# jcribeiro98/V-GAN

Hardware: AMD Instinct MI355X
Metric: V-GAN train steps/sec (batch=1024, d=784) (higher is better)
Workload: dtype f32; MMD contractions of `value`: split-bf16 x3 on the bf16 MFMA with fp32 accumulation (centred operand); the same step with the fp32 MFMA is timed in `fp32_mode`; 1 GPU; configs[2]: MNIST-pixels-as-features stand-in, d=784, batch=1024 (VGAN_no_kl step); global_batch=1024, features=784, latent=49, rows_per_gpu=1024, parallelism=dp1 (row-sharded Gram, replicated front), hip_graph=True, generator=collapsed, chain_association=depth, mmd_precision=bf16x3, gram_tile=64

## Files before the change

include/vgan_hip.h:

```cpp
#ifndef VGAN_HIP_H
#define VGAN_HIP_H

#include <stdint.h>

#ifdef __cplusplus
extern "C" {
#endif

#define VGAN_OK 0
#define VGAN_ERR_ARG 1
#define VGAN_ERR_HIP 2

#define VGAN_ABI_VERSION 11

typedef void* vgan_stream_t;

int vgan_abi_version(void);
const char* vgan_last_error(void);

int vgan_linear_forward(const float* x, int ldx, int x_nslabs, int64_t x_slab_stride, const float* W,
                        int ldw, const float* b, float* y, int ldy, int n, int in, int out,
                        vgan_stream_t stream);
int vgan_linear_backward_input(const float* dy, int lddy, const float* W, int ldw,
                               float* dx, int lddx, int n, int in, int out, vgan_stream_t stream);
int vgan_linear_backward_params(const float* dy, int lddy, const float* x, int ldx, int x_nslabs,
                                int64_t x_slab_stride, float* dW, int lddw, float* db, int n, int in,
                                int out, int splits, int64_t slab_stride, vgan_stream_t stream);
struct vgan_xx_job;
int vgan_linear_backward_params_xx_supported(int n, int in, int out);
int vgan_linear_backward_params_xx(const float* dy, int lddy, const float* x, int ldx, float* dW, int lddw, int n, int in,
                                   int out, const struct vgan_xx_job* xx, vgan_stream_t stream);
int vgan_reduce_slabs(const float* src, int64_t slab_stride, int nslabs, float* dst, int64_t count,
                      vgan_stream_t stream);

typedef struct vgan_logits_chain {
    const float* za;
    const float* At4;
    int32_t ldza, ldat, e0, pad;
} vgan_logits_chain;
int vgan_mask_project_forward(const float* logits, int ldl, const float* data, int ldd,
                              const int32_t* rows, const uint64_t* row_cursor, int row_batches,
                              int row_stride, int row_offset, float* S, float* U, float* Zx, float* Zy,
                              int ldz, float* sqx, float* sqy, int n, int d, const float* center,
                              int norm_split, const vgan_logits_chain* chain, vgan_stream_t stream);
int vgan_col_mean(const float* data, int ldd, int rows, int d, float* out, vgan_stream_t stream);
int vgan_gather_rows(const float* data, int ldd, const int32_t* rows, const uint64_t* row_cursor,
                     int row_batches, int row_stride, int row_offset, float* out, int ldo,
                     float* sq, int n, int d, vgan_stream_t stream);
int vgan_gather_rows_split(const float* data, int ldd, const int32_t* rows, const uint64_t* row_cursor,
                           int row_batches, int row_stride, int row_offset, const float* center, float* out,
                           int ldo, float* sq, int norm_split, uint16_t* Zh, uint16_t* Zl, int kp, int n, int d,
                           vgan_stream_t stream);
int vgan_mask_backward(const float* gU, int ldg, int nslabs, int64_t slab_stride, const float* S,
                       int lds, const uint64_t* colkey, float pen_weight, int row_offset,
                       float* dlogits, int ldo, int n, int d, vgan_stream_t stream);
int vgan_colmax_chunks(int n);
int vgan_colmax(const float* S, int lds, int from_softmax, int row_offset, uint64_t* part,
                uint64_t* colkey, int n, int d, vgan_stream_t stream);
int vgan_colmax_partial(const float* S, int lds, int from_softmax, int row_offset, uint64_t* part,
                        int n, int d, vgan_stream_t stream);
int vgan_mask_from_softmax(const float* S, int lds, float* U, int ldu, int n, int d, vgan_stream_t stream);
int vgan_upper_softmax_forward(const float* logits, int ldl, float* S, float* U, int n, int d,
                               vgan_stream_t stream);

#define VGAN_TILE 64
#define VGAN_TILE_INTS 8
#define VGAN_TF_SLOT_MASK 3
#define VGAN_TF_TWICE 4
#define VGAN_TF_STORE 8
#define VGAN_TF_MIRROR 16
#define VGAN_TF_NEG 32

int vgan_mmd_build_tiles(int n, int grad_mode, int rank, int world, int tile, int32_t* out, int cap);
int vgan_mmd_order_tiles(int32_t* tiles, int count, int tile);

int vgan_mmd_gram(const float* Z, int ldz, const float* sq, int n, int p, const float* bw,
                  const int32_t* tiles, int ntiles, int calibrate,
                  float* Wg, int ldw, int wrow0, float* partial, vgan_stream_t stream);
#define VGAN_RBF_MAX_KERNELS 8
int vgan_mmd_gram_general(const float* Z, int ldz, const float* sq, int n, int p, const float* bw,
                          const int32_t* tiles, int ntiles, const float* multipliers, int n_kernels,
                          float* Wg, int ldw, int wrow0, float* partial, vgan_stream_t stream);
int vgan_mmd_gram_colmax(const float* Z, int ldz, const float* sq, int n, int p, const float* bw,
                         const int32_t* tiles, int ntiles, float* Wg, int ldw, int wrow0, float* partial,
                         const float* S, int lds, int from_softmax, int row_offset, uint64_t* colpart,
                         int nrows, int d, vgan_stream_t stream);
int vgan_mmd_reduce(const float* partial, const int32_t* tiles, int ntiles, double* stats,
                    int zero_first, vgan_stream_t stream);
int vgan_mmd_set_bandwidth(const double* stats, int n, float* bw, vgan_stream_t stream);
int vgan_mmd_loss(const double* stats, const uint64_t* colkey, int n, int d, float weight,
                  float* loss, float* loss_accum, float accum_scale, uint64_t* step_counter,
                  vgan_stream_t stream);
int vgan_mmd_finalize(const float* partial, const int32_t* tiles, int ntiles, const uint64_t* colpart,
                      int chunks, uint64_t* colkey, int n, int d, float weight, double* stats,
                      float* loss, float* loss_accum, float accum_scale, uint64_t* step_counter,
                      vgan_stream_t stream);
typedef struct vgan_finalize_job {
    const float* partial;
    const int32_t* tiles;
    const uint64_t* colpart;
    uint64_t* colkey;
    double* stats;
    float* loss;
    float* loss_accum;
    uint64_t* step_counter;
    int32_t ntiles, chunks, n, d;
    float weight, accum_scale;
    int32_t mode, ntiles_main;
} vgan_finalize_job;
int vgan_mmd_backward(const float* Wg, int ldw, const float* Z, int ldz, int wrow0, int nr,
                      int ncols, int p, const float* mul, int ldmul, const float* mul_shift, float* out,
                      int ldo, int splits, int64_t slab_stride, const vgan_finalize_job* finalize,
                      vgan_stream_t stream);
int vgan_mmd_bf3_prepare(const float* Z, int ldz, int rows, int p, uint16_t* Zh, uint16_t* Zl, int kp,
                         uint16_t* ZTh, uint16_t* ZTl, int kn, vgan_stream_t stream);
int64_t vgan_mmd_gram_bf3_tail_ws_bytes(void);
int vgan_mmd_gram_bf3(const uint16_t* Zh, const uint16_t* Zl, int kp, const float* sq, int n, const float* bw,
                      const int32_t* tiles, int ntiles, int tile, uint16_t* Wh, uint16_t* Wl, int ldw,
                      int wrow0, float* partial, const float* S, int lds, int from_softmax, int row_offset,
                      uint64_t* colpart, int nrows, int d, void* tail_ws, int64_t tail_ws_bytes,
                      float* rs_part, int ldrs, vgan_stream_t stream);
int vgan_mmd_backward_bf3_tile(int nr, int p, int splits, int tile);
int vgan_mmd_backward_bf3(const uint16_t* Wh, const uint16_t* Wl, int ldw, const uint16_t* ZTh,
                          const uint16_t* ZTl, int kn, int kp, const float* Z, int ldz, int wrow0, int nr,
                          int p, const float* mul, int ldmul, const float* mul_shift, float* out, int ldo,
                          int splits, int64_t slab_stride, int tile, const vgan_finalize_job* finalize,
                          vgan_stream_t stream);
int vgan_mmd_backward_bf3_rm(const uint16_t* Wh, const uint16_t* Wl, int ldw, int kn, const uint16_t* Zh,
                             const uint16_t* Zl, int kp, int zrows, const float* Z, int ldz, int wrow0, int nr,
                             int p, const float* mul, int ldmul, const float* mul_shift, float* out, int ldo,
                             int splits, int64_t slab_stride, int tile, const vgan_finalize_job* finalize,
                             const float* rs_part, int ldrs, vgan_stream_t stream);
int vgan_mmd_backward_bf3_rm_xx(const uint16_t* Wh, const uint16_t* Wl, int ldw, int kn, const uint16_t* Zh,
                                const uint16_t* Zl, int kp, int zrows, const float* Z, int ldz, int wrow0, int nr,
                                int p, const float* mul, int ldmul, const float* mul_shift, float* out, int ldo,
                                int splits, int64_t slab_stride, const vgan_finalize_job* finalize,
                                const struct vgan_xx_job* xx, vgan_stream_t stream);
#define VGAN_GEMM_MAX_GROUP 4
#define VGAN_GEMM_NN 0
#define VGAN_GEMM_NT 1
#define VGAN_GEMM_TN 2
#define VGAN_GEMM_NT_NT 3
typedef struct vgan_gemm_problem {
    const float* a;
    const float* b;
    float* c;
    int32_t kind, m, n, k, lda, ldb, ldc, splitk;
    const float* d;
    float* scratch;
    int32_t ldd, k2;
} vgan_gemm_problem;
int vgan_gemm_grouped(const vgan_gemm_problem* problems, int count, vgan_stream_t stream);
typedef struct vgan_adadelta_layer {
    float* w_packed;
    int64_t off_w, off_b;
    int32_t ldp, out, in, pad;
} vgan_adadelta_layer;
typedef struct vgan_grouped_extras {
    const float* copy_src;
    float* copy_dst;
    int64_t copy_count;
    int32_t adadelta, pad;
    float* p;
    float* sq_avg;
    float* acc_delta;
    float lr, rho, eps, weight_decay, grad_scale;
    int32_t ld_extra;
    vgan_adadelta_layer layer[VGAN_GEMM_MAX_GROUP + 1];
    const float* g_extra;
    float* next_noise;
    int32_t noise_rows, noise_cols, noise_ld, noise_ones_col;
    uint64_t seed;
    const uint64_t* step_counter;
    const vgan_finalize_job* fold;
} vgan_grouped_extras;
int vgan_gemm_grouped_ex(const vgan_gemm_problem* problems, int count, const vgan_grouped_extras* extras,
                         vgan_stream_t stream);

typedef struct vgan_xx_job {
    const uint16_t* Dh;
    const uint16_t* Dl;
    const float* dsq;
    const int32_t* tiles;
    const float* bw;
    float* partial;
    int32_t ldd, ntiles;
} vgan_xx_job;
int vgan_mask_project_forward_bf3(const float* logits, int ldl, const float* data, int ldd, const int32_t* rows,
                                  const uint64_t* row_cursor, int row_batches, int row_stride, float* S, float* Z,
                                  int ldz, float* sq, uint16_t* Zh, uint16_t* Zl, int kp, uint16_t* ZTh,
                                  uint16_t* ZTl, int kn, int n, int d, const float* center, int write_x,
                                  const vgan_xx_job* xx, const vgan_logits_chain* chain, vgan_stream_t stream);
int vgan_row_sqnorm(const float* Z, int ldz, float* sq, int rows, int p, vgan_stream_t stream);

int vgan_adadelta_step(float* p, const float* g, int nslabs, int64_t slab_stride, float* sq_avg,
                       float* acc_delta, int64_t count, float lr, float rho, float eps,
                       float weight_decay, float grad_scale, vgan_stream_t stream);

int vgan_noise_normal(float* z, int rows, int cols, int ld, int ones_col, uint64_t seed,
                      const uint64_t* step_counter, uint64_t stream_id, vgan_stream_t stream);

int vgan_homogeneous_pack(const int64_t* desc, int count, int max_elems, int unpack, vgan_stream_t stream);
int vgan_adadelta_step_packed(float* p, const int32_t* pmap, const float* g_packed, float* w_packed,
                              float* sq_avg, float* acc_delta, int64_t count, float lr, float rho,
                              float eps, float weight_decay, float grad_scale, float* next_noise,
                              int noise_rows, int noise_cols, int noise_ld, int noise_ones_col,
                              uint64_t seed, const uint64_t* step_counter, vgan_stream_t stream);

int vgan_mse(const float* a, int lda, const float* b, int ldb, int n, int d, float scale,
             float* out, int accumulate, vgan_stream_t stream);

int vgan_mse_grad(const float* target, int ldt, const float* pred, int ldp, int n, int d, float gscale,
                  double* part, float* g, int ldg, vgan_stream_t stream);
int vgan_sum_f64(const double* in, int count, double scale, float* out, int accumulate, vgan_stream_t stream);

#define VGAN_DP_ID_BYTES 128
typedef struct vgan_dp_comm vgan_dp_comm;
int vgan_dp_unique_id(uint8_t* id );
int vgan_dp_comm_create(vgan_dp_comm** comm, int nranks, const uint8_t* id, int rank);
int vgan_dp_allreduce_sum(vgan_dp_comm* comm, float* buf, int64_t count, vgan_stream_t stream);
int vgan_dp_allgather(vgan_dp_comm* comm, void* buf, int64_t bytes_per_rank, vgan_stream_t stream);
int vgan_dp_comm_destroy(vgan_dp_comm* comm);

int vgan_shuffle_epoch(int32_t* perm, int64_t count, int64_t train_size, uint64_t seed, uint64_t epoch,
                       vgan_stream_t stream);
int64_t vgan_shuffle_index(int64_t i, int64_t train_size, uint64_t seed, uint64_t epoch);
int vgan_mask_unique(const uint8_t* masks, int ldm, int n, int d, uint64_t* keys, int32_t* work,
                     int32_t* out_row, int32_t* out_count, vgan_stream_t stream);

int vgan_rbf_kernel_matrix(const float* Z, int ldz, int m, int p, const float* sq, float alpha, float* K, int ldk,
                           vgan_stream_t stream);
int vgan_rbf_multi_kernel_matrix(const float* Z, int ldz, int m, int p, const float* sq, const float* bw,
                                 const float* multipliers, int n_kernels, float* K, int ldk, float* dK, int lddk,
                                 vgan_stream_t stream);
int vgan_rows_dot(const float* A, int lda, const float* B, int ldb, double* out, int rows, int cols,
                  vgan_stream_t stream);

#define VGAN_OUTLIER_MAX_K 32
#define VGAN_OUTLIER_ENGINE_EXACT 0
#define VGAN_OUTLIER_ENGINE_GRAM 1
#define VGAN_OUTLIER_KNN_LARGEST 0
#define VGAN_OUTLIER_KNN_MEAN 1
#define VGAN_OUTLIER_KNN_MEDIAN 2
#define VGAN_OUTLIER_LRD 3
#define VGAN_OUTLIER_LOF 4
#define VGAN_OUTLIER_KDE_MAX_ROWS 8388607
int vgan_outlier_pack(const float* X, int ldx, int n, int d, const float* center, const int32_t* feat,
                      const int32_t* feat_off, const int64_t* col_off, int first, int count, float* packed, float* sq,
                      vgan_stream_t stream);
int vgan_outlier_knn(const float* Pq, const float* sq_q, int nq, const float* Pr, const float* sq_r, int nr,
                     const int32_t* feat_off, const int64_t* col_off, int first, int count, int k, int exclude_self,
                     int engine, int splits, float* part_d, int32_t* part_i, int32_t* nbr, vgan_stream_t stream);
int vgan_outlier_refine(const float* Xq, int ldq, int nq, const float* Xr, int ldr, int nr, int d, const int32_t* feat,
                        const int32_t* feat_off, int first, int count, const int32_t* nbr, int k, int32_t* out_idx,
                        float* out_dist, float* kdist, vgan_stream_t stream);
int vgan_outlier_score(const int32_t* idx, const float* dist, int nq, int k, int count, int method, const float* kdist_ref,
                       const double* lrd_ref, int nr, float* score, const int32_t* score_row, int ld_score, double* lrd_out,
                       vgan_stream_t stream);
int vgan_outlier_kde(const float* Pq, const float* sq_q, int nq, const float* Pr, const float* sq_r, int nr,
                     const int32_t* feat_off, const int64_t* col_off, int first, int count, const double* bandwidth,
                     int exclude_self, int engine, int splits, uint32_t* pivot, uint64_t* acc, float* score,
                     const int32_t* score_row, int ld_score, vgan_stream_t stream);
int vgan_outlier_combine(const float* score, int ld, int S, int n, const double* weights, double* out,
                         vgan_stream_t stream);
int vgan_outlier_abod(const float* Xq, int ldq, int nq, const float* Xr, int ldr, int nr, int d, const int32_t* feat,
                      const int32_t* feat_off, int first, int count, const int32_t* idx, int k, float* score,
                      const int32_t* score_row, int ld_score, vgan_stream_t stream);
int vgan_outlier_abod_floor(float* score, int ld, int S, int n, int fit, double* score_floor, int32_t* n_degenerate,
                            vgan_stream_t stream);
#define VGAN_OUTLIER_NORM_ZSCORE 1
#define VGAN_OUTLIER_NORM_ROBUST 2
#define VGAN_OUTLIER_NORM_MINMAX 3
#define VGAN_OUTLIER_COMBINE_SUM 0
#define VGAN_OUTLIER_COMBINE_MAX 1
int64_t vgan_outlier_score_stats_ws_bytes(int S, int n, int mode);
int vgan_outlier_score_stats(const float* score, int ld, int S, int n, int mode, double* center, double* scale,
                             void* workspace, int64_t workspace_bytes, vgan_stream_t stream);
int vgan_outlier_combine_normalized(const float* score, int ld, int S, int n, const double* center, const double* scale,
                                    const double* weights, int combination, double* out, vgan_stream_t stream);

#define VGAN_CLUSTER_MAX_CLUSTERS 64
#define VGAN_CLUSTER_SLICE_ROWS 1024
int64_t vgan_cluster_lloyd_ws_bytes(int n, int n_clusters, int count, int total_dims);
int vgan_cluster_image(const double* centers, int n_clusters, const int32_t* feat, const int32_t* feat_off,
                       const int64_t* col_off, int first, int count, const float* col_center, float* img, float* img_sq,
                       vgan_stream_t stream);
int vgan_cluster_lloyd(const float* Pq, const float* sq_q, const float* X, int ldx, int n, int d, const int32_t* feat,
                       const int32_t* feat_off, const int64_t* col_off, int first, int count, int total_dims, int max_dims,
                       int n_clusters, int engine, const float* col_center, const double* tol_var, double* centers,
                       float* img, float* img_sq, int32_t* label, int32_t* changed, int32_t* done, int32_t* n_iter,
                       void* workspace, int64_t workspace_bytes, int iterations, vgan_stream_t stream);
int vgan_cluster_final(const float* Xq, int ldq, int nq, int d, const int32_t* feat, const int32_t* feat_off, int S,
                       int n_clusters, const double* centers, const int32_t* large, int64_t* sizes, int use_weights,
                       int32_t* label, double* inertia_part, double* inertia, float* score, const int32_t* score_row,
                       int ld_score, vgan_stream_t stream);

#ifdef __cplusplus
}
#endif
#endif
```

v-gan_amd/csrc/mmd_bf16.hip:

```cpp
#include "gemm_bf3.hpp"
#include "gemm_bf3w.hpp"
#include "mmd_common.hpp"
#include "mmd_xx.hpp"

namespace vgan {


__global__ __launch_bounds__(kBlock) void bf3_prepare_kernel(const float* __restrict__ Z, int ldz, int rows, int p,
                                                            unsigned short* __restrict__ Zh, unsigned short* __restrict__ Zl, int kp,
                                                            unsigned short* __restrict__ ZTh, unsigned short* __restrict__ ZTl, int kn,
                                                            int vec) {
    __shared__ unsigned short th[64][68], tl[64][68];
    const int j0 = blockIdx.x * 64, k0 = blockIdx.y * 64;
    const int tj = 4 * (threadIdx.x & 15), tk = 4 * (threadIdx.x >> 4);
    unsigned short hi[4][4], lo[4][4];
#pragma unroll
    for (int a = 0; a < 4; ++a) {
        const int k = k0 + tk + a;
        float v[4] = {0.f, 0.f, 0.f, 0.f};
        if (k < rows) {
            if (vec && j0 + tj + 3 < p) {
                const float4 q = *reinterpret_cast<const float4*>(Z + (long)k * ldz + j0 + tj);
                v[0] = q.x; v[1] = q.y; v[2] = q.z; v[3] = q.w;
            } else {
// ... 296 lines not shown
#pragma unroll
            for (int i = 0; i < 4; ++i)
#pragma unroll
                for (int j = 0; j < 4; ++j)
                    __builtin_amdgcn_raw_buffer_store_b128(__builtin_bit_cast(u32x4, acc[i][j]), slabs, mine + (4 * i + j) * (G::NCONS * 16), 0, kCoherent);
        }
        asm volatile("s_waitcnt vmcnt(0)" ::: "memory");
        __syncthreads();
        if (threadIdx.x == 0) {
            const int old = __hip_atomic_fetch_add(ts.tickets + tq, 1, __ATOMIC_RELAXED, __HIP_MEMORY_SCOPE_AGENT);
            last_part = old == ts.parts - 1;
            if (old == ts.parts - 1) __hip_atomic_store(ts.tickets + tq, 0, __ATOMIC_RELAXED, __HIP_MEMORY_SCOPE_AGENT);
        }
        __syncthreads();
        if (!last_part) return;
        if (cons) {
#pragma unroll
            for (int i = 0; i < 4; ++i)
#pragma unroll
                for (int j = 0; j < 4; ++j) acc[i][j] = f32x4w{0.f, 0.f, 0.f, 0.f};
            for (int q = 0; q < ts.parts; ++q) {
                const int theirs = slab0 + q * (int)kTailSlabBytes + threadIdx.x * 16;
#pragma unroll
                for (int i = 0; i < 4; ++i)
#pragma unroll
                    for (int j = 0; j < 4; ++j)
                        acc[i][j] += __builtin_bit_cast(f32x4w, __builtin_amdgcn_raw_buffer_load_b128(slabs, theirs + (4 * i + j) * (G::NCONS * 16), 0, kCoherent));
            }
        }
    }

    const float c2 = -1.4426950408889634f / (4.f * bw);
    const float wscale = -((td.flags & VGAN_TF_NEG) ? -1.f : 1.f) * 2.f / ((float)n * (float)n * bw);
    const bool store = (td.flags & VGAN_TF_STORE) && Wh != nullptr;
    const bool mirror = store && (td.flags & VGAN_TF_MIRROR);
    float ksum = 0.f;
    if (cons) {
#pragma unroll
        for (int i = 0; i < 4; ++i)
#pragma unroll
            for (int j = 0; j < 4; ++j)
#pragma unroll
                for (int r = 0; r < 4; ++r) {
                    const bool ok = (td.r0 + G::sub_row(i, r) < td.rlim) && (td.c0 + G::sub_col(j) < td.clim);
                    const float L = fmaxf(siv[i][r] + sjv[j] - 2.f * acc[i][j][r], 0.f);
                    const float t = __builtin_amdgcn_exp2f(L * c2);
                    const float t2 = t * t, t4 = t2 * t2, t8 = t4 * t4, t16 = t8 * t8;
                    ksum += ok ? ((t + t2) + (t4 + t8)) + t16 : 0.f;
                    acc[i][j][r] = wscale * (((0.25f * t + 0.5f * t2) + (t4 + 2.f * t8)) + 4.f * t16);
                }
    }
    if (store) {
        lds_f* Wt = (lds_f*)(float*)lds;
        auto emit = [&](const float (&w)[16], long rowo, int c_first, int c_lim) -> float {
            unsigned hp[8], lp[8];
            float sums[4] = {0.f, 0.f, 0.f, 0.f};
#pragma unroll
            for (int e = 0; e < 8; ++e) {
                unsigned short h0, l0, h1, l1;
                split_bf16(w[2 * e], h0, l0);
                split_bf16(w[2 * e + 1], h1, l1);
                hp[e] = (unsigned)h0 | ((unsigned)h1 << 16);
                lp[e] = (unsigned)l0 | ((unsigned)l1 << 16);
                const float v0 = __uint_as_float((unsigned)h0 << 16) + __uint_as_float((unsigned)l0 << 16);
                const float v1 = __uint_as_float((unsigned)h1 << 16) + __uint_as_float((unsigned)l1 << 16);
                sums[e & 3] += (c_first + 2 * e < c_lim ? v0 : 0.f) + (c_first + 2 * e + 1 < c_lim ? v1 : 0.f);
            }
            if (c_first + 15 < c_lim) {
                uint4* dh = reinterpret_cast<uint4*>(Wh + rowo + c_first);
                uint4* dl = reinterpret_cast<uint4*>(Wl + rowo + c_first);
                dh[0] = make_uint4(hp[0], hp[1], hp[2], hp[3]);
                dh[1] = make_uint4(hp[4], hp[5], hp[6], hp[7]);
                dl[0] = make_uint4(lp[0], lp[1], lp[2], lp[3]);
                dl[1] = make_uint4(lp[4], lp[5], lp[6], lp[7]);
            } else {
#pragma unroll
                for (int e = 0; e < 16; ++e)
                    if (c_first + e < c_lim) {
                        Wh[rowo + c_first + e] = (unsigned short)(hp[e >> 1] >> (16 * (e & 1)));
                        Wl[rowo + c_first + e] = (unsigned short)(lp[e >> 1] >> (16 * (e & 1)));
                    }
            }
            return (sums[0] + sums[1]) + (sums[2] + sums[3]);
        };
        auto slot_sum = [&](float v) -> float {
            v += __shfl_xor(v, 1);
            v += __shfl_xor(v, 2);
            v += __shfl_xor(v, 4);
            return v;
        };
        float w[16];
        if (cons) {
#pragma unroll
            for (int i = 0; i < 4; ++i)
#pragma unroll
                for (int j = 0; j < 4; ++j)
#pragma unroll
                    for (int r = 0; r < 4; ++r) Wt[G::sub_row(i, r) * LDT + G::sub_col(j)] = acc[i][j][r];
        }
        __syncthreads();
        for (int t = threadIdx.x; t < 256 * 8; t += G::NTH) {
            const int line = t >> 3, q16 = 16 * (t & 7);
            float cs = 0.f;
            if (td.r0 + line < td.rlim && td.c0 + q16 < td.clim) {
#pragma unroll
                for (int e = 0; e < 4; ++e) {
                    const f32x4 v = *(const lds_f4*)(Wt + line * LDT + q16 + 4 * e);
                    w[4 * e] = v[0]; w[4 * e + 1] = v[1]; w[4 * e + 2] = v[2]; w[4 * e + 3] = v[3];
                }
                cs = emit(w, (long)(td.r0 + line - wrow0) * ldw, td.c0 + q16, td.clim);
            }
            if (rs_part != nullptr) {
                cs = slot_sum(cs);
                if ((t & 7) == 0 && td.r0 + line < td.rlim) rs_part[(long)(td.c0 >> 7) * ldrs + (td.r0 + line - wrow0)] = cs;
            }
        }
        if (mirror) {
            __syncthreads();
            if (cons) {
#pragma unroll
                for (int i = 0; i < 4; ++i)
#pragma unroll
                    for (int j = 0; j < 4; ++j)
                        *(lds_f4*)(Wt + G::sub_col(j) * LDM + G::sub_row(i, 0)) = f32x4{acc[i][j][0], acc[i][j][1], acc[i][j][2], acc[i][j][3]};
            }
            __syncthreads();
            for (int t = threadIdx.x; t < 128 * 16; t += G::NTH) {
                const int line = t >> 4, q16 = 16 * (t & 15);
                float cs = 0.f;
                if (td.c0 + line < td.clim && td.r0 + q16 < td.rlim) {
#pragma unroll
                    for (int e = 0; e < 4; ++e) {
                        const f32x4 v = *(const lds_f4*)(Wt + line * LDM + q16 + 4 * e);
                        w[4 * e] = v[0]; w[4 * e + 1] = v[1]; w[4 * e + 2] = v[2]; w[4 * e + 3] = v[3];
                    }
                    cs = emit(w, (long)(td.c0 + line - wrow0) * ldw, td.r0 + q16, td.rlim);
                }
                if (rs_part != nullptr) {
                    cs = slot_sum(cs);
                    if ((t & 7) == 0 && td.c0 + line < td.clim && td.r0 + q16 < td.rlim)
                        rs_part[(long)((td.r0 + q16) >> 7) * ldrs + (td.c0 + line - wrow0)] = cs;
                }
            }
        }
    }
    ksum = wave_sum(ksum);
    if (lane == 0) red[wave] = ksum;
    __syncthreads();
    if (threadIdx.x == 0)
        reinterpret_cast<float4*>(partial)[ti] =
            make_float4(((red[0] + red[1]) + (red[2] + red[3])) + ((red[4] + red[5]) + (red[6] + red[7])), 0.f, 0.f, 0.f);
}

template <int BK, bool RM>
__global__ __launch_bounds__(kBlock, BK == 64 ? 2 : 3) void mmd_backward_bf3_kernel(const unsigned short* __restrict__ Wh, const unsigned short* __restrict__ Wl,
                                                                    int ldw, const unsigned short* __restrict__ ZTh,
                                                                    const unsigned short* __restrict__ ZTl, int kn, int ldb, int brows,
                                                                    const float* __restrict__ Z, int ldz, int wrow0, int nr, int p,
                                                                    int ptiles, const float* __restrict__ mul, int ldmul,
                                                                    const float* __restrict__ mul_shift, float* __restrict__ out, int ldo,
                                                                    int kchunk, long slab_stride, vgan_finalize_job job, int nfin,
                                                                    XXJob xx) {
    using G = GemmBF3<BK>;
    constexpr int kBytes = (RM ? G::kLdsBytesT : G::kLdsBytes) > G::kLdsBytes ? (RM ? G::kLdsBytesT : G::kLdsBytes) : G::kLdsBytes;
    __shared__ __attribute__((aligned(16))) char lds[kBytes];
    __shared__ float rs[64];
    const int gx = ptiles, gy = (nr + 63) / 64, total = gx * gy;
    if ((int)blockIdx.x >= total) {
        if (blockIdx.y != 0) return;
        const int extra = (int)blockIdx.x - total;
        if (extra < nfin)
            finalize_body(job);
        else if constexpr (BK == 64)
            xx_tile_body(xx, extra - nfin, lds, rs);
        return;
    }
    const int xcd = blockIdx.x % 8, kidx = blockIdx.x / 8;
    const int q = total / 8, r8 = total % 8;
    const int t = (xcd < r8 ? xcd * (q + 1) : r8 * (q + 1) + (xcd - r8) * q) + kidx;
    const int band = t / (4 * gx), rem = t - band * 4 * gx;
    const int rows_in_band = min(4, gy - band * 4);
    const int m0 = (band * 4 + rem % rows_in_band) * 64, n0 = (rem / rows_in_band) * 64;
    f32x16 acc;
#pragma unroll
    for (int r = 0; r < 16; ++r) acc[r] = 0.f;
    const int k0 = blockIdx.y * kchunk, klen = min(kchunk, kn - k0);
    out += blockIdx.y * slab_stride;
    const int col = n0 + G::sub_col(), colc = min(col, p - 1);
    float z_pre[16], m_pre[16];
    const float mshift = mul_shift != nullptr ? mul_shift[colc] : 0.f;
#pragma unroll
    for (int r = 0; r < 16; ++r) {
        const int rowc = min(m0 + G::sub_row(r), nr - 1);
        z_pre[r] = Z[(long)(wrow0 + rowc) * ldz + colc];
        m_pre[r] = mul != nullptr ? mul[(long)rowc * ldmul + colc] + mshift : 1.f;
    }
    if (klen > 0) {
        if constexpr (RM)
            G::template run_bt<true>(Wh + k0, Wl + k0, ldw, ZTh + (long)k0 * ldb, ZTl + (long)k0 * ldb, ldb, brows - k0, m0, n0, nr, klen, lds,
                                     rs, acc);
        else
            G::template run<true>(Wh + k0, Wl + k0, ldw, ZTh + k0, ZTl + k0, ldb, m0, n0, nr, gx * 64, klen, lds, rs, acc);
    }
    if (col >= p) return;
#pragma unroll
    for (int r = 0; r < 16; ++r) {
        const int lrow = G::sub_row(r), row = m0 + lrow;
        if (row < nr) {
            const float v = klen > 0 ? 2.f * (rs[lrow] * z_pre[r] - acc[r]) : 0.f;
            out[(long)row * ldo + col] = v * m_pre[r];
        }
    }
}

template <bool RM>
__global__ __launch_bounds__(512, 2) void mmd_backward_bf3_big_kernel(const unsigned short* __restrict__ Wh, const unsigned short* __restrict__ Wl,
                                                                      int ldw, const unsigned short* __restrict__ ZTh,
                                                                      const unsigned short* __restrict__ ZTl, int kn, int ldb, int brows,
                                                                      const float* __restrict__ Z, int ldz, int wrow0, int nr, int p,
                                                                      int ptiles, const float* __restrict__ mul, int ldmul,
                                                                      const float* __restrict__ mul_shift, float* __restrict__ out, int ldo,
                                                                      int kchunk, long slab_stride, int nb_rows, vgan_finalize_job job) {
    using G = GemmBF3Big;
    __shared__ __attribute__((aligned(16))) char lds[RM ? G::kLdsBytesT : G::kLdsBytes];
    __shared__ float rs[128];
    const int gx = ptiles, gy = (nr + 127) / 128, total = gx * gy;
    if ((int)blockIdx.x >= total) {
        if (blockIdx.y == 0) finalize_body(job);
        return;
    }
    const int xcd = blockIdx.x % 8, kidx = blockIdx.x / 8;
    const int q = total / 8, r8 = total % 8;
    const int t = (xcd < r8 ? xcd * (q + 1) : r8 * (q + 1) + (xcd - r8) * q) + kidx;
    const int band = t / (4 * gx), rem = t - band * 4 * gx;
    const int rows_in_band = min(4, gy - band * 4);
    const int m0 = (band * 4 + rem % rows_in_band) * 128, n0 = (rem / rows_in_band) * 128;
    const int k0 = blockIdx.y * kchunk, klen = min(kchunk, kn - k0);
    out += blockIdx.y * slab_stride;
    const int col = n0 + G::sub_col(), colc = min(col, p - 1);
    const float mshift = mul_shift != nullptr ? mul_shift[colc] : 0.f;
    f32x16 acc[2];
#pragma unroll
    for (int i2 = 0; i2 < 2; ++i2)
#pragma unroll
        for (int r = 0; r < 16; ++r) acc[i2][r] = 0.f;
    if (klen > 0) {
        if constexpr (RM)
            G::template run_bt<true>(Wh + k0, Wl + k0, ldw, ZTh + (long)k0 * ldb, ZTl + (long)k0 * ldb, ldb, nb_rows, brows - k0, m0, n0, nr, klen,
                                     lds, acc, rs);
        else
            G::template run<true>(Wh + k0, Wl + k0, ldw, ZTh + k0, ZTl + k0, ldb, m0, n0, nr, nb_rows, klen, lds, acc, rs);
    }
    if (col >= p) return;
#pragma unroll
    for (int i2 = 0; i2 < 2; ++i2) {
        float z_pre[16], m_pre[16];
#pragma unroll
        for (int r = 0; r < 16; ++r) {
            const int rowc = min(m0 + G::sub_row(i2, r), nr - 1);
            z_pre[r] = Z[(long)(wrow0 + rowc) * ldz + colc];
            m_pre[r] = mul != nullptr ? mul[(long)rowc * ldmul + colc] + mshift : 1.f;
        }
#pragma unroll
        for (int r = 0; r < 16; ++r) {
            const int lrow = G::sub_row(i2, r), row = m0 + lrow;
            if (row < nr) {
                const float v = klen > 0 ? 2.f * (rs[lrow] * z_pre[r] - acc[i2][r]) : 0.f;
                out[(long)row * ldo + col] = v * m_pre[r];
            }
        }
    }
}


__global__ __launch_bounds__(768, 3) void mmd_backward_bf3_wide_kernel(const unsigned short* __restrict__ Wh, const unsigned short* __restrict__ Wl,
                                                                       int ldw, const unsigned short* __restrict__ Bh,
                                                                       const unsigned short* __restrict__ Bl, int kn, int ldb, int brows,
                                                                       const float* __restrict__ Z, int ldz, int wrow0, int nr, int p,
                                                                       int ptiles, const float* __restrict__ mul, int ldmul,
                                                                       const float* __restrict__ mul_shift, float* __restrict__ out, int ldo,
                                                                       int kchunk, long slab_stride, int nb_cols, vgan_finalize_job job,
                                                                       const float* __restrict__ rs_part, int ldrs) {
    using G = GemmBF3Wide;
    extern __shared__ __attribute__((aligned(16))) char lds[];
    __shared__ float rs[256];
    const int gx = ptiles, gy = (nr + 255) / 256, total = gx * gy;
    if ((int)blockIdx.x >= total) {
        if (blockIdx.y == 0) finalize_body(job);
        return;
    }
    const int xcd = blockIdx.x % 8, kidx = blockIdx.x / 8;
    const int q = total / 8, r8 = total % 8;
    const int t = (xcd < r8 ? xcd * (q + 1) : r8 * (q + 1) + (xcd - r8) * q) + kidx;
    const int band = t / (4 * gx), rem = t - band * 4 * gx;
    const int rows_in_band = min(4, gy - band * 4);
    const int m0 = (band * 4 + rem % rows_in_band) * 256, n0 = (rem / rows_in_band) * 128;
    const int k0 = blockIdx.y * kchunk, klen = min(kchunk, kn - k0);
    out += blockIdx.y * slab_stride;
    f32x4w acc[4][4];
#pragma unroll
    for (int i = 0; i < 4; ++i)
#pragma unroll
        for (int j = 0; j < 4; ++j) acc[i][j] = f32x4w{0.f, 0.f, 0.f, 0.f};
    if (klen > 0 && rs_part != nullptr) {
        if (threadIdx.x < 256) {
            const float* src = rs_part + min(m0 + (int)threadIdx.x, nr - 1);
            const int s0 = k0 >> 7, s1 = (k0 + klen + 127) >> 7;
            float a0 = 0.f, a1 = 0.f, a2 = 0.f, a3 = 0.f;
            int sl = s0;
            for (; sl + 4 <= s1; sl += 4) {
                a0 += src[(long)sl * ldrs];
                a1 += src[(long)(sl + 1) * ldrs];
                a2 += src[(long)(sl + 2) * ldrs];
                a3 += src[(long)(sl + 3) * ldrs];
            }
            for (; sl < s1; ++sl) a0 += src[(long)sl * ldrs];
            rs[threadIdx.x] = (a0 + a1) + (a2 + a3);
        }
        G::run_bt<false>(Wh + k0, Wl + k0, ldw, Bh + (long)k0 * ldb, Bl + (long)k0 * ldb, ldb, nb_cols, brows - k0, m0, n0, nr, klen, lds, acc);
    } else if (klen > 0)
        G::run_bt<true>(Wh + k0, Wl + k0, ldw, Bh + (long)k0 * ldb, Bl + (long)k0 * ldb, ldb, nb_cols, brows - k0, m0, n0, nr, klen, lds, acc, rs);
    if (G::is_loader()) return;
#pragma unroll
    for (int j = 0; j < 4; ++j) {
        const int col = n0 + G::sub_col(j);
        if (col >= p) continue;
        const float mshift = mul_shift != nullptr ? mul_shift[col] : 0.f;
#pragma unroll
        for (int i = 0; i < 4; ++i) {
            float z_pre[4], m_pre[4];
#pragma unroll
            for (int r = 0; r < 4; ++r) {
                const int rowc = min(m0 + G::sub_row(i, r), nr - 1);
                z_pre[r] = Z[(long)(wrow0 + rowc) * ldz + col];
                m_pre[r] = mul != nullptr ? mul[(long)rowc * ldmul + col] + mshift : 1.f;
            }
#pragma unroll
            for (int r = 0; r < 4; ++r) {
                const int lrow = G::sub_row(i, r), row = m0 + lrow;
                if (row < nr) {
                    const float v = klen > 0 ? 2.f * (rs[lrow] * z_pre[r] - acc[i][j][r]) : 0.f;
                    out[(long)row * ldo + col] = v * m_pre[r];
                }
            }
        }
    }
}

}

using namespace vgan;

extern "C" int vgan_mmd_bf3_prepare(const float* Z, int ldz, int rows, int p, uint16_t* Zh, uint16_t* Zl, int kp, uint16_t* ZTh,
                                    uint16_t* ZTl, int kn, vgan_stream_t stream) {
    VGAN_CHECK_ARG(Z && Zh && Zl && rows > 0 && p > 0 && ldz >= p && kp >= p && kp % 64 == 0 && aligned16(Zh) && aligned16(Zl));
    VGAN_CHECK_ARG((ZTh == nullptr) == (ZTl == nullptr) && (ZTh == nullptr || (kn >= rows && kn % 64 == 0)));
    dim3 grid(kp / 64, (rows + 63) / 64);
    if (ZTh != nullptr) grid.y = kn / 64;
    const int vec = (ldz % 4 == 0) && aligned16(Z);
    hipLaunchKernelGGL(bf3_prepare_kernel, grid, dim3(kBlock), 0, (hipStream_t)stream, Z, ldz, rows, p, Zh, Zl, kp, ZTh, ZTl, kn, vec);
    VGAN_CHECK_LAUNCH();
    return VGAN_OK;
}

#ifndef VGAN_TAIL_MAX_PARTS
#define VGAN_TAIL_MAX_PARTS 4
#endif
extern "C" int64_t vgan_mmd_gram_bf3_tail_ws_bytes(void) { return kTailSlabs * kTailSlabBytes + kTailTicketBytes; }

extern "C" int vgan_mmd_gram_bf3(const uint16_t* Zh, const uint16_t* Zl, int kp, const float* sq, int n, const float* bw,
                                 const int32_t* tiles, int ntiles, int tile, uint16_t* Wh, uint16_t* Wl, int ldw, int wrow0,
                                 float* partial, const float* S, int lds, int from_softmax, int row_offset, uint64_t* colpart,
                                 int nrows, int d, void* tail_ws, int64_t tail_ws_bytes, float* rs_part, int ldrs,
                                 vgan_stream_t stream) {
    VGAN_CHECK_ARG(Zh && Zl && sq && bw && tiles && partial && n > 0 && ntiles > 0 && kp > 0 && kp % 64 == 0);
    VGAN_CHECK_ARG((Wh == nullptr) == (Wl == nullptr) && (reinterpret_cast<uintptr_t>(partial) & 15) == 0);
    VGAN_CHECK_ARG(aligned16(Zh) && aligned16(Zl) && (Wh == nullptr || (aligned16(Wh) && aligned16(Wl))));
    ColmaxJob cj{};
    int extra = 0;
    if (S != nullptr) {
        VGAN_CHECK_ARG(colpart && nrows > 0 && d > 0 && lds >= d);
        cj = ColmaxJob{S, reinterpret_cast<unsigned long long*>(colpart), lds, row_offset, nrows, d, from_softmax, (d + 63) / 64};
        extra = cj.nbx * ((nrows + kColChunkRows - 1) / kColChunkRows);
    }
    VGAN_CHECK_ARG(tile == 64 || tile == 128 || tile == 256);
    VGAN_CHECK_ARG(rs_part == nullptr || (tile == 256 && Wh != nullptr && ldrs > 0 && wrow0 >= 0 && n % 128 == 0));
    if (tile == 256) {
        static const hipError_t attr = hipFuncSetAttribute(reinterpret_cast<const void*>(&mmd_gram_bf3_wide_kernel),
                                                           hipFuncAttributeMaxDynamicSharedMemorySize, GemmBF3Wide::kLdsBytes);
        VGAN_CHECK_ARG(attr == hipSuccess);
        TailSplit ts{nullptr, nullptr, ntiles, 1, kp};
        if (tail_ws != nullptr) {
            VGAN_CHECK_ARG(tail_ws_bytes >= vgan_mmd_gram_bf3_tail_ws_bytes() && aligned16(tail_ws));
            static const int cus = [] {
                int dev = 0, v = 0;
                if (hipGetDevice(&dev) != hipSuccess || hipDeviceGetAttribute(&v, hipDeviceAttributeMultiprocessorCount, dev) != hipSuccess) v = 0;
                return v;
            }();
            const int slots = cus < kTailSlabs ? cus : kTailSlabs;
            const int r = slots > 0 ? ntiles % slots : 0, nst = kp / GemmBF3Wide::BK;
            int parts = 1;
            while (r > 0 && parts < VGAN_TAIL_MAX_PARTS && 2 * parts * r <= slots && nst / (2 * parts) >= 8) parts *= 2;
            if (parts > 1) {
                const int kchunk = ((nst + parts - 1) / parts) * GemmBF3Wide::BK;
                ts = TailSplit{static_cast<float*>(tail_ws), reinterpret_cast<int*>(static_cast<char*>(tail_ws) + kTailSlabs * kTailSlabBytes),
                               ntiles - r, (kp + kchunk - 1) / kchunk, kchunk};
            }
        }
        const int nblk = ts.first + (ntiles - ts.first) * ts.parts;
        hipLaunchKernelGGL(mmd_gram_bf3_wide_kernel, dim3(nblk + extra), dim3(GemmBF3Wide::NTH), GemmBF3Wide::kLdsBytes, (hipStream_t)stream, Zh,
                           Zl, kp, sq, n, bw, reinterpret_cast<const TileDesc*>(tiles), ntiles, Wh, Wl, ldw, wrow0, partial, cj, ts, rs_part, ldrs);
    } else if (tile == 128)
        hipLaunchKernelGGL(mmd_gram_bf3_big_kernel, dim3(ntiles + extra), dim3(512), 0, (hipStream_t)stream, Zh, Zl, kp, sq, n, bw,
                           reinterpret_cast<const TileDesc*>(tiles), ntiles, Wh, Wl, ldw, wrow0, partial, cj);
    else
        hipLaunchKernelGGL(mmd_gram_bf3_kernel<64>, dim3(ntiles + extra), dim3(kBlock), 0, (hipStream_t)stream, Zh, Zl, kp, sq, n, bw,
                           reinterpret_cast<const TileDesc*>(tiles), ntiles, Wh, Wl, ldw, wrow0, partial, cj);
    VGAN_CHECK_LAUNCH();
    return VGAN_OK;
}

extern "C" int vgan_mmd_backward_bf3_tile(int nr, int p, int splits, int tile) {
    if (tile == 64 || tile == 128 || tile == 256) return tile;
    const int wide_tiles = ((p + 127) / 128) * ((nr + 255) / 256);
    if (nr >= 256 && wide_tiles * splits >= 256) return 256;
    const int big_tiles = ((p + 127) / 128) * ((nr + 127) / 128);
    return big_tiles * splits >= 512 ? 128 : 64;
}

static int launch_backward_bf3(int rm, const uint16_t* Wh, const uint16_t* Wl, int ldw, const uint16_t* Bh, const uint16_t* Bl, int kn, int kp,
                               int zrows, const float* Z, int ldz, int wrow0, int nr, int p, const float* mul, int ldmul,
                               const float* mul_shift, float* out, int ldo, int splits, int64_t slab_stride, int tile,
                               const vgan_finalize_job* finalize, vgan_stream_t stream, const vgan_xx_job* xxjob = nullptr,
                               const float* rs_part = nullptr, int ldrs = 0) {
    VGAN_CHECK_ARG(Wh && Wl && Bh && Bl && Z && out && nr > 0 && p > 0 && kn > 0 && kn % 64 == 0 && kp >= p && kp % 64 == 0);
    VGAN_CHECK_ARG(ldw >= kn && ldz >= p && ldo >= p && (mul == nullptr || ldmul >= p) && wrow0 >= 0);
    VGAN_CHECK_ARG(aligned16(Wh) && aligned16(Wl) && aligned16(Bh) && aligned16(Bl) && ldw % 8 == 0);
    VGAN_CHECK_ARG(splits >= 1 && splits <= 64 && (splits == 1 || slab_stride >= (int64_t)nr * ldo));
    VGAN_CHECK_ARG((tile == 0 || tile == 64 || tile == 128 || tile == 256) && (mul_shift == nullptr || mul != nullptr) && (!rm || zrows > 0));
    const int kchunk = ((kn / 64 + splits - 1) / splits) * 64;
    const int ldb = rm ? kp : kn;
    vgan_finalize_job job{};
    if (finalize != nullptr) {
        VGAN_CHECK_ARG(finalize_job_ok(*finalize));
        job = *finalize;
    }
    hipStream_t st = (hipStream_t)stream;
    XXJob xx{};
    if (xxjob != nullptr) {
        const vgan_xx_job& j = *xxjob;
        VGAN_CHECK_ARG(rm && tile == 64 && j.Dh && j.Dl && j.dsq && j.tiles && j.bw && j.partial && j.ntiles > 0 && j.ldd % 64 == 0 &&
                       aligned16(j.Dh) && aligned16(j.Dl) && (reinterpret_cast<uintptr_t>(j.partial) & 15) == 0);
        xx = XXJob{j.Dh, j.Dl, j.dsq, nullptr, nullptr, reinterpret_cast<const TileDesc*>(j.tiles), j.bw, j.partial, j.ldd, 1, 0, j.ntiles, 0};
    }
    const int nfin = finalize != nullptr ? 1 : 0;
    int edge = vgan_mmd_backward_bf3_tile(nr, p, splits, tile);
    if (edge == 256 && !rm) edge = 128;
    if (edge == 256) {
        static const hipError_t attr = hipFuncSetAttribute(reinterpret_cast<const void*>(&mmd_backward_bf3_wide_kernel),
                                                           hipFuncAttributeMaxDynamicSharedMemorySize, GemmBF3Wide::kLdsBytes);
        VGAN_CHECK_ARG(attr == hipSuccess);
        const int pt = (p + 127) / 128;
        dim3 grid(pt * ((nr + 255) / 256) + nfin, splits);
        if (rs_part != nullptr && !(ldrs >= nr && (splits == 1 || kchunk % 128 == 0))) rs_part = nullptr;
        hipLaunchKernelGGL(mmd_backward_bf3_wide_kernel, grid, dim3(GemmBF3Wide::NTH), GemmBF3Wide::kLdsBytes, st, Wh, Wl, ldw, Bh, Bl, kn, ldb,
                           zrows, Z, ldz, wrow0, nr, p, pt, mul, ldmul, mul_shift, out, ldo, kchunk, (long)slab_stride, kp, job, rs_part, ldrs);
        VGAN_CHECK_LAUNCH();
        return VGAN_OK;
    }
    if (edge == 128) {
        const int pt = (p + 127) / 128;
        dim3 grid(pt * ((nr + 127) / 128) + (finalize != nullptr ? 1 : 0), splits);
        if (rm)
            hipLaunchKernelGGL(mmd_backward_bf3_big_kernel<true>, grid, dim3(512), 0, st, Wh, Wl, ldw, Bh, Bl, kn, ldb, zrows, Z, ldz, wrow0, nr,
                               p, pt, mul, ldmul, mul_shift, out, ldo, kchunk, (long)slab_stride, kp, job);
        else
            hipLaunchKernelGGL(mmd_backward_bf3_big_kernel<false>, grid, dim3(512), 0, st, Wh, Wl, ldw, Bh, Bl, kn, ldb, 0, Z, ldz, wrow0, nr, p,
                               pt, mul, ldmul, mul_shift, out, ldo, kchunk, (long)slab_stride, kp, job);
        VGAN_CHECK_LAUNCH();
        return VGAN_OK;
    }
    const int ptiles = (p + 63) / 64;
    dim3 grid(ptiles * ((nr + 63) / 64) + nfin + xx.ntiles, splits);
    if (rm)
        hipLaunchKernelGGL((mmd_backward_bf3_kernel<64, true>), grid, dim3(kBlock), 0, st, Wh, Wl, ldw, Bh, Bl, kn, ldb, zrows, Z, ldz, wrow0, nr,
                           p, ptiles, mul, ldmul, mul_shift, out, ldo, kchunk, (long)slab_stride, job, nfin, xx);
    else
        hipLaunchKernelGGL((mmd_backward_bf3_kernel<64, false>), grid, dim3(kBlock), 0, st, Wh, Wl, ldw, Bh, Bl, kn, ldb, 0, Z, ldz, wrow0, nr, p,
                           ptiles, mul, ldmul, mul_shift, out, ldo, kchunk, (long)slab_stride, job, nfin, xx);
    VGAN_CHECK_LAUNCH();
    return VGAN_OK;
}

extern "C" int vgan_mmd_backward_bf3(const uint16_t* Wh, const uint16_t* Wl, int ldw, const uint16_t* ZTh, const uint16_t* ZTl, int kn,
                                     int kp, const float* Z, int ldz, int wrow0, int nr, int p, const float* mul, int ldmul,
                                     const float* mul_shift, float* out, int ldo, int splits, int64_t slab_stride, int tile,
                                     const vgan_finalize_job* finalize, vgan_stream_t stream) {
    return launch_backward_bf3(0, Wh, Wl, ldw, ZTh, ZTl, kn, kp, 0, Z, ldz, wrow0, nr, p, mul, ldmul, mul_shift, out, ldo, splits, slab_stride,
                               tile, finalize, stream);
}

extern "C" int vgan_mmd_backward_bf3_rm_xx(const uint16_t* Wh, const uint16_t* Wl, int ldw, int kn, const uint16_t* Zh, const uint16_t* Zl,
                                           int kp, int zrows, const float* Z, int ldz, int wrow0, int nr, int p, const float* mul, int ldmul,
                                           const float* mul_shift, float* out, int ldo, int splits, int64_t slab_stride,
                                           const vgan_finalize_job* finalize, const vgan_xx_job* xx, vgan_stream_t stream) {
    VGAN_CHECK_ARG(xx != nullptr);
    return launch_backward_bf3(1, Wh, Wl, ldw, Zh, Zl, kn, kp, zrows, Z, ldz, wrow0, nr, p, mul, ldmul, mul_shift, out, ldo, splits,
                               slab_stride, 64, finalize, stream, xx);
}

extern "C" int vgan_mmd_backward_bf3_rm(const uint16_t* Wh, const uint16_t* Wl, int ldw, int kn, const uint16_t* Zh, const uint16_t* Zl,
                                        int kp, int zrows, const float* Z, int ldz, int wrow0, int nr, int p, const float* mul, int ldmul,
                                        const float* mul_shift, float* out, int ldo, int splits, int64_t slab_stride, int tile,
                                        const vgan_finalize_job* finalize, const float* rs_part, int ldrs, vgan_stream_t stream) {
    return launch_backward_bf3(1, Wh, Wl, ldw, Zh, Zl, kn, kp, zrows, Z, ldz, wrow0, nr, p, mul, ldmul, mul_shift, out, ldo, splits,
                               slab_stride, tile, finalize, stream, nullptr, rs_part, ldrs);
}
```

v-gan_amd/csrc/rows.hip:

```cpp
#include "mmd_xx.hpp"
#include "vgan_common.hpp"

namespace vgan {

constexpr int kRowsPerBlock = kBlock / kWave;

struct RowSel {
    const int* rows;
    const unsigned long long* cursor;
    int row_batches, row_stride, row_offset;
    __device__ __forceinline__ long operator()(int i) const {
        if (rows == nullptr) return (long)(row_offset + i);
        const long b = cursor ? (long)(cursor[0] % (unsigned long long)row_batches) : 0l;
        return (long)rows[b * row_stride + row_offset + i];
    }
};

__device__ __forceinline__ float project_centred(float u, float x, float c) {
#pragma clang fp contract(off)
    const float y = u * x;
    return y - c;
}

template <bool PROJECT>
__global__ __launch_bounds__(kBlock) void mask_forward_kernel(const float* __restrict__ logits, int ldl, const float* __restrict__ data,
                                                             int ldd, RowSel rows, float* __restrict__ S,
                                                             float* __restrict__ U, float* __restrict__ Zx, float* __restrict__ Zy,
                                                             int ldz, float* __restrict__ sqx, float* __restrict__ sqy, int n, int d,
                                                             const float* __restrict__ center, int norm_split) {
    const int lane = threadIdx.x & 63;
    const int i = blockIdx.x * kRowsPerBlock + (threadIdx.x >> 6);
    if (i >= n) return;
    const float* x = logits + (long)i * ldl;
    float m = -INFINITY;
    for (int j = lane; j < d; j += 64) m = fmaxf(m, x[j]);
    m = wave_max(m);
    float sum = 0.f;
    for (int j = lane; j < d; j += 64) sum += expf(x[j] - m);
    sum = wave_sum(sum);
    const float tau = 1.0f / (float)d;
    const float* xr = nullptr;
    float *zx = nullptr, *zy = nullptr;
    if constexpr (PROJECT) {
        const long src = rows(i);
        xr = data + src * ldd;
        zx = Zx ? Zx + (long)i * ldz : nullptr;
        zy = Zy + (long)i * ldz;
    }
    float nx = 0.f, ny = 0.f;
    for (int j = lane; j < d; j += 64) {
        const float s = expf(x[j] - m) / sum;
        const float u = s < tau ? s : 1.0f;
        S[(long)i * d + j] = s;
        if (U) U[(long)i * d + j] = u;
        if constexpr (PROJECT) {
            const float c = center ? center[j] : 0.f;
            const float xv = xr[j] - c;
            const float yv = project_centred(u, xr[j], c);
            if (zx) zx[j] = xv;
            zy[j] = yv;
            const float xn = norm_split ? split_value(xv) : xv, yn = norm_split ? split_value(yv) : yv;
            nx = fmaf(xn, xn, nx);
            ny = fmaf(yn, yn, ny);
        }
    }
    if constexpr (PROJECT) {
        nx = wave_sum(nx);
        ny = wave_sum(ny);
        if (lane == 0) {
            if (sqx) sqx[i] = nx;
            sqy[i] = ny;
        }
    }
}


struct LogitsChain {
    const float* za;
    const float* At4;
    int ldza, ldat, e0;
};
constexpr int kChainK = 16;
__host__ __device__ constexpr int chain_pitch(int d) { return ((d + 3) / 4) * 4 + 4; }

template <int NT>
__device__ __forceinline__ void chain_logits(const LogitsChain& ch, float* __restrict__ lds_at, int d, int row, bool row_ok, float4 (&v)[NT]) {
    const int lane = threadIdx.x & 63, nq = d >> 2, pitch = chain_pitch(d);
#pragma unroll
    for (int t = 0; t < NT; ++t) v[t] = make_float4(0.f, 0.f, 0.f, 0.f);
    const float* zr = ch.za + (long)(row_ok ? row : 0) * ch.ldza;
    for (int kc = 0; kc < ch.e0; kc += kChainK) {
        __syncthreads();
        for (int idx = threadIdx.x; idx < d * (kChainK / 4); idx += blockDim.x) {
            const int col = idx / (kChainK / 4), kq = idx % (kChainK / 4), k = kc + 4 * kq;
            const float4 a = k < ch.e0 ? *reinterpret_cast<const float4*>(ch.At4 + (long)col * ch.ldat + k) : make_float4(0.f, 0.f, 0.f, 0.f);
            lds_at[(4 * kq + 0) * pitch + col] = a.x;
            lds_at[(4 * kq + 1) * pitch + col] = a.y;
            lds_at[(4 * kq + 2) * pitch + col] = a.z;
            lds_at[(4 * kq + 3) * pitch + col] = a.w;
        }
        __syncthreads();
        const int kw = min(kChainK, ch.e0 - kc);
        for (int k = 0; k < kw; ++k) {
            const float z = zr[kc + k];
#pragma unroll
            for (int t = 0; t < NT; ++t) {
                const int q = min(lane + 64 * t, nq - 1);
                const float4 a = *reinterpret_cast<const float4*>(lds_at + k * pitch + 4 * q);
                v[t].x = fmaf(z, a.x, v[t].x);
                v[t].y = fmaf(z, a.y, v[t].y);
                v[t].z = fmaf(z, a.z, v[t].z);
                v[t].w = fmaf(z, a.w, v[t].w);
            }
        }
    }
#pragma unroll
    for (int t = 0; t < NT; ++t)
        if (lane + 64 * t >= nq) v[t] = make_float4(-INFINITY, -INFINITY, -INFINITY, -INFINITY);
}

template <int NT, bool CHAIN>
__global__ __launch_bounds__(kBlock) void mask_forward_vec_kernel(const float* __restrict__ logits, int ldl, const float* __restrict__ data,
                                                                 int ldd, RowSel rows, float* __restrict__ S, float* __restrict__ U,
                                                                 float* __restrict__ Zx, float* __restrict__ Zy, int ldz,
                                                                 float* __restrict__ sqx, float* __restrict__ sqy, int n, int d,
                                                                 const float* __restrict__ center, int norm_split, LogitsChain ch) {
    extern __shared__ __attribute__((aligned(16))) float chain_lds[];
    const int lane = threadIdx.x & 63;
    const int i = blockIdx.x * kRowsPerBlock + (threadIdx.x >> 6);
    const int nq = d >> 2;
    float4 v[NT], xv[NT], cv[NT];
    if constexpr (CHAIN) chain_logits<NT>(ch, chain_lds, d, i, i < n, v);
    if (i >= n) return;
    const float4* x4 = reinterpret_cast<const float4*>(logits + (long)i * ldl);
    const float4* xr4 = reinterpret_cast<const float4*>(data + rows(i) * ldd);
#pragma unroll
    for (int t = 0; t < NT; ++t) {
        const int q = lane + 64 * t;
        const bool ok = q < nq;
        if constexpr (!CHAIN) v[t] = ok ? x4[min(q, nq - 1)] : make_float4(-INFINITY, -INFINITY, -INFINITY, -INFINITY);
        xv[t] = xr4[min(q, nq - 1)];
        cv[t] = center ? reinterpret_cast<const float4*>(center)[min(q, nq - 1)] : make_float4(0.f, 0.f, 0.f, 0.f);
    }
    float m = -INFINITY;
#pragma unroll
    for (int t = 0; t < NT; ++t) m = fmaxf(m, fmaxf(fmaxf(v[t].x, v[t].y), fmaxf(v[t].z, v[t].w)));
    m = wave_max(m);
    float sum = 0.f;
#pragma unroll
    for (int t = 0; t < NT; ++t) {
        v[t].x = expf(v[t].x - m); v[t].y = expf(v[t].y - m); v[t].z = expf(v[t].z - m); v[t].w = expf(v[t].w - m);
        sum += (v[t].x + v[t].y) + (v[t].z + v[t].w);
    }
    sum = wave_sum(sum);
    const float tau = 1.0f / (float)d;
    float nx = 0.f, ny = 0.f;
#pragma unroll
    for (int t = 0; t < NT; ++t) {
        const int q = lane + 64 * t;
        if (q < nq) {
            float4 s4 = make_float4(v[t].x / sum, v[t].y / sum, v[t].z / sum, v[t].w / sum);
            float4 u4 = make_float4(s4.x < tau ? s4.x : 1.f, s4.y < tau ? s4.y : 1.f, s4.z < tau ? s4.z : 1.f, s4.w < tau ? s4.w : 1.f);
            const float4 x4c = make_float4(xv[t].x - cv[t].x, xv[t].y - cv[t].y, xv[t].z - cv[t].z, xv[t].w - cv[t].w);
            const float4 y4 = make_float4(project_centred(u4.x, xv[t].x, cv[t].x), project_centred(u4.y, xv[t].y, cv[t].y), project_centred(u4.z, xv[t].z, cv[t].z),
                                              project_centred(u4.w, xv[t].w, cv[t].w));
            reinterpret_cast<float4*>(S + (long)i * d)[q] = s4;
            if (U) reinterpret_cast<float4*>(U + (long)i * d)[q] = u4;
            if (Zx) reinterpret_cast<float4*>(Zx + (long)i * ldz)[q] = x4c;
            reinterpret_cast<float4*>(Zy + (long)i * ldz)[q] = y4;
            const float xs[4] = {x4c.x, x4c.y, x4c.z, x4c.w}, ys[4] = {y4.x, y4.y, y4.z, y4.w};
            float xn[4], yn[4];
#pragma unroll
            for (int e = 0; e < 4; ++e) {
                xn[e] = norm_split ? split_value(xs[e]) : xs[e];
                yn[e] = norm_split ? split_value(ys[e]) : ys[e];
            }
            nx += (xn[0] * xn[0] + xn[1] * xn[1]) + (xn[2] * xn[2] + xn[3] * xn[3]);
            ny += (yn[0] * yn[0] + yn[1] * yn[1]) + (yn[2] * yn[2] + yn[3] * yn[3]);
        }
    }
    nx = wave_sum(nx);
    ny = wave_sum(ny);
    if (lane == 0) {
        if (sqx) sqx[i] = nx;
        sqy[i] = ny;
    }
}

template <int NT, bool XX, bool CHAIN>
__global__ __launch_bounds__(512) void mask_forward_bf3_kernel(const float* __restrict__ logits, int ldl, const float* __restrict__ data,
                                                                 int ldd, RowSel rows, float* __restrict__ S, float* __restrict__ Z,
                                                                 int ldz, float* __restrict__ sq, unsigned short* __restrict__ Zh,
                                                                 unsigned short* __restrict__ Zl, int kp, unsigned short* __restrict__ ZTh,
                                                                 unsigned short* __restrict__ ZTl, int kn, int n, int d,
                                                                 const float* __restrict__ center, int write_x, int mask_blocks,
                                                                 XXJob xx, LogitsChain ch) {
    constexpr int R = 8;
    if constexpr (XX) {
        __shared__ __attribute__((aligned(16))) char xx_lds[GemmBF3<64>::kLdsBytes];
        __shared__ float xx_red[4];
        if ((int)blockIdx.x >= mask_blocks) {
            xx_tile_body(xx, blockIdx.x - mask_blocks, xx_lds, xx_red);
            return;
        }
    }
    extern __shared__ __attribute__((aligned(16))) unsigned short tile[];
    const int ldt = 4 * (d >> 2) + 8;
    const int lane = threadIdx.x & 63, wave = threadIdx.x >> 6;
    const int nq = d >> 2;
    const int groups = n / R, C = (groups + 7) / 8;
    const int grp = (blockIdx.x % 8) * C + blockIdx.x / 8;
    if (grp >= groups) return;
    const int i0 = grp * R;
    const float tau = 1.0f / (float)d;
    {
        const int lr = wave, i = i0 + lr;
        float4 v[NT];
        if constexpr (CHAIN) chain_logits<NT>(ch, reinterpret_cast<float*>(tile), d, i, i < n, v);
        if (i < n) {
            const float4* x4 = reinterpret_cast<const float4*>(logits + (long)i * ldl);
            const float4* xr4 = reinterpret_cast<const float4*>(data + rows(i) * ldd);
            float4 xv[NT], cv[NT];
#pragma unroll
            for (int t = 0; t < NT; ++t) {
                const int q = lane + 64 * t;
                const bool ok = q < nq;
                if constexpr (!CHAIN) v[t] = ok ? x4[min(q, nq - 1)] : make_float4(-INFINITY, -INFINITY, -INFINITY, -INFINITY);
                xv[t] = xr4[min(q, nq - 1)];
                cv[t] = center ? reinterpret_cast<const float4*>(center)[min(q, nq - 1)] : make_float4(0.f, 0.f, 0.f, 0.f);
            }
            float m = -INFINITY;
#pragma unroll
            for (int t = 0; t < NT; ++t) m = fmaxf(m, fmaxf(fmaxf(v[t].x, v[t].y), fmaxf(v[t].z, v[t].w)));
            m = wave_max(m);
            float sum = 0.f;
#pragma unroll
            for (int t = 0; t < NT; ++t) {
                v[t].x = expf(v[t].x - m); v[t].y = expf(v[t].y - m); v[t].z = expf(v[t].z - m); v[t].w = expf(v[t].w - m);
                sum += (v[t].x + v[t].y) + (v[t].z + v[t].w);
            }
            sum = wave_sum(sum);
            float nx = 0.f, ny = 0.f;
#pragma unroll
            for (int t = 0; t < NT; ++t) {
                const int q = lane + 64 * t;
                if (q < nq) {
                    const float4 s4 = make_float4(v[t].x / sum, v[t].y / sum, v[t].z / sum, v[t].w / sum);
                    const float4 u4 = make_float4(s4.x < tau ? s4.x : 1.f, s4.y < tau ? s4.y : 1.f, s4.z < tau ? s4.z : 1.f, s4.w < tau ? s4.w : 1.f);
                    const float4 x4c = make_float4(xv[t].x - cv[t].x, xv[t].y - cv[t].y, xv[t].z - cv[t].z, xv[t].w - cv[t].w);
                    const float4 y4 = make_float4(project_centred(u4.x, xv[t].x, cv[t].x), project_centred(u4.y, xv[t].y, cv[t].y), project_centred(u4.z, xv[t].z, cv[t].z),
                                              project_centred(u4.w, xv[t].w, cv[t].w));
                    reinterpret_cast<float4*>(S + (long)i * d)[q] = s4;
                    if (write_x) reinterpret_cast<float4*>(Z + (long)i * ldz)[q] = x4c;
                    reinterpret_cast<float4*>(Z + (long)(n + i) * ldz)[q] = y4;
                    const float xs[4] = {x4c.x, x4c.y, x4c.z, x4c.w}, ys[4] = {y4.x, y4.y, y4.z, y4.w};
                    unsigned short h[2][4], l[2][4];
                    float xn[4], yn[4];
#pragma unroll
                    for (int e = 0; e < 4; ++e) {
                        split_bf16(xs[e], h[0][e], l[0][e]);
                        split_bf16(ys[e], h[1][e], l[1][e]);
                        xn[e] = bf16_val(h[0][e]) + bf16_val(l[0][e]);
                        yn[e] = bf16_val(h[1][e]) + bf16_val(l[1][e]);
                    }
                    nx += (xn[0] * xn[0] + xn[1] * xn[1]) + (xn[2] * xn[2] + xn[3] * xn[3]);
                    ny += (yn[0] * yn[0] + yn[1] * yn[1]) + (yn[2] * yn[2] + yn[3] * yn[3]);
#pragma unroll
                    for (int im = 0; im < 2; ++im) {
                        const uint2 ph = make_uint2((unsigned)h[im][0] | ((unsigned)h[im][1] << 16), (unsigned)h[im][2] | ((unsigned)h[im][3] << 16));
                        const uint2 pl = make_uint2((unsigned)l[im][0] | ((unsigned)l[im][1] << 16), (unsigned)l[im][2] | ((unsigned)l[im][3] << 16));
                        const long grow = (long)(im * n + i) * kp + 4 * q;
                        if (im == 1 || write_x) {
                            *reinterpret_cast<uint2*>(Zh + grow) = ph;
                            *reinterpret_cast<uint2*>(Zl + grow) = pl;
                        }
                        if (ZTh != nullptr) {
                            *reinterpret_cast<uint2*>(tile + ((2 * im) * R + lr) * ldt + 4 * q) = ph;
                            *reinterpret_cast<uint2*>(tile + ((2 * im + 1) * R + lr) * ldt + 4 * q) = pl;
                        }
                    }
                }
            }
            nx = wave_sum(nx);
            ny = wave_sum(ny);
            if (lane == 0) {
                if (write_x) sq[i] = nx;
                sq[n + i] = ny;
            }
        } else if (ZTh != nullptr) {
            for (int c = lane; c < ldt; c += 64)
#pragma unroll
                for (int im = 0; im < 4; ++im) tile[(im * R + lr) * ldt + c] = 0;
        }
    }
    if (ZTh == nullptr) return;
    __syncthreads();
    const int npairs = d >> 1;
    for (int item = threadIdx.x; item < 4 * npairs; item += 512) {
        const int im = item / npairs, j = 2 * (item - im * npairs);
        unsigned w0[4], w1[4];
#pragma unroll
        for (int e = 0; e < 4; ++e) {
            const unsigned a = *reinterpret_cast<const unsigned*>(tile + (im * R + 2 * e) * ldt + j);
            const unsigned c = *reinterpret_cast<const unsigned*>(tile + (im * R + 2 * e + 1) * ldt + j);
            w0[e] = (a & 0xFFFFu) | (c << 16);
            w1[e] = (a >> 16) | (c & 0xFFFF0000u);
        }
        unsigned short* dst = ((im & 1) ? ZTl : ZTh) + (long)j * kn + (im >> 1) * n + i0;
        *reinterpret_cast<uint4*>(dst) = make_uint4(w0[0], w0[1], w0[2], w0[3]);
        *reinterpret_cast<uint4*>(dst + kn) = make_uint4(w1[0], w1[1], w1[2], w1[3]);
    }
}

template <int NT>
__global__ __launch_bounds__(kBlock) void mask_backward_vec_kernel(const float* __restrict__ gU, int ldg, const float* __restrict__ S,
                                                                  int lds, const unsigned long long* __restrict__ colkey,
                                                                  float pen_weight, int row_offset, float* __restrict__ dlogits,
                                                                  int ldo, int n, int d, int nslabs, long slab_stride) {
    const int lane = threadIdx.x & 63;
    const int i = blockIdx.x * kRowsPerBlock + (threadIdx.x >> 6);
    if (i >= n) return;
    const int nq = d >> 2;
    const float tau = 1.0f / (float)d;
    const float pg = -pen_weight / (float)d;
    const unsigned me = (unsigned)(row_offset + i);
    float4 sv[NT], gs[NT];
    float dot = 0.f;
#pragma unroll
    for (int t = 0; t < NT; ++t) {
        const int q = min(lane + 64 * t, nq - 1);
        const bool ok = lane + 64 * t < nq;
        sv[t] = reinterpret_cast<const float4*>(S + (long)i * lds)[q];
        float4 g = reinterpret_cast<const float4*>(gU + (long)i * ldg)[q];
        for (int sl = 1; sl < nslabs; ++sl) {
            const float4 b = reinterpret_cast<const float4*>(gU + sl * slab_stride + (long)i * ldg)[q];
            g.x += b.x; g.y += b.y; g.z += b.z; g.w += b.w;
        }
        if (colkey != nullptr) {
            const ulonglong2 k0 = reinterpret_cast<const ulonglong2*>(colkey)[2 * q], k1 = reinterpret_cast<const ulonglong2*>(colkey)[2 * q + 1];
            if (colkey_row(k0.x) == me) g.x += pg;
            if (colkey_row(k0.y) == me) g.y += pg;
            if (colkey_row(k1.x) == me) g.z += pg;
            if (colkey_row(k1.y) == me) g.w += pg;
        }
        gs[t] = make_float4(ok && sv[t].x < tau ? g.x : 0.f, ok && sv[t].y < tau ? g.y : 0.f, ok && sv[t].z < tau ? g.z : 0.f,
                            ok && sv[t].w < tau ? g.w : 0.f);
        dot += (gs[t].x * sv[t].x + gs[t].y * sv[t].y) + (gs[t].z * sv[t].z + gs[t].w * sv[t].w);
    }
    dot = wave_sum(dot);
#pragma unroll
    for (int t = 0; t < NT; ++t) {
        const int q = lane + 64 * t;
        if (q < nq)
            reinterpret_cast<float4*>(dlogits + (long)i * ldo)[q] =
                make_float4(sv[t].x * (gs[t].x - dot), sv[t].y * (gs[t].y - dot), sv[t].z * (gs[t].z - dot), sv[t].w * (gs[t].w - dot));
    }
}

__global__ __launch_bounds__(kBlock) void mask_backward_kernel(const float* __restrict__ gU, int ldg, const float* __restrict__ S,
                                                              int lds, const unsigned long long* __restrict__ colkey,
                                                              float pen_weight, int row_offset, float* __restrict__ dlogits,
                                                              int ldo, int n, int d, int nslabs, long slab_stride) {
    const int lane = threadIdx.x & 63;
    const int i = blockIdx.x * kRowsPerBlock + (threadIdx.x >> 6);
    if (i >= n) return;
    const float tau = 1.0f / (float)d;
    const float pg = -pen_weight / (float)d;
    const float* g = gU + (long)i * ldg;
    const float* s = S + (long)i * lds;
    const unsigned me = (unsigned)(row_offset + i);
    auto grad = [&](int j) {
        float gv = g[j];
        for (int q = 1; q < nslabs; ++q) gv += g[q * slab_stride + j];
        if (colkey != nullptr && colkey_row(colkey[j]) == me) gv += pg;
        return gv;
    };
    float dot = 0.f;
    for (int j = lane; j < d; j += 64) {
        const float sv = s[j];
        dot = fmaf(sv < tau ? grad(j) : 0.f, sv, dot);
    }
    dot = wave_sum(dot);
    for (int j = lane; j < d; j += 64) {
        const float sv = s[j];
        dlogits[(long)i * ldo + j] = sv * ((sv < tau ? grad(j) : 0.f) - dot);
    }
}

__global__ __launch_bounds__(kBlock) void colmax_partial_kernel(const float* __restrict__ S, int lds, int row_offset,
                                                               unsigned long long* __restrict__ part, int n, int d, int from_softmax) {
    colmax_partial_body<4>(S, lds, row_offset, part, n, d, from_softmax, blockIdx.x, blockIdx.y);
}
__global__ void colmax_final_kernel(const unsigned long long* __restrict__ part, int chunks, unsigned long long* __restrict__ colkey,
                                    int d) {
    const int j = blockIdx.x * blockDim.x + threadIdx.x;
    if (j >= d) return;
    unsigned long long b = 0ull;
    for (int c = 0; c < chunks; ++c) {
        const unsigned long long k = part[(long)c * d + j];
        b = k > b ? k : b;
    }
    colkey[j] = b;
}

__global__ __launch_bounds__(kBlock) void gather_rows_kernel(const float* __restrict__ data, int ldd, RowSel rows,
                                                            float* __restrict__ out, int ldo, float* __restrict__ sq, int n, int d) {
    const int lane = threadIdx.x & 63;
    const int i = blockIdx.x * kRowsPerBlock + (threadIdx.x >> 6);
    if (i >= n) return;
    const float* x = data + rows(i) * ldd;
    float* o = out + (long)i * ldo;
    float nx = 0.f;
    for (int j = lane; j < d; j += 64) {
        const float v = x[j];
        o[j] = v;
        nx = fmaf(v, v, nx);
    }
    nx = wave_sum(nx);
    if (lane == 0 && sq) sq[i] = nx;
}

__global__ __launch_bounds__(kBlock) void gather_center_split_kernel(const float* __restrict__ data, int ldd, RowSel rows,
                                                                    const float* __restrict__ center, float* __restrict__ out, int ldo,
                                                                    float* __restrict__ sq, int norm_split,
                                                                    unsigned short* __restrict__ Zh, unsigned short* __restrict__ Zl,
                                                                    int kp, int n, int d) {
    const int lane = threadIdx.x & 63;
    const int i = blockIdx.x * kRowsPerBlock + (threadIdx.x >> 6);
    if (i >= n) return;
    const float* x = data + rows(i) * ldd;
    float nx = 0.f;
    for (int j = lane; j < d; j += 64) {
        const float v = x[j] - (center ? center[j] : 0.f);
        if (out) out[(long)i * ldo + j] = v;
        unsigned short hi, lo;
        split_bf16(v, hi, lo);
        if (Zh) {
            Zh[(long)i * kp + j] = hi;
            Zl[(long)i * kp + j] = lo;
        }
        const float vn = norm_split ? bf16_val(hi) + bf16_val(lo) : v;
        nx = fmaf(vn, vn, nx);
    }
    nx = wave_sum(nx);
    if (lane == 0 && sq) sq[i] = nx;
}

__global__ __launch_bounds__(kBlock) void gather_center_split_vec_kernel(const float* __restrict__ data, int ldd, RowSel rows,
                                                                        const float* __restrict__ center, float* __restrict__ out, int ldo,
                                                                        float* __restrict__ sq, int norm_split,
                                                                        unsigned short* __restrict__ Zh, unsigned short* __restrict__ Zl,
                                                                        int kp, int n, int d) {
    const int lane = threadIdx.x & 63;
    const int i = blockIdx.x * kRowsPerBlock + (threadIdx.x >> 6);
    if (i >= n) return;
    const float4* x4 = reinterpret_cast<const float4*>(data + rows(i) * ldd);
    const int nq = d >> 2;
    float nx = 0.f;
    for (int q = lane; q < nq; q += 64) {
        float4 v = x4[q];
        if (center) {
            const float4 c = reinterpret_cast<const float4*>(center)[q];
            v.x -= c.x; v.y -= c.y; v.z -= c.z; v.w -= c.w;
        }
        if (out) reinterpret_cast<float4*>(out + (long)i * ldo)[q] = v;
        const float vs[4] = {v.x, v.y, v.z, v.w};
        unsigned short h[4], l[4];
        float vn[4];
#pragma unroll
        for (int e = 0; e < 4; ++e) {
            split_bf16(vs[e], h[e], l[e]);
            vn[e] = norm_split ? bf16_val(h[e]) + bf16_val(l[e]) : vs[e];
        }
        if (Zh) {
            *reinterpret_cast<uint2*>(Zh + (long)i * kp + 4 * q) = make_uint2((unsigned)h[0] | ((unsigned)h[1] << 16), (unsigned)h[2] | ((unsigned)h[3] << 16));
            *reinterpret_cast<uint2*>(Zl + (long)i * kp + 4 * q) = make_uint2((unsigned)l[0] | ((unsigned)l[1] << 16), (unsigned)l[2] | ((unsigned)l[3] << 16));
        }
        nx += (vn[0] * vn[0] + vn[1] * vn[1]) + (vn[2] * vn[2] + vn[3] * vn[3]);
    }
    nx = wave_sum(nx);
    if (lane == 0 && sq) sq[i] = nx;
}

__global__ void mask_from_softmax_kernel(const float* __restrict__ S, int lds, float* __restrict__ U, int ldu, int n, int d) {
    const long idx = (long)blockIdx.x * blockDim.x + threadIdx.x;
    if (idx >= (long)n * d) return;
    const int i = (int)(idx / d), j = (int)(idx % d);
    const float sv = S[(long)i * lds + j];
    U[(long)i * ldu + j] = sv < 1.0f / (float)d ? sv : 1.0f;
}

}

using namespace vgan;

extern "C" int vgan_mask_project_forward(const float* logits, int ldl, const float* data, int ldd, const int32_t* rows,
                                         const uint64_t* row_cursor, int row_batches, int row_stride, int row_offset, float* S,
                                         float* U, float* Zx, float* Zy, int ldz, float* sqx, float* sqy, int n, int d,
                                         const float* center, int norm_split, const vgan_logits_chain* chain, vgan_stream_t stream) {
    VGAN_CHECK_ARG((logits || chain) && data && S && Zy && sqy && n > 0 && d > 0 && (logits == nullptr || ldl >= d) && ldd >= d && ldz >= d);
    VGAN_CHECK_ARG(row_batches >= 1 && row_stride >= 0 && row_offset >= 0);
    LogitsChain ch{};
    if (chain != nullptr) {
        VGAN_CHECK_ARG(chain->za && chain->At4 && chain->e0 > 0 && chain->e0 % 4 == 0 && chain->ldza >= chain->e0 && chain->ldat >= chain->e0 &&
                       chain->ldat % 4 == 0 && aligned16(chain->At4));
        ch = LogitsChain{chain->za, chain->At4, chain->ldza, chain->ldat, chain->e0};
        if (logits == nullptr) { logits = chain->za; ldl = 4; }
    }
    const RowSel sel{rows, reinterpret_cast<const unsigned long long*>(row_cursor), row_batches, row_stride, row_offset};
    const dim3 grid((n + kRowsPerBlock - 1) / kRowsPerBlock), block(kBlock);
    hipStream_t st = (hipStream_t)stream;
    const bool vec = (d % 4 == 0) && (d <= (chain != nullptr ? 1024 : 4096)) && (ldl % 4 == 0) && (ldd % 4 == 0) && (ldz % 4 == 0) && aligned16(logits) &&
                     aligned16(data) && aligned16(S) && (U == nullptr || aligned16(U)) && (Zx == nullptr || aligned16(Zx)) && aligned16(Zy) && (center == nullptr || aligned16(center));
    if (vec) {
        const int nt = (d / 4 + 63) / 64;
        const size_t chain_bytes = (size_t)kChainK * chain_pitch(d) * sizeof(float);
#define VGAN_LAUNCH_FWD(NT)                                                                                                               \
    do {                                                                                                                                  \
        if (chain != nullptr) {                                                                                                           \
            if (chain_bytes > 64 * 1024)                                                                                                  \
                (void)hipFuncSetAttribute(reinterpret_cast<const void*>(&mask_forward_vec_kernel<NT, true>),                                \
                                          hipFuncAttributeMaxDynamicSharedMemorySize, (int)chain_bytes);                                  \
            hipLaunchKernelGGL((mask_forward_vec_kernel<NT, true>), grid, block, chain_bytes, st, logits, ldl, data, ldd, sel, S, U, Zx, Zy, ldz, \
                               sqx, sqy, n, d, center, norm_split, ch);                                                                   \
        } else                                                                                                                            \
            hipLaunchKernelGGL((mask_forward_vec_kernel<NT, false>), grid, block, 0, st, logits, ldl, data, ldd, sel, S, U, Zx, Zy, ldz, sqx, \
                               sqy, n, d, center, norm_split, ch);                                                                        \
    } while (0)
        if (nt == 1) VGAN_LAUNCH_FWD(1); else if (nt == 2) VGAN_LAUNCH_FWD(2); else if (nt == 3) VGAN_LAUNCH_FWD(3); else if (nt == 4) VGAN_LAUNCH_FWD(4);
        else if (nt <= 8)
            hipLaunchKernelGGL((mask_forward_vec_kernel<8, false>), grid, block, 0, st, logits, ldl, data, ldd, sel, S, U, Zx, Zy, ldz, sqx, sqy, n, d,
                               center, norm_split, ch);
        else
            hipLaunchKernelGGL((mask_forward_vec_kernel<16, false>), grid, block, 0, st, logits, ldl, data, ldd, sel, S, U, Zx, Zy, ldz, sqx, sqy, n, d,
                               center, norm_split, ch);
#undef VGAN_LAUNCH_FWD
    } else {
        VGAN_CHECK_ARG(chain == nullptr);
        hipLaunchKernelGGL(mask_forward_kernel<true>, grid, block, 0, st, logits, ldl, data, ldd, sel, S, U, Zx, Zy, ldz, sqx, sqy, n, d, center,
                           norm_split);
    }
    VGAN_CHECK_LAUNCH();
    return VGAN_OK;
}

extern "C" int vgan_mask_project_forward_bf3(const float* logits, int ldl, const float* data, int ldd, const int32_t* rows,
                                             const uint64_t* row_cursor, int row_batches, int row_stride, float* S, float* Z, int ldz,
                                             float* sq, uint16_t* Zh, uint16_t* Zl, int kp, uint16_t* ZTh, uint16_t* ZTl, int kn,
                                             int n, int d, const float* center, int write_x, const vgan_xx_job* xxjob,
                                             const vgan_logits_chain* chain, vgan_stream_t stream) {
    VGAN_CHECK_ARG((logits || chain) && data && S && Z && sq && Zh && Zl && n > 0 && d > 0 && (logits == nullptr || ldl >= d) && ldd >= d &&
                   ldz >= d);
    LogitsChain ch{};
    if (chain != nullptr) {
        VGAN_CHECK_ARG(ZTh == nullptr && chain->za && chain->At4 && chain->e0 > 0 && chain->e0 % 4 == 0 && chain->ldza >= chain->e0 &&
                       chain->ldat >= chain->e0 && chain->ldat % 4 == 0 && aligned16(chain->At4));
        ch = LogitsChain{chain->za, chain->At4, chain->ldza, chain->ldat, chain->e0};
        if (logits == nullptr) { logits = chain->za; ldl = 4; }
    }
    VGAN_CHECK_ARG((ZTh == nullptr) == (ZTl == nullptr));
    VGAN_CHECK_ARG(row_batches >= 1 && row_stride >= 0 && kp >= d && kp % 64 == 0 && (ZTh == nullptr || (kn >= 2 * n && kn % 64 == 0)));
    VGAN_CHECK_ARG(write_x || ZTh == nullptr);
    VGAN_CHECK_ARG(d % 4 == 0 && d <= 1024 && n % 8 == 0 && ldl % 4 == 0 && ldd % 4 == 0 && ldz % 4 == 0);
    VGAN_CHECK_ARG(aligned16(logits) && aligned16(data) && aligned16(S) && aligned16(Z) && aligned16(Zh) && aligned16(Zl) &&
                   (ZTh == nullptr || (aligned16(ZTh) && aligned16(ZTl))) && (center == nullptr || aligned16(center)));
    const RowSel sel{rows, reinterpret_cast<const unsigned long long*>(row_cursor), row_batches, row_stride, 0};
    const int mask_blocks = 8 * ((n / 8 + 7) / 8);
    XXJob xx{};
    int xx_blocks = 0;
    if (xxjob != nullptr) {
        const vgan_xx_job& j = *xxjob;
        VGAN_CHECK_ARG(ZTh == nullptr && j.Dh && j.Dl && j.dsq && j.tiles && j.bw && j.partial && j.ntiles > 0 && j.ldd >= d && j.ldd % 64 == 0);
        VGAN_CHECK_ARG(aligned16(j.Dh) && aligned16(j.Dl) && (reinterpret_cast<uintptr_t>(j.partial) & 15) == 0);
        xx = XXJob{j.Dh, j.Dl, j.dsq, rows, reinterpret_cast<const unsigned long long*>(row_cursor), reinterpret_cast<const TileDesc*>(j.tiles),
                   j.bw, j.partial, j.ldd, row_batches, row_stride, j.ntiles, n};
        xx_blocks = j.ntiles;
    }
    const dim3 grid(mask_blocks + xx_blocks), block(512);
    const size_t shmem = ZTh != nullptr ? (size_t)4 * 8 * (d + 8) * sizeof(unsigned short)
                                        : (chain != nullptr ? (size_t)kChainK * chain_pitch(d) * sizeof(float) : 0);
    hipStream_t st = (hipStream_t)stream;
    const int nt = (d / 4 + 63) / 64;
#define VGAN_LAUNCH_K3(NT, XXF, CHF)                                                                                                \
    do {                                                                                                                            \
        if (shmem > 64 * 1024)                                                                                                      \
            (void)hipFuncSetAttribute(reinterpret_cast<const void*>(&mask_forward_bf3_kernel<NT, XXF, CHF>),                          \
                                      hipFuncAttributeMaxDynamicSharedMemorySize, (int)shmem);                                      \
        hipLaunchKernelGGL((mask_forward_bf3_kernel<NT, XXF, CHF>), grid, block, shmem, st, logits, ldl, data, ldd, sel, S, Z, ldz, sq, \
                           Zh, Zl, kp, ZTh, ZTl, kn, n, d, center, write_x, mask_blocks, xx, ch);                                    \
    } while (0)
#define VGAN_LAUNCH_FWD3(NT)                                                                                                        \
    do {                                                                                                                            \
        if (xx_blocks > 0 && chain != nullptr) VGAN_LAUNCH_K3(NT, true, true);                                                      \
        else if (xx_blocks > 0) VGAN_LAUNCH_K3(NT, true, false);                                                                    \
        else if (chain != nullptr) VGAN_LAUNCH_K3(NT, false, true);                                                                 \
        else VGAN_LAUNCH_K3(NT, false, false);                                                                                      \
    } while (0)
    if (nt == 1) VGAN_LAUNCH_FWD3(1); else if (nt == 2) VGAN_LAUNCH_FWD3(2); else if (nt == 3) VGAN_LAUNCH_FWD3(3); else VGAN_LAUNCH_FWD3(4);
#undef VGAN_LAUNCH_FWD3
#undef VGAN_LAUNCH_K3
    VGAN_CHECK_LAUNCH();
    return VGAN_OK;
}

extern "C" int vgan_upper_softmax_forward(const float* logits, int ldl, float* S, float* U, int n, int d, vgan_stream_t stream) {
    VGAN_CHECK_ARG(logits && S && n > 0 && d > 0 && ldl >= d);
    hipLaunchKernelGGL(mask_forward_kernel<false>, dim3((n + kRowsPerBlock - 1) / kRowsPerBlock), dim3(kBlock), 0,
                       (hipStream_t)stream, logits, ldl, nullptr, 0, RowSel{nullptr, nullptr, 1, 0, 0}, S, U, nullptr, nullptr, 0, nullptr, nullptr, n, d, nullptr, 0);
    VGAN_CHECK_LAUNCH();
    return VGAN_OK;
}

extern "C" int vgan_mask_backward(const float* gU, int ldg, int nslabs, int64_t slab_stride, const float* S, int lds,
                                  const uint64_t* colkey, float pen_weight, int row_offset, float* dlogits, int ldo, int n, int d,
                                  vgan_stream_t stream) {
    VGAN_CHECK_ARG(gU && S && dlogits && n > 0 && d > 0 && ldg >= d && lds >= d && ldo >= d && nslabs >= 1);
    const dim3 grid((n + kRowsPerBlock - 1) / kRowsPerBlock), block(kBlock);
    hipStream_t st = (hipStream_t)stream;
    const unsigned long long* ck = reinterpret_cast<const unsigned long long*>(colkey);
    const bool vec = (d % 4 == 0) && (d <= 4096) && (ldg % 4 == 0) && (lds % 4 == 0) && (ldo % 4 == 0) && (slab_stride % 4 == 0) &&
                     aligned16(gU) && aligned16(S) && aligned16(dlogits) && (colkey == nullptr || aligned16(colkey));
    if (vec) {
        const int nt = (d / 4 + 63) / 64;
#define VGAN_LAUNCH_BWD(NT) hipLaunchKernelGGL(mask_backward_vec_kernel<NT>, grid, block, 0, st, gU, ldg, S, lds, ck, pen_weight, row_offset, dlogits, ldo, n, d, nslabs, (long)slab_stride)
        if (nt == 1) VGAN_LAUNCH_BWD(1); else if (nt == 2) VGAN_LAUNCH_BWD(2); else if (nt == 3) VGAN_LAUNCH_BWD(3); else if (nt == 4) VGAN_LAUNCH_BWD(4);
        else if (nt <= 8) VGAN_LAUNCH_BWD(8); else VGAN_LAUNCH_BWD(16);
#undef VGAN_LAUNCH_BWD
    } else
        hipLaunchKernelGGL(mask_backward_kernel, grid, block, 0, st, gU, ldg, S, lds, ck, pen_weight, row_offset, dlogits, ldo, n, d, nslabs,
                           (long)slab_stride);
    VGAN_CHECK_LAUNCH();
    return VGAN_OK;
}

extern "C" int vgan_gather_rows(const float* data, int ldd, const int32_t* rows, const uint64_t* row_cursor, int row_batches,
                                int row_stride, int row_offset, float* out, int ldo, float* sq, int n, int d, vgan_stream_t stream) {
    VGAN_CHECK_ARG(data && out && n > 0 && d > 0 && ldd >= d && ldo >= d && row_batches >= 1 && row_stride >= 0 && row_offset >= 0);
    const RowSel sel{rows, reinterpret_cast<const unsigned long long*>(row_cursor), row_batches, row_stride, row_offset};
    hipLaunchKernelGGL(gather_rows_kernel, dim3((n + kRowsPerBlock - 1) / kRowsPerBlock), dim3(kBlock), 0, (hipStream_t)stream, data,
                       ldd, sel, out, ldo, sq, n, d);
    VGAN_CHECK_LAUNCH();
    return VGAN_OK;
}

extern "C" int vgan_gather_rows_split(const float* data, int ldd, const int32_t* rows, const uint64_t* row_cursor, int row_batches,
                                      int row_stride, int row_offset, const float* center, float* out, int ldo, float* sq,
                                      int norm_split, uint16_t* Zh, uint16_t* Zl, int kp, int n, int d, vgan_stream_t stream) {
    VGAN_CHECK_ARG(data && n > 0 && d > 0 && ldd >= d && row_batches >= 1 && row_stride >= 0 && row_offset >= 0);
    VGAN_CHECK_ARG((out == nullptr || ldo >= d) && (out || sq || Zh) && (Zh == nullptr) == (Zl == nullptr) && (Zh == nullptr || kp >= d));
    const RowSel sel{rows, reinterpret_cast<const unsigned long long*>(row_cursor), row_batches, row_stride, row_offset};
    const bool vec = (d % 4 == 0) && (ldd % 4 == 0) && aligned16(data) && (center == nullptr || aligned16(center)) &&
                     (out == nullptr || (ldo % 4 == 0 && aligned16(out))) && (Zh == nullptr || (kp % 4 == 0 && aligned16(Zh) && aligned16(Zl)));
    const dim3 grid((n + kRowsPerBlock - 1) / kRowsPerBlock), block(kBlock);
    if (vec)
        hipLaunchKernelGGL(gather_center_split_vec_kernel, grid, block, 0, (hipStream_t)stream, data, ldd, sel, center, out, ldo, sq, norm_split,
                           Zh, Zl, kp, n, d);
    else
        hipLaunchKernelGGL(gather_center_split_kernel, grid, block, 0, (hipStream_t)stream, data, ldd, sel, center, out, ldo, sq, norm_split,
                           Zh, Zl, kp, n, d);
    VGAN_CHECK_LAUNCH();
    return VGAN_OK;
}

extern "C" int vgan_colmax_chunks(int n) { return n > 0 ? (n + kColChunkRows - 1) / kColChunkRows : 0; }

extern "C" int vgan_colmax_partial(const float* S, int lds, int from_softmax, int row_offset, uint64_t* part, int n, int d,
                                   vgan_stream_t stream) {
    VGAN_CHECK_ARG(S && part && n > 0 && d > 0 && lds >= d);
    hipLaunchKernelGGL(colmax_partial_kernel, dim3((d + 63) / 64, vgan_colmax_chunks(n)), dim3(kBlock), 0, (hipStream_t)stream, S,
                       lds, row_offset, reinterpret_cast<unsigned long long*>(part), n, d, from_softmax);
    VGAN_CHECK_LAUNCH();
    return VGAN_OK;
}

extern "C" int vgan_colmax(const float* S, int lds, int from_softmax, int row_offset, uint64_t* part, uint64_t* colkey, int n,
                           int d, vgan_stream_t stream) {
    VGAN_CHECK_ARG(S && part && colkey && n > 0 && d > 0 && lds >= d);
    const int chunks = vgan_colmax_chunks(n);
    hipLaunchKernelGGL(colmax_partial_kernel, dim3((d + 63) / 64, chunks), dim3(kBlock), 0, (hipStream_t)stream, S, lds, row_offset,
                       reinterpret_cast<unsigned long long*>(part), n, d, from_softmax);
    VGAN_CHECK_LAUNCH();
    hipLaunchKernelGGL(colmax_final_kernel, dim3((d + 255) / 256), dim3(256), 0, (hipStream_t)stream,
                       reinterpret_cast<const unsigned long long*>(part), chunks, reinterpret_cast<unsigned long long*>(colkey), d);
    VGAN_CHECK_LAUNCH();
    return VGAN_OK;
}

extern "C" int vgan_mask_from_softmax(const float* S, int lds, float* U, int ldu, int n, int d, vgan_stream_t stream) {
    VGAN_CHECK_ARG(S && U && n > 0 && d > 0 && lds >= d && ldu >= d);
    const long total = (long)n * d;
    hipLaunchKernelGGL(mask_from_softmax_kernel, dim3((unsigned)((total + 255) / 256)), dim3(256), 0, (hipStream_t)stream, S, lds, U,
                       ldu, n, d);
    VGAN_CHECK_LAUNCH();
    return VGAN_OK;
}
```

v-gan_amd/csrc/vgan_common.hpp:

```cpp
#pragma once
#include <hip/hip_runtime.h>
#include <stdint.h>

#include "../../include/vgan_hip.h"

namespace vgan {

typedef float f32x16 __attribute__((ext_vector_type(16)));
typedef float f32x4 __attribute__((ext_vector_type(4)));

constexpr int kWave = 64;
constexpr int kBlock = 256;

void set_error(const char* fmt, ...);

#define VGAN_CHECK_ARG(cond)                                                        \
    do {                                                                            \
        if (!(cond)) {                                                              \
            ::vgan::set_error("%s:%d: bad argument: %s", __FILE__, __LINE__, #cond); \
            return VGAN_ERR_ARG;                                                    \
        }                                                                           \
    } while (0)

#define VGAN_CHECK_LAUNCH()                                                                     \
    do {                                                                                        \
        hipError_t e_ = hipGetLastError();                                                      \
        if (e_ != hipSuccess) {                                                                 \
            ::vgan::set_error("%s:%d: launch failed: %s", __FILE__, __LINE__, hipGetErrorString(e_)); \
            return VGAN_ERR_HIP;                                                                \
        }                                                                                       \
    } while (0)

__device__ __forceinline__ float wave_sum(float v) {
#pragma unroll
    for (int o = 32; o > 0; o >>= 1) v += __shfl_xor(v, o, 64);
    return v;
}
__device__ __forceinline__ double wave_sum(double v) {
#pragma unroll
    for (int o = 32; o > 0; o >>= 1) v += __shfl_xor(v, o, 64);
    return v;
}
__device__ __forceinline__ int wave_sum(int v) {
#pragma unroll
    for (int o = 32; o > 0; o >>= 1) v += __shfl_xor(v, o, 64);
    return v;
}
__device__ __forceinline__ float wave_max(float v) {
#pragma unroll
    for (int o = 32; o > 0; o >>= 1) v = fmaxf(v, __shfl_xor(v, o, 64));
    return v;
}
__device__ __forceinline__ unsigned long long wave_max(unsigned long long v) {
#pragma unroll
    for (int o = 32; o > 0; o >>= 1) {
        unsigned long long t = __shfl_xor(v, o, 64);
        v = t > v ? t : v;
    }
    return v;
}

__device__ __forceinline__ double block_sum(double v, double* red) {
    v = wave_sum(v);
    if ((threadIdx.x & 63) == 0) red[threadIdx.x >> 6] = v;
    __syncthreads();
    return ((red[0] + red[1]) + red[2]) + red[3];
}

__device__ __forceinline__ unsigned long long colkey_pack(float u, unsigned row) {
    return ((unsigned long long)__float_as_uint(u) << 32) | (unsigned long long)(0xFFFFFFFFu - row);
}
__device__ __forceinline__ float colkey_value(unsigned long long k) { return __uint_as_float((unsigned)(k >> 32)); }
__device__ __forceinline__ unsigned colkey_row(unsigned long long k) { return 0xFFFFFFFFu - (unsigned)(k & 0xFFFFFFFFull); }

constexpr int kColChunkRows = 64;
template <int NW>
__device__ __forceinline__ void colmax_partial_body(const float* __restrict__ S, int lds, int row_offset,
                                                    unsigned long long* __restrict__ part, int n, int d, int from_softmax, int bx,
                                                    int by) {
    __shared__ unsigned long long colmax_red[NW][64];
    const int lane = threadIdx.x & 63, wave = threadIdx.x >> 6;
    const int j = bx * 64 + lane;
    const int r0 = by * kColChunkRows;
    const float tau = from_softmax ? 1.0f / (float)d : INFINITY;
    unsigned long long best = 0ull;
    if (j < d) {
        constexpr int PER = (kColChunkRows + NW - 1) / NW;
        float sv[PER];
#pragma unroll
        for (int e = 0; e < PER; ++e) sv[e] = S[(long)min(r0 + min(wave + e * NW, kColChunkRows - 1), n - 1) * lds + j];
#pragma unroll
        for (int e = 0; e < PER; ++e) {
            const unsigned long long k = colkey_pack(sv[e] < tau ? sv[e] : 1.0f,
                                                     (unsigned)(row_offset + min(r0 + min(wave + e * NW, kColChunkRows - 1), n - 1)));
            best = k > best ? k : best;
        }
    }
    colmax_red[wave][lane] = best;
    __syncthreads();
    if (wave == 0 && j < d) {
        unsigned long long b = colmax_red[0][lane];
#pragma unroll
        for (int w = 1; w < NW; ++w) b = colmax_red[w][lane] > b ? colmax_red[w][lane] : b;
        part[(long)by * d + j] = b;
    }
}

__device__ __forceinline__ unsigned short bf16_bits(float v) { return __builtin_bit_cast(unsigned short, (__bf16)v); }
__device__ __forceinline__ float bf16_val(unsigned short b) { return __uint_as_float((unsigned)b << 16); }
__device__ __forceinline__ void split_bf16(float v, unsigned short& hi, unsigned short& lo) {
    hi = bf16_bits(v);
    lo = bf16_bits(v - bf16_val(hi));
}

__device__ __forceinline__ float split_value(float v) {
    unsigned short hi, lo;
    split_bf16(v, hi, lo);
    return bf16_val(hi) + bf16_val(lo);
}

inline bool aligned16(const void* p) { return (reinterpret_cast<uintptr_t>(p) & 15) == 0; }

}
```

v-gan_amd/lib.py:

```python
import ctypes
import os

_HERE = os.path.dirname(os.path.abspath(__file__))
LIB_PATH = os.path.join(_HERE, "libvgan_hip.so")

_p = ctypes.c_void_p
_i = ctypes.c_int
_f = ctypes.c_float
_i64 = ctypes.c_int64
_u64 = ctypes.c_uint64

class FinalizeJob(ctypes.Structure):
    _fields_ = [("partial", _p), ("tiles", _p), ("colpart", _p), ("colkey", _p), ("stats", _p), ("loss", _p), ("loss_accum", _p),
                ("step_counter", _p), ("ntiles", ctypes.c_int32), ("chunks", ctypes.c_int32), ("n", ctypes.c_int32),
                ("d", ctypes.c_int32), ("weight", _f), ("accum_scale", _f), ("mode", ctypes.c_int32), ("ntiles_main", ctypes.c_int32)]


class GemmProblem(ctypes.Structure):
    _fields_ = [("a", _p), ("b", _p), ("c", _p), ("kind", ctypes.c_int32), ("m", ctypes.c_int32), ("n", ctypes.c_int32),
                ("k", ctypes.c_int32), ("lda", ctypes.c_int32), ("ldb", ctypes.c_int32), ("ldc", ctypes.c_int32), ("splitk", ctypes.c_int32),
                ("d", _p), ("scratch", _p), ("ldd", ctypes.c_int32), ("k2", ctypes.c_int32)]


class LogitsChain(ctypes.Structure):
    _fields_ = [("za", _p), ("At4", _p), ("ldza", ctypes.c_int32), ("ldat", ctypes.c_int32), ("e0", ctypes.c_int32), ("pad", ctypes.c_int32)]


class XXJob(ctypes.Structure):
    _fields_ = [("Dh", _p), ("Dl", _p), ("dsq", _p), ("tiles", _p), ("bw", _p), ("partial", _p), ("ldd", ctypes.c_int32),
                ("ntiles", ctypes.c_int32)]


class AdadeltaLayer(ctypes.Structure):
    _fields_ = [("w_packed", _p), ("off_w", _i64), ("off_b", _i64), ("ldp", ctypes.c_int32), ("out", ctypes.c_int32),
                ("inp", ctypes.c_int32), ("pad", ctypes.c_int32)]


class GroupedExtras(ctypes.Structure):
    _fields_ = [("copy_src", _p), ("copy_dst", _p), ("copy_count", _i64), ("adadelta", ctypes.c_int32), ("pad", ctypes.c_int32),
                ("p", _p), ("sq_avg", _p), ("acc_delta", _p), ("lr", _f), ("rho", _f), ("eps", _f), ("weight_decay", _f),
                ("grad_scale", _f), ("ld_extra", ctypes.c_int32), ("layer", AdadeltaLayer * 5), ("g_extra", _p), ("next_noise", _p),
                ("noise_rows", ctypes.c_int32), ("noise_cols", ctypes.c_int32), ("noise_ld", ctypes.c_int32),
                ("noise_ones_col", ctypes.c_int32), ("seed", _u64), ("step_counter", _p), ("fold", _p)]


GEMM_NN, GEMM_NT, GEMM_TN, GEMM_NT_NT = 0, 1, 2, 3
GEMM_MAX_GROUP = 4

SIGNATURES = {
    "vgan_abi_version": (_i, []),
    "vgan_last_error": (ctypes.c_char_p, []),
    "vgan_linear_forward": (_i, [_p, _i, _i, _i64, _p, _i, _p, _p, _i, _i, _i, _i, _p]),
    "vgan_linear_backward_input": (_i, [_p, _i, _p, _i, _p, _i, _i, _i, _i, _p]),
    "vgan_linear_backward_params": (_i, [_p, _i, _p, _i, _i, _i64, _p, _i, _p, _i, _i, _i, _i, _i64, _p]),
    "vgan_linear_backward_params_xx_supported": (_i, [_i, _i, _i]),
    "vgan_linear_backward_params_xx": (_i, [_p, _i, _p, _i, _p, _i, _i, _i, _i, _p, _p]),
    "vgan_reduce_slabs": (_i, [_p, _i64, _i, _p, _i64, _p]),
    "vgan_mask_project_forward": (_i, [_p, _i, _p, _i, _p, _p, _i, _i, _i, _p, _p, _p, _p, _i, _p, _p, _i, _i, _p, _i, _p, _p]),
    "vgan_col_mean": (_i, [_p, _i, _i, _i, _p, _p]),
    "vgan_gather_rows": (_i, [_p, _i, _p, _p, _i, _i, _i, _p, _i, _p, _i, _i, _p]),
    "vgan_gather_rows_split": (_i, [_p, _i, _p, _p, _i, _i, _i, _p, _p, _i, _p, _i, _p, _p, _i, _i, _i, _p]),
    "vgan_mask_backward": (_i, [_p, _i, _i, _i64, _p, _i, _p, _f, _i, _p, _i, _i, _i, _p]),
    "vgan_colmax_partial": (_i, [_p, _i, _i, _i, _p, _i, _i, _p]),
    "vgan_mmd_finalize": (_i, [_p, _p, _i, _p, _i, _p, _i, _i, _f, _p, _p, _p, _f, _p, _p]),
    "vgan_colmax_chunks": (_i, [_i]),
    "vgan_colmax": (_i, [_p, _i, _i, _i, _p, _p, _i, _i, _p]),
    "vgan_mask_from_softmax": (_i, [_p, _i, _p, _i, _i, _i, _p]),
    "vgan_upper_softmax_forward": (_i, [_p, _i, _p, _p, _i, _i, _p]),
    "vgan_mmd_build_tiles": (_i, [_i, _i, _i, _i, _i, _p, _i]),
    "vgan_mmd_order_tiles": (_i, [_p, _i, _i]),
    "vgan_mmd_gram": (_i, [_p, _i, _p, _i, _i, _p, _p, _i, _i, _p, _i, _i, _p, _p]),
    "vgan_mmd_gram_general": (_i, [_p, _i, _p, _i, _i, _p, _p, _i, _p, _i, _p, _i, _i, _p, _p]),
    "vgan_mmd_gram_colmax": (_i, [_p, _i, _p, _i, _i, _p, _p, _i, _p, _i, _i, _p, _p, _i, _i, _i, _p, _i, _i, _p]),
    "vgan_mmd_reduce": (_i, [_p, _p, _i, _p, _i, _p]),
    "vgan_mmd_set_bandwidth": (_i, [_p, _i, _p, _p]),
    "vgan_mmd_loss": (_i, [_p, _p, _i, _i, _f, _p, _p, _f, _p, _p]),
    "vgan_mmd_backward": (_i, [_p, _i, _p, _i, _i, _i, _i, _i, _p, _i, _p, _p, _i, _i, _i64, _p, _p]),
    "vgan_mmd_bf3_prepare": (_i, [_p, _i, _i, _i, _p, _p, _i, _p, _p, _i, _p]),
    "vgan_mmd_gram_bf3": (_i, [_p, _p, _i, _p, _i, _p, _p, _i, _i, _p, _p, _i, _i, _p, _p, _i, _i, _i, _p, _i, _i, _p, _i64, _p, _i, _p]),
    "vgan_mmd_gram_bf3_tail_ws_bytes": (_i64, []),
    "vgan_mmd_backward_bf3": (_i, [_p, _p, _i, _p, _p, _i, _i, _p, _i, _i, _i, _i, _p, _i, _p, _p, _i, _i, _i64, _i, _p, _p]),
    "vgan_mmd_backward_bf3_tile": (_i, [_i, _i, _i, _i]),
    "vgan_mmd_backward_bf3_rm": (_i, [_p, _p, _i, _i, _p, _p, _i, _i, _p, _i, _i, _i, _i, _p, _i, _p, _p, _i, _i, _i64, _i, _p, _p, _i, _p]),
    "vgan_mmd_backward_bf3_rm_xx": (_i, [_p, _p, _i, _i, _p, _p, _i, _i, _p, _i, _i, _i, _i, _p, _i, _p, _p, _i, _i, _i64, _p, _p, _p]),
    "vgan_row_sqnorm": (_i, [_p, _i, _p, _i, _i, _p]),
    "vgan_adadelta_step": (_i, [_p, _p, _i, _i64, _p, _p, _i64, _f, _f, _f, _f, _f, _p]),
    "vgan_noise_normal": (_i, [_p, _i, _i, _i, _i, _u64, _p, _u64, _p]),
    "vgan_homogeneous_pack": (_i, [_p, _i, _i, _i, _p]),
    "vgan_adadelta_step_packed": (_i, [_p, _p, _p, _p, _p, _p, _i64, _f, _f, _f, _f, _f, _p, _i, _i, _i, _i, _u64, _p, _p]),
    "vgan_gemm_grouped": (_i, [_p, _i, _p]),
    "vgan_gemm_grouped_ex": (_i, [_p, _i, _p, _p]),
    "vgan_mask_project_forward_bf3": (_i, [_p, _i, _p, _i, _p, _p, _i, _i, _p, _p, _i, _p, _p, _p, _i, _p, _p, _i, _i, _i, _p, _i, _p, _p, _p]),
    "vgan_mse_grad": (_i, [_p, _i, _p, _i, _i, _i, _f, _p, _p, _i, _p]),
    "vgan_sum_f64": (_i, [_p, _i, ctypes.c_double, _p, _i, _p]),
    "vgan_rbf_kernel_matrix": (_i, [_p, _i, _i, _i, _p, _f, _p, _i, _p]),
    "vgan_rbf_multi_kernel_matrix": (_i, [_p, _i, _i, _i, _p, _p, _p, _i, _p, _i, _p, _i, _p]),
    "vgan_rows_dot": (_i, [_p, _i, _p, _i, _p, _i, _i, _p]),
    "vgan_shuffle_epoch": (_i, [_p, _i64, _i64, _u64, _u64, _p]),
    "vgan_shuffle_index": (_i64, [_i64, _i64, _u64, _u64]),
    "vgan_mask_unique": (_i, [_p, _i, _i, _i, _p, _p, _p, _p, _p]),
    "vgan_dp_unique_id": (_i, [_p]),
    "vgan_dp_comm_create": (_i, [_p, _i, _p, _i]),
    "vgan_dp_allreduce_sum": (_i, [_p, _p, _i64, _p]),
    "vgan_dp_allgather": (_i, [_p, _p, _i64, _p]),
    "vgan_dp_comm_destroy": (_i, [_p]),
    "vgan_mse": (_i, [_p, _i, _p, _i, _i, _i, _f, _p, _i, _p]),
    "vgan_outlier_pack": (_i, [_p, _i, _i, _i, _p, _p, _p, _p, _i, _i, _p, _p, _p]),
    "vgan_outlier_knn": (_i, [_p, _p, _i, _p, _p, _i, _p, _p, _i, _i, _i, _i, _i, _i, _p, _p, _p, _p]),
    "vgan_outlier_refine": (_i, [_p, _i, _i, _p, _i, _i, _i, _p, _p, _i, _i, _p, _i, _p, _p, _p, _p]),
    "vgan_outlier_score": (_i, [_p, _p, _i, _i, _i, _i, _p, _p, _i, _p, _p, _i, _p, _p]),
    "vgan_outlier_kde": (_i, [_p, _p, _i, _p, _p, _i, _p, _p, _i, _i, _p, _i, _i, _i, _p, _p, _p, _p, _i, _p]),
    "vgan_outlier_combine": (_i, [_p, _i, _i, _i, _p, _p, _p]),
    "vgan_outlier_abod": (_i, [_p, _i, _i, _p, _i, _i, _i, _p, _p, _i, _i, _p, _i, _p, _p, _i, _p]),
    "vgan_outlier_abod_floor": (_i, [_p, _i, _i, _i, _i, _p, _p, _p]),
    "vgan_outlier_score_stats_ws_bytes": (_i64, [_i, _i, _i]),
    "vgan_outlier_score_stats": (_i, [_p, _i, _i, _i, _i, _p, _p, _p, _i64, _p]),
    "vgan_outlier_combine_normalized": (_i, [_p, _i, _i, _i, _p, _p, _p, _i, _p, _p]),
    "vgan_cluster_lloyd_ws_bytes": (_i64, [_i, _i, _i, _i]),
    "vgan_cluster_image": (_i, [_p, _i, _p, _p, _p, _i, _i, _p, _p, _p, _p]),
    "vgan_cluster_lloyd": (_i, [_p, _p, _p, _i, _i, _i, _p, _p, _p, _i, _i, _i, _i, _i, _i, _p, _p, _p, _p, _p, _p, _p, _p, _p,
                                _p, _i64, _i, _p]),
    "vgan_cluster_final": (_i, [_p, _i, _i, _i, _p, _p, _i, _i, _p, _p, _p, _i, _p, _p, _p, _p, _p, _i, _p]),
}

ABI_VERSION = 11
_lib = None


class VganHipError(RuntimeError):
    pass


def load():
    global _lib
    if _lib is not None:
        return _lib
    if not os.path.exists(LIB_PATH):
        raise VganHipError(
            f"{LIB_PATH} is missing: build it with `python -c 'import __graft_entry__ as g; g.build()'` "
            "(or `make -C v-gan_amd/csrc`).  vgan_amd has no CPU fallback.")
    lib = ctypes.CDLL(LIB_PATH)
    for name, (res, args) in SIGNATURES.items():
        fn = getattr(lib, name)
        fn.restype = res
        fn.argtypes = args
    if lib.vgan_abi_version() != ABI_VERSION:
        raise VganHipError(f"ABI mismatch: library {lib.vgan_abi_version()} vs binding {ABI_VERSION}")
    _lib = lib
    return lib


def check(rc, what=""):
    if rc != 0:
        msg = load().vgan_last_error().decode(errors="replace")
        raise VganHipError(f"{what} failed (code {rc}): {msg}")


def build_tiles(n, grad_mode, rank=0, world=1, tile=64):
    lib = load()
    cnt = lib.vgan_mmd_build_tiles(n, grad_mode, rank, world, tile, None, 0)
    if cnt < 0:
        raise VganHipError("vgan_mmd_build_tiles: " + lib.vgan_last_error().decode())
    buf = (ctypes.c_int32 * (cnt * 8))()
    got = lib.vgan_mmd_build_tiles(n, grad_mode, rank, world, tile, ctypes.cast(buf, ctypes.c_void_p), cnt)
    if got != cnt:
        raise VganHipError("vgan_mmd_build_tiles: inconsistent tile count")
    return list(buf), cnt


def split_tiles(table, tile=64, yy_last=False):
    import torch
    lib = load()
    slot = table[:, 4] & 3
    first = (slot != 2) if yy_last else (slot != 0)
    parts = []
    for keep in (first, ~first):
        sub = table[keep].contiguous()
        if sub.shape[0] > 1:
            buf = (ctypes.c_int32 * sub.numel())(*sub.reshape(-1).tolist())
            if lib.vgan_mmd_order_tiles(ctypes.cast(buf, ctypes.c_void_p), sub.shape[0], tile) != 0:
                raise VganHipError("vgan_mmd_order_tiles: " + lib.vgan_last_error().decode())
            sub = torch.tensor(list(buf), dtype=torch.int32).view(-1, 8)
        parts.append(sub)
    return parts
```

v-gan_amd/ops.py:

```python
import ctypes

import torch

from . import lib as _lib

_f32 = torch.float32


def _round4(v):
    return (int(v) + 3) // 4 * 4


def _ptr(t):
    return ctypes.c_void_p(t.data_ptr()) if t is not None else None


def _mat(t, name):
    if not (t.is_cuda and t.dtype == _f32 and t.dim() == 2 and t.stride(1) == 1):
        raise ValueError(f"{name}: need a float32 HIP matrix with unit inner stride, got "
                         f"{t.dtype} {tuple(t.shape)} strides {t.stride()} on {t.device}")
    return t


def _vec(t, name, dtype=_f32):
    if not (t.is_cuda and t.dtype == dtype and t.is_contiguous()):
        raise ValueError(f"{name}: need a contiguous {dtype} HIP tensor, got {t.dtype} on {t.device}")
    return t


class HipOps:

    name = "hip"

    def __init__(self):
        self.lib = _lib.load()
        if not torch.cuda.is_available():
            raise _lib.VganHipError("vgan_amd needs a HIP device (torch.cuda.is_available() is False); "
                                    "there is no CPU fallback")

    @staticmethod
    def _stream():
        return ctypes.c_void_p(torch.cuda.current_stream().cuda_stream)

    def build_tiles(self, n, grad_mode, rank=0, world=1, device=None, tile=64, split_xx=False, split=None):
        flat, cnt = _lib.build_tiles(n, grad_mode, rank, world, tile)
        table = torch.tensor(flat, dtype=torch.int32).view(cnt, 8)
        if split_xx or split:
            first, second = _lib.split_tiles(table, tile, yy_last=(split == "yy_last"))
            return torch.cat([first, second]).to(device or "cuda"), first.shape[0]
        return table.to(device or "cuda")

    def colmax_chunks(self, n):
        return self.lib.vgan_colmax_chunks(n)

    def linear_forward(self, x, W, b, y, x_nslabs=1, x_slab_stride=0):
        _mat(x, "x"), _mat(W, "W"), _mat(y, "y")
        n, kin = x.shape
        out = W.shape[0]
        assert W.shape[1] == kin and y.shape == (n, out)
        _lib.check(self.lib.vgan_linear_forward(_ptr(x), x.stride(0), int(x_nslabs), int(x_slab_stride), _ptr(W), W.stride(0),
                                                _ptr(b), _ptr(y), y.stride(0), n, kin, out, self._stream()), "vgan_linear_forward")

    def linear_backward_input(self, dy, W, dx):
        _mat(dy, "dy"), _mat(W, "W"), _mat(dx, "dx")
        n, out = dy.shape
        kin = W.shape[1]
        assert W.shape[0] == out and dx.shape == (n, kin)
        _lib.check(self.lib.vgan_linear_backward_input(_ptr(dy), dy.stride(0), _ptr(W), W.stride(0), _ptr(dx), dx.stride(0),
                                                       n, kin, out, self._stream()), "vgan_linear_backward_input")

    def linear_backward_params(self, dy, x, dW, db, splits=1, slab_stride=0, x_nslabs=1, x_slab_stride=0):
        _mat(dy, "dy"), _mat(x, "x"), _mat(dW, "dW")
        n, out = dy.shape
        kin = x.shape[1]
        assert x.shape[0] == n and dW.shape == (out, kin)
        _lib.check(self.lib.vgan_linear_backward_params(_ptr(dy), dy.stride(0), _ptr(x), x.stride(0), int(x_nslabs), int(x_slab_stride),
                                                        _ptr(dW), dW.stride(0), _ptr(db), n, kin, out, int(splits), int(slab_stride),
                                                        self._stream()), "vgan_linear_backward_params")

    def linear_backward_params_xx_supported(self, n, kin, out):
        return bool(self.lib.vgan_linear_backward_params_xx_supported(int(n), int(kin), int(out)))

    def linear_backward_params_xx(self, dy, x, dW, xx):
        _mat(dy, "dy"), _mat(x, "x"), _mat(dW, "dW")
        n, out = dy.shape
        kin = x.shape[1]
        assert x.shape[0] == n and dW.shape == (out, kin)
        _lib.check(self.lib.vgan_linear_backward_params_xx(_ptr(dy), dy.stride(0), _ptr(x), x.stride(0), _ptr(dW), dW.stride(0), n, kin, out,
                                                           ctypes.byref(xx), self._stream()), "vgan_linear_backward_params_xx")

    def reduce_slabs(self, src, slab_stride, nslabs, dst):
        _vec(dst, "dst")
        _lib.check(self.lib.vgan_reduce_slabs(_ptr(src), int(slab_stride), int(nslabs), _ptr(dst), dst.numel(), self._stream()),
                   "vgan_reduce_slabs")

    def col_mean(self, data, out):
        _mat(data, "data"), _vec(out, "out")
        rows, d = data.shape
        assert out.numel() >= d
        _lib.check(self.lib.vgan_col_mean(_ptr(data), data.stride(0), rows, d, _ptr(out), self._stream()), "vgan_col_mean")

    @staticmethod
    def logits_chain(za, At4):
        _mat(za, "za"), _mat(At4, "At4")
        assert za.shape[1] == At4.shape[1]
        return _lib.LogitsChain(_ptr(za), _ptr(At4), za.stride(0), At4.stride(0), za.shape[1], 0)

    @staticmethod
    def chain_fusable(n, d, *lds):
        return d % 4 == 0 and d <= 1024 and all(int(v) % 4 == 0 for v in lds)

    def mask_project_forward(self, logits, data, rows, S, U, Zx, Zy, sqx, sqy, row_cursor=None, row_batches=1, row_stride=0,
                             row_offset=0, center=None, norm_split=False, chain=None):
        _mat(data, "data"), _mat(Zy, "Zy"), _mat(S, "S")
        n, d = S.shape
        if logits is not None:
            _mat(logits, "logits")
            assert tuple(logits.shape) == (n, d)
        assert S.is_contiguous() and S.shape == (n, d) and (U is None or (U.is_contiguous() and U.shape == (n, d)))
        assert Zx is None or Zx.stride(0) == Zy.stride(0)
        if rows is not None:
            _vec(rows, "rows", torch.int32)
        _lib.check(self.lib.vgan_mask_project_forward(_ptr(logits), logits.stride(0) if logits is not None else 0, _ptr(data), data.stride(0), _ptr(rows),
                                                      _ptr(row_cursor), int(row_batches), int(row_stride), int(row_offset), _ptr(S), _ptr(U), _ptr(Zx), _ptr(Zy), Zy.stride(0), _ptr(sqx), _ptr(sqy),
                                                      n, d, _ptr(center), int(bool(norm_split)),
                                                      ctypes.byref(chain) if chain is not None else None, self._stream()), "vgan_mask_project_forward")

    def xx_job(self, Dh, Dl, dsq, tiles, bw, partial):
        assert tiles.is_contiguous() and partial.is_contiguous() and Dh.stride(0) == Dl.stride(0)
        return _lib.XXJob(_ptr(Dh), _ptr(Dl), _ptr(dsq), _ptr(tiles), _ptr(bw), _ptr(partial), Dh.stride(0), tiles.shape[0])

    def mask_project_forward_bf3(self, logits, data, rows, S, Z, sq, Zh, Zl, ZTh, ZTl, row_cursor=None, row_batches=1, row_stride=0,
                                 center=None, write_x=True, xx=None, chain=None):
        _mat(data, "data"), _mat(Z, "Z"), _mat(S, "S")
        n, d = S.shape
        if logits is not None:
            _mat(logits, "logits")
        _lib.check(self.lib.vgan_mask_project_forward_bf3(_ptr(logits), logits.stride(0) if logits is not None else 0, _ptr(data), data.stride(0), _ptr(rows),
                                                          _ptr(row_cursor), int(row_batches), int(row_stride), _ptr(S), _ptr(Z), Z.stride(0),
                                                          _ptr(sq), _ptr(Zh), _ptr(Zl), Zh.stride(0), _ptr(ZTh), _ptr(ZTl),
                                                          ZTh.stride(0) if ZTh is not None else 0,
                                                          n, d, _ptr(center), int(bool(write_x)),
                                                          ctypes.byref(xx) if xx is not None else None,
                                                          ctypes.byref(chain) if chain is not None else None, self._stream()),
                   "vgan_mask_project_forward_bf3")

    @staticmethod
    def bf3_fusable(n, d, *lds):
        return d % 4 == 0 and d <= 1024 and n % 8 == 0 and all(int(v) % 4 == 0 for v in lds)

    def gather_rows(self, data, rows, out, sq, row_cursor=None, row_batches=1, row_stride=0, row_offset=0):
        _mat(data, "data"), _mat(out, "out")
        n, d = out.shape[0], data.shape[1]
        _lib.check(self.lib.vgan_gather_rows(_ptr(data), data.stride(0), _ptr(rows), _ptr(row_cursor), int(row_batches),
                                             int(row_stride), int(row_offset), _ptr(out), out.stride(0), _ptr(sq), n, d,
                                             self._stream()), "vgan_gather_rows")

    def gather_rows_split(self, data, rows, center, out, sq, norm_split=False, Zh=None, Zl=None, row_cursor=None, row_batches=1,
                          row_stride=0, row_offset=0, n=None):
        _mat(data, "data")
        d = data.shape[1]
        n = int(n if n is not None else (out.shape[0] if out is not None else sq.numel()))
        _lib.check(self.lib.vgan_gather_rows_split(_ptr(data), data.stride(0), _ptr(rows), _ptr(row_cursor), int(row_batches),
                                                   int(row_stride), int(row_offset), _ptr(center), _ptr(out),
                                                   out.stride(0) if out is not None else 0, _ptr(sq), int(bool(norm_split)), _ptr(Zh),
                                                   _ptr(Zl), Zh.stride(0) if Zh is not None else 0, n, d, self._stream()),
                   "vgan_gather_rows_split")

    def upper_softmax_forward(self, logits, S, U):
        _mat(logits, "logits")
        n, d = logits.shape
        assert S.is_contiguous() and (U is None or U.is_contiguous())
        _lib.check(self.lib.vgan_upper_softmax_forward(_ptr(logits), logits.stride(0), _ptr(S), _ptr(U), n, d, self._stream()),
                   "vgan_upper_softmax_forward")

    def mask_backward(self, gU, S, colkey, pen_weight, row_offset, dlogits, nslabs=1, slab_stride=0):
        _mat(gU, "gU"), _mat(S, "S"), _mat(dlogits, "dlogits")
        n, d = S.shape
        _lib.check(self.lib.vgan_mask_backward(_ptr(gU), gU.stride(0), int(nslabs), int(slab_stride), _ptr(S), S.stride(0),
                                               _ptr(colkey), float(pen_weight),
                                               int(row_offset), _ptr(dlogits), dlogits.stride(0), n, d, self._stream()),
                   "vgan_mask_backward")

    def colmax(self, S, row_offset, part, colkey, from_softmax=True):
        _mat(S, "S")
        n, d = S.shape
        assert part.dtype == torch.int64 and colkey.dtype == torch.int64 and part.numel() >= self.colmax_chunks(n) * d
        _lib.check(self.lib.vgan_colmax(_ptr(S), S.stride(0), int(bool(from_softmax)), int(row_offset), _ptr(part), _ptr(colkey), n, d, self._stream()),
                   "vgan_colmax")

    def colmax_partial(self, S, row_offset, part, from_softmax=True):
        _mat(S, "S")
        n, d = S.shape
        assert part.dtype == torch.int64 and part.numel() >= self.colmax_chunks(n) * d
        _lib.check(self.lib.vgan_colmax_partial(_ptr(S), S.stride(0), int(bool(from_softmax)), int(row_offset), _ptr(part), n, d,
                                                self._stream()), "vgan_colmax_partial")

    def mmd_finalize(self, partial, tiles, colpart, chunks, colkey, n, d, weight, stats, loss, loss_accum=None, accum_scale=1.0,
                     step_counter=None):
        _lib.check(self.lib.vgan_mmd_finalize(_ptr(partial), _ptr(tiles), tiles.shape[0], _ptr(colpart), int(chunks), _ptr(colkey),
                                              int(n), int(d), float(weight), _ptr(stats), _ptr(loss), _ptr(loss_accum),
                                              float(accum_scale), _ptr(step_counter), self._stream()), "vgan_mmd_finalize")

    def finalize_job(self, partial, tiles, colpart, chunks, colkey, n, d, weight, stats, loss, loss_accum=None, accum_scale=1.0,
                     step_counter=None, mode=0, ntiles_main=0):
        return _lib.FinalizeJob(_ptr(partial), _ptr(tiles), _ptr(colpart), _ptr(colkey), _ptr(stats), _ptr(loss), _ptr(loss_accum),
                                _ptr(step_counter), tiles.shape[0], int(chunks), int(n), int(d), float(weight), float(accum_scale),
                                int(mode), int(ntiles_main))

    def mask_from_softmax(self, S, U):
        _mat(S, "S"), _mat(U, "U")
        n, d = S.shape
        _lib.check(self.lib.vgan_mask_from_softmax(_ptr(S), S.stride(0), _ptr(U), U.stride(0), n, d, self._stream()),
                   "vgan_mask_from_softmax")

    def row_sqnorm(self, Z, sq, p):
        _mat(Z, "Z")
        _lib.check(self.lib.vgan_row_sqnorm(_ptr(Z), Z.stride(0), _ptr(sq), Z.shape[0], int(p), self._stream()), "vgan_row_sqnorm")

    def mmd_gram(self, Z, sq, n, p, bw, tiles, calibrate, Wg, wrow0, partial):
        _mat(Z, "Z")
        assert (calibrate or Z.shape[0] >= 2 * n) and tiles.dtype == torch.int32 and tiles.is_contiguous()
        ntiles = tiles.shape[0]
        assert partial.numel() >= 4 * ntiles
        ldw = Wg.stride(0) if Wg is not None else 0
        _lib.check(self.lib.vgan_mmd_gram(_ptr(Z), Z.stride(0), _ptr(sq), int(n), int(p), _ptr(bw), _ptr(tiles), ntiles,
                                          int(bool(calibrate)), _ptr(Wg), ldw, int(wrow0), _ptr(partial), self._stream()),
                   "vgan_mmd_gram")

    @staticmethod
    def _mults(multipliers):
        vals = [float(v) for v in multipliers]
        return (ctypes.c_float * len(vals))(*vals), len(vals)

    def mmd_gram_general(self, Z, sq, n, p, bw, tiles, multipliers, Wg, wrow0, partial):
        _mat(Z, "Z")
        ntiles = tiles.shape[0]
        assert partial.numel() >= 4 * ntiles
        arr, nk = self._mults(multipliers)
        ldw = Wg.stride(0) if Wg is not None else 0
        _lib.check(self.lib.vgan_mmd_gram_general(_ptr(Z), Z.stride(0), _ptr(sq), int(n), int(p), _ptr(bw), _ptr(tiles), ntiles, arr, nk,
                                                  _ptr(Wg), ldw, int(wrow0), _ptr(partial), self._stream()), "vgan_mmd_gram_general")

    def rbf_multi_kernel_matrix(self, Z, sq, bw, multipliers, K, dK=None):
        _mat(Z, "Z"), _mat(K, "K")
        m, p = Z.shape
        arr, nk = self._mults(multipliers)
        _lib.check(self.lib.vgan_rbf_multi_kernel_matrix(_ptr(Z), Z.stride(0), m, p, _ptr(sq), _ptr(bw), arr, nk, _ptr(K), K.stride(0),
                                                         _ptr(dK), dK.stride(0) if dK is not None else 0, self._stream()),
                   "vgan_rbf_multi_kernel_matrix")

    def mmd_gram_colmax(self, Z, sq, n, p, bw, tiles, Wg, wrow0, partial, S, row_offset, colpart, from_softmax=True):
        _mat(Z, "Z"), _mat(S, "S")
        ntiles = tiles.shape[0]
        nrows, d = S.shape
        assert partial.numel() >= 4 * ntiles and colpart.dtype == torch.int64 and colpart.numel() >= self.colmax_chunks(nrows) * d
        ldw = Wg.stride(0) if Wg is not None else 0
        _lib.check(self.lib.vgan_mmd_gram_colmax(_ptr(Z), Z.stride(0), _ptr(sq), int(n), int(p), _ptr(bw), _ptr(tiles), ntiles,
                                                 _ptr(Wg), ldw, int(wrow0), _ptr(partial), _ptr(S), S.stride(0),
                                                 int(bool(from_softmax)), int(row_offset), _ptr(colpart), nrows, d, self._stream()),
                   "vgan_mmd_gram_colmax")

    def mmd_reduce(self, partial, tiles, stats, zero_first=True):
        assert stats.dtype == torch.float64 and stats.numel() >= 4
        _lib.check(self.lib.vgan_mmd_reduce(_ptr(partial), _ptr(tiles), tiles.shape[0], _ptr(stats), int(bool(zero_first)),
                                            self._stream()), "vgan_mmd_reduce")

    def mmd_set_bandwidth(self, stats, n, bw):
        _lib.check(self.lib.vgan_mmd_set_bandwidth(_ptr(stats), int(n), _ptr(bw), self._stream()), "vgan_mmd_set_bandwidth")

    def mmd_loss(self, stats, colkey, n, d, weight, loss, loss_accum=None, accum_scale=1.0, step_counter=None):
        _lib.check(self.lib.vgan_mmd_loss(_ptr(stats), _ptr(colkey), int(n), int(d), float(weight), _ptr(loss), _ptr(loss_accum),
                                          float(accum_scale), _ptr(step_counter), self._stream()), "vgan_mmd_loss")

    def mmd_backward(self, Wg, Z, wrow0, nr, ncols, p, mul, out, splits=1, slab_stride=0, finalize=None, mul_shift=None):
        _mat(Wg, "Wg"), _mat(Z, "Z"), _mat(out, "out")
        ldmul = mul.stride(0) if mul is not None else 0
        _lib.check(self.lib.vgan_mmd_backward(_ptr(Wg), Wg.stride(0), _ptr(Z), Z.stride(0), int(wrow0), int(nr), int(ncols), int(p),
                                              _ptr(mul), ldmul, _ptr(mul_shift), _ptr(out), out.stride(0), int(splits), int(slab_stride),
                                              ctypes.byref(finalize) if finalize is not None else None, self._stream()),
                   "vgan_mmd_backward")

    def mmd_bf3_prepare(self, Z, rows, p, Zh, Zl, ZTh=None, ZTl=None):
        _mat(Z, "Z")
        for t in (Zh, Zl, ZTh, ZTl):
            assert t is None or (t.dtype == torch.int16 and t.is_cuda and t.stride(1) == 1)
        kn = ZTh.stride(0) if ZTh is not None else 0
        _lib.check(self.lib.vgan_mmd_bf3_prepare(_ptr(Z), Z.stride(0), int(rows), int(p), _ptr(Zh), _ptr(Zl), Zh.stride(0),
                                                 _ptr(ZTh), _ptr(ZTl), kn, self._stream()), "vgan_mmd_bf3_prepare")

    def gram_tail_workspace(self, device):
        return torch.zeros(int(self.lib.vgan_mmd_gram_bf3_tail_ws_bytes()) // 4, dtype=torch.int32, device=device)

    def mmd_gram_bf3(self, Zh, Zl, sq, n, bw, tiles, Wh, Wl, wrow0, partial, S=None, row_offset=0, colpart=None, from_softmax=True,
                     tile=64, tail_ws=None, rs_part=None):
        ntiles = tiles.shape[0]
        nrows, d = (S.shape if S is not None else (0, 0))
        ldw = Wh.stride(0) if Wh is not None else 0
        _lib.check(self.lib.vgan_mmd_gram_bf3(_ptr(Zh), _ptr(Zl), Zh.stride(0), _ptr(sq), int(n), _ptr(bw), _ptr(tiles), ntiles,
                                              int(tile), _ptr(Wh), _ptr(Wl), ldw, int(wrow0), _ptr(partial), _ptr(S),
                                              S.stride(0) if S is not None else 0, int(bool(from_softmax)), int(row_offset),
                                              _ptr(colpart), nrows, d, _ptr(tail_ws), tail_ws.numel() * 4 if tail_ws is not None else 0,
                                              _ptr(rs_part), rs_part.stride(0) if rs_part is not None else 0, self._stream()),
                   "vgan_mmd_gram_bf3")

    def mmd_backward_bf3(self, Wh, Wl, ZTh, ZTl, Z, wrow0, nr, p, mul, out, splits=1, slab_stride=0, finalize=None, mul_shift=None,
                         tile=0):
        _mat(Z, "Z"), _mat(out, "out")
        ldmul = mul.stride(0) if mul is not None else 0
        _lib.check(self.lib.vgan_mmd_backward_bf3(_ptr(Wh), _ptr(Wl), Wh.stride(0), _ptr(ZTh), _ptr(ZTl), ZTh.stride(0),
                                                  ZTh.shape[0], _ptr(Z), Z.stride(0), int(wrow0), int(nr), int(p), _ptr(mul), ldmul,
                                                  _ptr(mul_shift), _ptr(out), out.stride(0), int(splits), int(slab_stride), int(tile),
                                                  ctypes.byref(finalize) if finalize is not None else None, self._stream()),
                   "vgan_mmd_backward_bf3")

    def mmd_backward_bf3_rm(self, Wh, Wl, Zh, Zl, zrows, Z, wrow0, nr, p, mul, out, splits=1, slab_stride=0, finalize=None, mul_shift=None,
                            tile=0, xx=None, rs_part=None):
        _mat(Z, "Z"), _mat(out, "out")
        ldmul = mul.stride(0) if mul is not None else 0
        kn = (int(zrows) + 63) // 64 * 64
        assert Wh.stride(0) >= kn and Zh.shape[0] >= zrows
        if xx is not None:
            assert tile in (0, 64)
            _lib.check(self.lib.vgan_mmd_backward_bf3_rm_xx(_ptr(Wh), _ptr(Wl), Wh.stride(0), kn, _ptr(Zh), _ptr(Zl), Zh.stride(0), int(zrows),
                                                            _ptr(Z), Z.stride(0), int(wrow0), int(nr), int(p), _ptr(mul), ldmul, _ptr(mul_shift),
                                                            _ptr(out), out.stride(0), int(splits), int(slab_stride),
                                                            ctypes.byref(finalize) if finalize is not None else None, ctypes.byref(xx),
                                                            self._stream()), "vgan_mmd_backward_bf3_rm_xx")
            return
        _lib.check(self.lib.vgan_mmd_backward_bf3_rm(_ptr(Wh), _ptr(Wl), Wh.stride(0), kn, _ptr(Zh), _ptr(Zl), Zh.stride(0), int(zrows),
                                                     _ptr(Z), Z.stride(0), int(wrow0), int(nr), int(p), _ptr(mul), ldmul, _ptr(mul_shift),
                                                     _ptr(out), out.stride(0), int(splits), int(slab_stride), int(tile),
                                                     ctypes.byref(finalize) if finalize is not None else None, _ptr(rs_part),
                                                     rs_part.stride(0) if rs_part is not None else 0, self._stream()),
                   "vgan_mmd_backward_bf3_rm")

    def mmd_backward_bf3_tile(self, nr, p, splits=1, tile=0):
        return int(self.lib.vgan_mmd_backward_bf3_tile(int(nr), int(p), int(splits), int(tile)))

    def gemm_grouped(self, problems, copy=None, adadelta=None, noise=None, fold=None):
        assert 1 <= len(problems) <= _lib.GEMM_MAX_GROUP
        arr = (_lib.GemmProblem * len(problems))()
        for q, (kind, A, B, C, *rest) in zip(arr, problems):
            if kind == "NT2":
                D, scratch = rest
                _mat(A, "A"), _mat(B, "B"), _mat(C, "C"), _mat(D, "D")
                (m, k), (k2, kb), (n, k2d) = A.shape, B.shape, D.shape
                assert k == kb and k2 == k2d and tuple(C.shape) == (m, n)
                tiles = ((m + 63) // 64) * ((n + 63) // 64)
                assert scratch.is_cuda and scratch.dtype == _f32 and scratch.is_contiguous() and scratch.numel() >= tiles * 64 * _round4(k2)
                q.a, q.b, q.c, q.d, q.scratch = A.data_ptr(), B.data_ptr(), C.data_ptr(), D.data_ptr(), scratch.data_ptr()
                q.kind, q.m, q.n, q.k, q.k2, q.splitk = _lib.GEMM_NT_NT, m, n, k, k2, 1
                q.lda, q.ldb, q.ldc, q.ldd = A.stride(0), B.stride(0), C.stride(0), D.stride(0)
                continue
            q.splitk = int(rest[0]) if rest else 1
            if q.splitk > 1:
                assert C.dim() == 3 and C.shape[0] == q.splitk and C.is_contiguous()
                C = C[0]
            _mat(A, "A"), _mat(B, "B"), _mat(C, "C")
            if kind == "NN":
                (m, k), (k2, n), code = A.shape, B.shape, _lib.GEMM_NN
            elif kind == "NT":
                (m, k), (n, k2), code = A.shape, B.shape, _lib.GEMM_NT
            elif kind == "TN":
                (k, m), (k2, n), code = A.shape, B.shape, _lib.GEMM_TN
            else:
                raise ValueError(kind)
            assert k == k2 and tuple(C.shape) == (m, n), (kind, tuple(A.shape), tuple(B.shape), tuple(C.shape))
            q.a, q.b, q.c, q.kind, q.m, q.n, q.k = A.data_ptr(), B.data_ptr(), C.data_ptr(), code, m, n, k
            q.lda, q.ldb, q.ldc = A.stride(0), B.stride(0), C.stride(0)
        if copy is None and adadelta is None and noise is None and fold is None:
            _lib.check(self.lib.vgan_gemm_grouped(arr, len(problems), self._stream()), "vgan_gemm_grouped")
            return
        x = _lib.GroupedExtras()
        if copy is not None:
            src, dst = copy
            _vec(src, "copy src"), _vec(dst, "copy dst")
            assert src.numel() == dst.numel()
            x.copy_src, x.copy_dst, x.copy_count = src.data_ptr(), dst.data_ptr(), src.numel()
        if adadelta is not None:
            a = adadelta
            for nm in ("p", "sq", "acc"):
                _vec(a[nm], nm)
            x.adadelta, x.p, x.sq_avg, x.acc_delta = 1, a["p"].data_ptr(), a["sq"].data_ptr(), a["acc"].data_ptr()
            x.lr, x.rho, x.eps, x.weight_decay, x.grad_scale = (float(a["lr"]), float(a.get("rho", 0.9)), float(a.get("eps", 1e-6)),
                                                                float(a.get("weight_decay", 0.0)), float(a.get("grad_scale", 1.0)))
            extra = a.get("extra_grad")
            assert len(a["layers"]) == len(problems) + (1 if extra is not None else 0)
            for L, (w, off_w, off_b, out, inp) in zip(x.layer, a["layers"]):
                _mat(w, "w_packed")
                L.w_packed, L.off_w, L.off_b, L.ldp, L.out, L.inp = w.data_ptr(), int(off_w), int(off_b), w.stride(0), int(out), int(inp)
            if extra is not None:
                _mat(extra, "extra_grad")
                x.g_extra, x.ld_extra = extra.data_ptr(), extra.stride(0)
        if noise is not None:
            z = noise["next_noise"]
            x.next_noise, x.noise_rows, x.noise_ld = z.data_ptr(), z.shape[0], z.stride(0)
            x.noise_cols, x.noise_ones_col = int(noise["noise_cols"]), int(noise["noise_ones_col"])
            x.seed, x.step_counter = int(noise["seed"]) & 0xFFFFFFFFFFFFFFFF, noise["step_counter"].data_ptr()
        if fold is not None:
            x.fold = ctypes.addressof(fold)
        _lib.check(self.lib.vgan_gemm_grouped_ex(arr, len(problems), ctypes.byref(x), self._stream()), "vgan_gemm_grouped_ex")

    def mse_grad(self, target, pred, gscale, part, g):
        _mat(target, "target"), _mat(pred, "pred"), _mat(g, "g")
        n, d = pred.shape
        assert part.dtype == torch.float64 and part.numel() >= (n + 3) // 4
        _lib.check(self.lib.vgan_mse_grad(_ptr(target), target.stride(0), _ptr(pred), pred.stride(0), n, d, float(gscale), _ptr(part),
                                          _ptr(g), g.stride(0), self._stream()), "vgan_mse_grad")

    def sum_f64(self, src, count, scale, out, accumulate=False):
        assert src.dtype == torch.float64
        _lib.check(self.lib.vgan_sum_f64(_ptr(src), int(count), float(scale), _ptr(out), int(bool(accumulate)), self._stream()),
                   "vgan_sum_f64")

    def rbf_kernel_matrix(self, Z, sq, alpha, K):
        _mat(Z, "Z"), _mat(K, "K")
        m, p = Z.shape
        _lib.check(self.lib.vgan_rbf_kernel_matrix(_ptr(Z), Z.stride(0), m, p, _ptr(sq), float(alpha), _ptr(K), K.stride(0),
                                                   self._stream()), "vgan_rbf_kernel_matrix")

    def rows_dot(self, A, B, out, broadcast_b=False):
        _mat(A, "A")
        rows, cols = A.shape
        assert out.dtype == torch.float64 and out.numel() >= rows
        ldb = 0 if broadcast_b else B.stride(0)
        _lib.check(self.lib.vgan_rows_dot(_ptr(A), A.stride(0), _ptr(B), ldb, _ptr(out), rows, cols, self._stream()), "vgan_rows_dot")

    def dp_unique_id(self):
        buf = (ctypes.c_uint8 * 128)()
        _lib.check(self.lib.vgan_dp_unique_id(ctypes.cast(buf, ctypes.c_void_p)), "vgan_dp_unique_id")
        return bytes(buf)

    def dp_comm_create(self, nranks, unique_id, rank):
        comm = ctypes.c_void_p()
        buf = (ctypes.c_uint8 * 128).from_buffer_copy(unique_id)
        _lib.check(self.lib.vgan_dp_comm_create(ctypes.byref(comm), int(nranks), ctypes.cast(buf, ctypes.c_void_p), int(rank)),
                   "vgan_dp_comm_create")
        return comm

    def dp_allreduce_sum(self, comm, t):
        _vec(t, "t")
        _lib.check(self.lib.vgan_dp_allreduce_sum(comm, _ptr(t), t.numel(), self._stream()), "vgan_dp_allreduce_sum")

    def dp_allgather(self, comm, t, nranks):
        assert t.is_cuda and t.is_contiguous() and t.shape[0] % nranks == 0
        _lib.check(self.lib.vgan_dp_allgather(comm, _ptr(t), t.numel() * t.element_size() // nranks, self._stream()), "vgan_dp_allgather")

    def dp_comm_destroy(self, comm):
        _lib.check(self.lib.vgan_dp_comm_destroy(comm), "vgan_dp_comm_destroy")

    def shuffle_epoch(self, perm, train_size, seed, epoch):
        _vec(perm, "perm", torch.int32)
        _lib.check(self.lib.vgan_shuffle_epoch(_ptr(perm), perm.numel(), int(train_size), int(seed) & 0xFFFFFFFFFFFFFFFF,
                                               int(epoch) & 0xFFFFFFFFFFFFFFFF, self._stream()), "vgan_shuffle_epoch")

    def shuffle_index(self, i, train_size, seed, epoch):
        return int(self.lib.vgan_shuffle_index(int(i), int(train_size), int(seed) & 0xFFFFFFFFFFFFFFFF, int(epoch) & 0xFFFFFFFFFFFFFFFF))

    def mask_unique(self, masks):
        assert masks.is_cuda and masks.dtype == torch.bool and masks.dim() == 2
        m8 = masks.contiguous().view(torch.uint8)
        n, d = m8.shape
        dev = masks.device
        keys = torch.empty(n * ((d + 63) // 64), dtype=torch.int64, device=dev)
        work = torch.empty(2 * n, dtype=torch.int32, device=dev)
        out_row = torch.zeros(n, dtype=torch.int32, device=dev)
        out_count = torch.zeros(n, dtype=torch.int32, device=dev)
        _lib.check(self.lib.vgan_mask_unique(_ptr(m8), m8.stride(0), n, d, _ptr(keys), _ptr(work), _ptr(out_row), _ptr(out_count),
                                             self._stream()), "vgan_mask_unique")
        cnt = out_count.cpu()
        m = int((cnt > 0).sum())
        return masks[out_row[:m].long()], cnt[:m].to(torch.int64)

    def adadelta_step(self, p, g, sq, acc, lr, rho=0.9, eps=1e-6, weight_decay=0.0, grad_scale=1.0, nslabs=1, slab_stride=0):
        for t, nm in ((p, "p"), (sq, "sq"), (acc, "acc")):
            _vec(t, nm)
        _lib.check(self.lib.vgan_adadelta_step(_ptr(p), _ptr(g), int(nslabs), int(slab_stride), _ptr(sq), _ptr(acc), p.numel(),
                                               float(lr), float(rho), float(eps),
                                               float(weight_decay), float(grad_scale), self._stream()), "vgan_adadelta_step")

    def adadelta_step_packed(self, p, pmap, g_packed, w_packed, sq, acc, lr, rho=0.9, eps=1e-6, weight_decay=0.0, grad_scale=1.0,
                             next_noise=None, noise_cols=0, noise_ones_col=-1, seed=0, step_counter=None):
        for t, nm in ((p, "p"), (sq, "sq"), (acc, "acc"), (g_packed, "g_packed"), (w_packed, "w_packed")):
            _vec(t, nm)
        _vec(pmap, "pmap", torch.int32)
        assert pmap.numel() == p.numel()
        zr, zld = (next_noise.shape[0], next_noise.stride(0)) if next_noise is not None else (0, 0)
# ... 180 lines not shown
```

v-gan_amd/trainer.py:

```python
import os

import torch

ADADELTA_RHO = 0.9
ADADELTA_EPS = 1e-6


def _round4(v):
    return (v + 3) // 4 * 4


def _launch_rounds(tiles, slots, can_split):
    if tiles <= 0:
        return 0.0
    full, r = divmod(tiles, slots)
    if r == 0:
        return float(full)
    x = r / slots
    last = 0.55 if x <= 0.5 else 0.55 + 0.9 * (x - 0.5)
    if can_split and x <= 0.125:
        last = 0.25
    elif can_split and x <= 0.25:
        last = 0.4
    elif can_split and x <= 0.5:
# ... 104 lines not shown
            self.acts_own = [a[self.lo:self.lo + nl] for a in self.acts]
            self.dacts = [None] + [torch.zeros(nl, w, **f32) for w in self.widths[1:4]]
        else:
            e = self.e
            poff = [0]
            for k in range(1, 5):
                poff.append(poff[-1] + e[k] * e[k - 1])
            self.Wt_all = torch.zeros(poff[-1], **f32)
            self.Gt_all = torch.zeros(poff[-1], **f32)
            self.Wt = [None] + [self.Wt_all[poff[k - 1]:poff[k]].view(e[k], e[k - 1]) for k in range(1, 5)]
            self.Gt = [None] + [self.Gt_all[poff[k - 1]:poff[k]].view(e[k], e[k - 1]) for k in range(1, 5)]
            self.At = [None, self.Wt[1]] + [torch.zeros(e[k], e[0], **f32) for k in range(2, 5)]
            self.M = [None, self.Gt[1]] + [torch.zeros(e[k], e[0], **f32) for k in range(2, 5)]
            self.B3 = torch.zeros(e[4], e[2], **f32)
            self.B2 = torch.zeros(e[4], e[1], **f32)
            self.At1s = torch.zeros(e[1], e[0], **f32)
            want_assoc = chain_assoc or os.environ.get("VGAN_CHAIN_ASSOC", "auto")
            if want_assoc not in ("auto", "depth", "flops"):
                raise ValueError(f"chain_assoc must be 'auto', 'depth' or 'flops', got {want_assoc!r}")
            self.chain_flops = want_assoc == "flops" or (want_assoc == "auto" and 2.0 * e[4] * e[3] * e[2] >= 1e9)
            if self.chain_flops:
                self.fuse_update = False
                def split_of(m, n_, k):
                    t64 = ((m + 63) // 64) * ((n_ + 63) // 64)
                    return 1 if 2.0 * m * n_ * k < 2.5e8 else max(1, min(8, 1024 // t64, k // 256))
                self.fwd_split = {k: split_of(e[k], e[0], e[k - 1]) for k in (2, 3, 4)}
                self.bwd_split = {k: split_of(e[k - 1], e[0], e[k]) for k in (4, 3, 2)}
                if os.environ.get("VGAN_CHAIN_SPLITK", "1") != "1":
                    self.fwd_split, self.bwd_split = {k: 1 for k in (2, 3, 4)}, {k: 1 for k in (4, 3, 2)}
                need = max([self.fwd_split[k] * e[k] * e[0] for k in (2, 3, 4)] + [self.bwd_split[k] * e[k - 1] * e[0] for k in (4, 3, 2)])
                self.chain_ws = torch.zeros(need, **f32)
            pmap = torch.full((self.fp.total,), -1, dtype=torch.int32)
            for k in range(1, 5):
                wk, wk1 = self.widths[k], self.widths[k - 1]
                r = torch.arange(wk, dtype=torch.int32)[:, None] * e[k - 1]
                ow, ob = self.fp.offsets[2 * (k - 1)], self.fp.offsets[2 * (k - 1) + 1]
                pmap[ow:ow + wk * wk1] = (poff[k - 1] + r + torch.arange(wk1, dtype=torch.int32)[None, :]).reshape(-1)
                pmap[ob:ob + wk] = (poff[k - 1] + r + wk1).reshape(-1)
            self.pmap = pmap.to(self.dev)
            self.pack_layers = [(self.W[k - 1], self.b[k - 1], self.Wt[k]) for k in range(1, 5)]
            self.unpack_layers = [(self.fp.view(self.fp.grad, 2 * (k - 1)), self.fp.view(self.fp.grad, 2 * (k - 1) + 1), self.Gt[k])
                                  for k in range(1, 5)]
            ops.homogeneous_pack(self.pack_layers, unpack=False)

        self.precision = mmd_precision or os.environ.get("VGAN_MMD_PRECISION", "auto")
        if self.precision not in ("auto", "fp32", "bf16x3"):
            raise ValueError(f"mmd_precision must be 'auto', 'fp32' or 'bf16x3', got {self.precision!r}")
        if self.precision == "auto":
            self.precision = "bf16x3" if 2 * n * d >= (1 << 20) else "fp32"
        self.bf3 = self.precision == "bf16x3"
        self.center = torch.zeros(dp, **f32)
        if center_operand:
            ops.col_mean(data, self.center)
        self.bwd_tile = int(os.environ.get("VGAN_BWD_TILE", "0"))
        self._fin = None
        self.S = torch.zeros(n, d, **f32)
        self.S_own = self.S[self.lo:self.lo + nl]
        self.Z = torch.zeros(2 * n, dp, **f32)
        self.sqn = torch.zeros(2 * n, **f32)
        self.sq_cal = torch.zeros(2 * n, **f32) if self.bf3 else self.sqn
        self.Wg = torch.zeros(nl, 2 * n, **f32)
        out_tiles = ((nl + 63) // 64) * ((d + 63) // 64)
        auto_splits = max(2 if self.bf3 else 1, min(4, 256 // max(out_tiles, 1), max(1, (2 * n) // 64)))
        rm = self.front_sharded or os.environ.get("VGAN_BWD_OPERAND", "rowmajor") != "transposed"
        if self.bf3 and rm and self.bwd_tile in (0, 256) and ops.mmd_backward_bf3_tile(nl, d, 1, self.bwd_tile) == 256:
            auto_splits = 1
        self.bsplits = max(1, int(os.environ.get("VGAN_BWD_SPLITS", str(auto_splits))))
        self.gU_slabs = torch.zeros(self.bsplits, nl, dp, **f32)
        self.gU = self.gU_slabs[0]
        self.dlogits_pad = torch.zeros(nl, dp, **f32)
        self.dlogits = self.dlogits_pad[:, :d]
        self.rm_backward = True
        if self.precision == "bf16x3":
            i16 = dict(dtype=torch.int16, device=self.dev)
            self.kp, self.kn = (d + 63) // 64 * 64, (2 * n + 63) // 64 * 64
            self.Zh, self.Zl = torch.zeros(2 * n, self.kp, **i16), torch.zeros(2 * n, self.kp, **i16)
            self.rm_backward = self.front_sharded or os.environ.get("VGAN_BWD_OPERAND", "rowmajor") != "transposed"
            if self.rm_backward:
                self.ZTh = self.ZTl = None
            else:
                self.ZTh, self.ZTl = torch.zeros(self.kp, self.kn, **i16), torch.zeros(self.kp, self.kn, **i16)
            self.Wh, self.Wl = torch.zeros(nl, self.kn, **i16), torch.zeros(nl, self.kn, **i16)
        self.fused_prepare = (self.bf3 and not self.front_sharded and ops.bf3_fusable(n, d, self.logits.stride(0), data.stride(0), dp) and
                              os.environ.get("VGAN_FUSED_PREPARE", "1") == "1")
        self.chain_in_mask = (self.mode == "collapsed" and not self.front_sharded and ops.chain_fusable(n, d, data.stride(0), dp) and
                              (not self.bf3 or self.fused_prepare) and os.environ.get("VGAN_CHAIN_IN_MASK", "0") == "1")
        self._chain = None
        self.two_stage_logits = (self.mode == "collapsed" and not self.chain_flops and not self.chain_in_mask and not self.front_sharded and
                                 os.environ.get("VGAN_LOGITS_2STAGE", "0") == "1")
        if self.two_stage_logits:
            e2 = self.e[2]
            self.T = torch.zeros(n, e2, **f32)
            self.T_ws = torch.zeros(((n + 63) // 64) * ((e2 + 63) // 64) * 64 * _round4(self.e[1]), **f32)
        self.perm = torch.zeros(self.nb, n, dtype=torch.int32, device=self.dev)
        self.perm_next = torch.zeros_like(self.perm)
        self.epoch_staged = False
        self.gram_tile = 64
        want = os.environ.get("VGAN_GRAM_TILE", "auto")
        if self.bf3 and nl % 128 == 0 and want in ("auto", "128"):
            if want == "128" or len(ops.build_tiles(n, 1, rank, world, device=self.dev, tile=128)) >= 512:
                self.gram_tile = 128
        if self.bf3 and nl % 256 == 0 and want in ("auto", "256"):
            if want == "256" or len(ops.build_tiles(n, 1, rank, world, device=self.dev, tile=256)) >= 512:
                self.gram_tile = 256
        self.gram_tail_ws = (ops.gram_tail_workspace(self.dev)
                             if self.gram_tile == 256 and os.environ.get("VGAN_GRAM_TAIL", "1") != "0" else None)
        self.rs_part = None
        if (self.gram_tile == 256 and self.rm_backward and n % 128 == 0 and os.environ.get("VGAN_RS_FROM_GRAM", "1") != "0"
                and ops.mmd_backward_bf3_tile(nl, d, self.bsplits, self.bwd_tile) == 256):
            self.rs_part = torch.zeros((2 * n + 127) // 128, nl, **f32)
        if overlap_exchange is None and os.environ.get("VGAN_OVERLAP") is not None:
            overlap_exchange = {"1": True, "0": False}.get(os.environ["VGAN_OVERLAP"], os.environ["VGAN_OVERLAP"])
        self.overlap = False if overlap_exchange is None else bool(overlap_exchange)
        if self.front_sharded and self.overlap:
            raise ValueError("overlap_exchange and front='sharded' are two schedules of the same exchange: choose one")
        self._side = torch.cuda.Stream(device=self.dev) if (self.overlap and data.is_cuda and overlap_exchange != "serial") else None
        self.x_ahead = self.overlap and (not self.bf3 or self.rm_backward)
        self.xx_ride = False
        self._xx = None
        if (self.fused_prepare and self.gram_tile == 64 and not self.overlap and self.rm_backward and
                os.environ.get("VGAN_XX_RIDE", "0") == "1"):
            split, n_main = ops.build_tiles(n, 1, rank, world, device=self.dev, tile=64, split_xx=True)
            xx_tiles = split.shape[0] - n_main
            self.xx_ride = xx_tiles > 0 and 8 * ((n // 8 + 7) // 8) + xx_tiles <= 512
        if self.xx_ride:
            i16 = dict(dtype=torch.int16, device=self.dev)
            rows_total = data.shape[0]
            self.Dh, self.Dl = torch.zeros(rows_total, self.kp, **i16), torch.zeros(rows_total, self.kp, **i16)
            self.dsq = torch.zeros(rows_total, **f32)
            ops.gather_rows_split(data, None, self.center, None, self.dsq, True, self.Dh, self.Dl, n=rows_total)
        self.xx_in_m4 = (self.bf3 and self.mode == "collapsed" and self.gram_tile == 64 and not self.overlap and not self.xx_ride and
                         not self.front_sharded and
                         ops.linear_backward_params_xx_supported(nl, self.e[0], dp) and os.environ.get("VGAN_XX_IN_M4", "1") == "1")
        self._xx_m4 = self._fold = None
        if self.front_sharded:
            self.tiles, self.n_main = ops.build_tiles(n, 1, rank, world, device=self.dev, tile=self.gram_tile, split="yy_last")
            slots = 256 if self.gram_tile >= 128 else (512 if self.bf3 else 1024)
            self.n_main = _best_boundary(self.n_main, self.tiles.shape[0], slots, self.gram_tail_ws is not None)
        elif self.overlap or self.xx_ride or self.xx_in_m4:
            self.tiles, self.n_main = ops.build_tiles(n, 1, rank, world, device=self.dev, tile=self.gram_tile, split_xx=True)
            if self.xx_in_m4:
                slots = int(os.environ.get("VGAN_GRAM_SLOTS", "512"))
                self.n_main = min(self.tiles.shape[0], max(self.n_main, slots))
                if self.n_main == self.tiles.shape[0]:
                    self.xx_in_m4 = False
        else:
            self.tiles = ops.build_tiles(n, 1, rank, world, device=self.dev, tile=self.gram_tile)
            self.n_main = self.tiles.shape[0]
        self.xx_late_in_backward = False
        if self.xx_in_m4 and self.rm_backward and os.environ.get("VGAN_XX_LATE", "backward") == "backward":
            late = self.tiles.shape[0] - self.n_main
            bwd_wgs = ((d + 63) // 64) * ((nl + 63) // 64) * self.bsplits + 1
            self.xx_late_in_backward = (ops.mmd_backward_bf3_tile(nl, d, self.bsplits, self.bwd_tile) == 64 and late <= 512 - bwd_wgs)
        self.tiles_cal = self.tiles if (world == 1 and self.gram_tile == 64 and not (self.overlap or self.xx_ride or self.xx_in_m4 or self.front_sharded)) else ops.build_tiles(n, 0, 0, 1, device=self.dev)
        self.partial = torch.zeros(max(self.tiles.shape[0], self.tiles_cal.shape[0]), 4, **f32)
        self.stats = torch.zeros(4, dtype=torch.float64, device=self.dev)
        self.bw = torch.zeros(1, **f32)
        self.has_bw = False
        self.loss = torch.zeros(1, **f32)
        self.loss_accum = torch.zeros(1, **f32)
        self._hist, self._hist_n, self._hist_events = None, 0, []
        self._read_stream, self._loss_host = None, None
        self.accum_scale = (1.0 / self.nb) if loss_accum_scale is None else float(loss_accum_scale)
        self.step_counter = torch.zeros(1, dtype=torch.int64, device=self.dev)
        self.col_chunks = (world * ops.colmax_chunks(nl)) if self.front_sharded else ops.colmax_chunks(n)
        self.colpart = torch.zeros(self.col_chunks * d, dtype=torch.int64, device=self.dev)
        own = ops.colmax_chunks(nl) * d
        self.colpart_own = self.colpart[rank * own:(rank + 1) * own] if self.front_sharded else self.colpart
        self.colkey = torch.zeros(d, dtype=torch.int64, device=self.dev)
        if self.front_sharded and data.is_cuda and self._collect().is_initialized():
            self._coalesce = self._probe_coalescing(self._collect())

    def set_epoch_batches(self, idx):
        if os.environ.get("VGAN_FEED_DIRECT") == "1":
            self.perm.copy_(idx.to(dtype=torch.int32), non_blocking=True)
            self._after_new_epoch_table()
            return
        self.stage_epoch_batches(idx)
        self.begin_epoch()

    def stage_epoch_batches(self, idx):
        self.perm_next.copy_(idx.to(dtype=torch.int32).view(self.nb, self.n), non_blocking=True)
        self.epoch_staged = True

    def begin_epoch(self):
        if not self.epoch_staged:
            raise RuntimeError("begin_epoch without a staged table (stage_epoch_batches)")
        self.perm.copy_(self.perm_next)
        self.epoch_staged = False
        self._after_new_epoch_table()

    def _after_new_epoch_table(self):
        if self.overlap and self.has_bw:
            self._prefetch_xx()

    def _prefetch_xx(self):
        self._prefetch_x_operand()
        self._xx_tiles()
        self._xx_primed = True

    def _prefetch_x_operand(self):
        ops, n = self.ops, self.n
        rowsel = dict(row_cursor=self.step_counter, row_batches=self.nb, row_stride=n)
        if self.bf3:
            ops.gather_rows_split(self.data, self.perm, self.center, self.Z[:n], self.sqn[:n], True, self.Zh[:n], self.Zl[:n], **rowsel)
        else:
            ops.gather_rows_split(self.data, self.perm, self.center, self.Z[:n], self.sqn[:n], False, **rowsel)

    def _xx_tiles(self):
        ops, n = self.ops, self.n
        ntx = self.tiles.shape[0] - self.n_main
        if ntx == 0:
            return
        tx, px = self.tiles[self.n_main:], self.partial[self.n_main:self.n_main + ntx]
        if self.bf3:
            ops.mmd_gram_bf3(self.Zh, self.Zl, self.sqn, n, self.bw, tx, None, None, 0, px, tile=self.gram_tile)
        else:
            ops.mmd_gram(self.Z, self.sqn, n, self.dp, self.bw, tx, False, None, 0, px)

    def _fork_prefetch(self):
        if not self.overlap:
            return
        if self._side is None:
            self._prefetch_xx()
            return
        self._side.wait_stream(torch.cuda.current_stream())
        with torch.cuda.stream(self._side):
            self._prefetch_xx()

    def _join_prefetch(self):
        if self.overlap and self._side is not None:
            torch.cuda.current_stream().wait_stream(self._side)

    def shuffle_epoch(self, epoch):
        self.ops.shuffle_epoch(self.perm, self.data.shape[0], self.seed, int(epoch))
        self._after_new_epoch_table()

    def set_bandwidth(self, value):
        self.bw.fill_(float(value))
        self.has_bw = True

    def set_noise(self, z):
        self.za[:, :self.L].copy_(z.to(dtype=torch.float32), non_blocking=True)

    def epoch_loss(self):
        v = float(self._sum_over_ranks(self.loss_accum).item())
        self.loss_accum.zero_()
        return v

    def close_epoch(self):
        if self._hist is None or self._hist_n == self._hist.numel():
            grown = torch.zeros(max(64, 2 * self._hist_n), dtype=torch.float32, device=self.dev)
            if self._hist is not None:
                grown[:self._hist_n].copy_(self._hist)
            self._hist = grown
        slot = self._hist_n
        cell = self._hist[slot:slot + 1]
        cell.copy_(self.loss_accum)
        self.loss_accum.zero_()
        if self.exchange:
            self._collect().all_reduce(cell, group=self.group)
        ev = None
        if self.data.is_cuda:
            ev = torch.cuda.Event()
            ev.record()
        self._hist_events.append(ev)
        self._hist_n += 1
        return slot

    def read_epoch_loss(self, slot):
        ev = self._hist_events[slot]
        if ev is None:
            return float(self._hist[slot])
        if self._read_stream is None:
            self._read_stream = torch.cuda.Stream(self.dev)
            self._loss_host = torch.zeros(1, dtype=torch.float32).pin_memory()
        self._read_stream.wait_event(ev)
        with torch.cuda.stream(self._read_stream):
            self._loss_host.copy_(self._hist[slot:slot + 1], non_blocking=True)
        self._read_stream.synchronize()
        return float(self._loss_host[0])

    def step_loss(self):
        return float(self._sum_over_ranks(self.loss).item())

    def _sum_over_ranks(self, t):
        if not self.exchange:
            return t
        t = t.clone()
        self._collect().all_reduce(t, group=self.group)
        return t

    def grad_view(self, k):
        if self.mode == "collapsed":
            self.ops.homogeneous_pack(self.unpack_layers, unpack=True)
        elif not self.exchange and self.splits > 1:
            return sum(self.fp.view(self.gslab[sl], k) for sl in range(self.splits))
        return self.fp.view(self.fp.grad, k)

    def _generator_forward(self, own_rows=False):
        ops = self.ops
        if self.mode == "layered":
            for k in range(4):
                ops.linear_forward(self.acts[k], self.W[k], self.b[k], self.acts[k + 1])
            return
        Wt, At = self.Wt, self.At
        if self.chain_flops:
            for k in (2, 3, 4):
                sp = self.fwd_split[k]
                if sp > 1:
                    ops.gemm_grouped([("NN", Wt[k], At[k - 1], self._slabs(sp, At[k]), sp)])
                    ops.reduce_slabs(self.chain_ws, At[k].numel(), sp, At[k])
                else:
                    ops.gemm_grouped([("NN", Wt[k], At[k - 1], At[k])])
        elif self.two_stage_logits:
            ops.gemm_grouped([("NN", Wt[2], At[1], At[2]), ("NN", Wt[4], Wt[3], self.B3), ("NT2", self.za, Wt[1], self.T, Wt[2], self.T_ws)])
            ops.gemm_grouped([("NN", Wt[3], At[2], At[3]), ("NN", self.B3, Wt[2], self.B2), ("NT", self.T, self.B3[:self.d], self.logits)])
            return
        else:
            ops.gemm_grouped([("NN", Wt[2], At[1], At[2]), ("NN", Wt[4], Wt[3], self.B3)])
            ops.gemm_grouped([("NN", Wt[3], At[2], At[3]), ("NN", self.B3, At[2], At[4]), ("NN", self.B3, Wt[2], self.B2)])
        if own_rows:
            ops.linear_forward(self.z_own, At[4][:self.d], None, self.logits[self.lo:self.lo + self.nl])
        elif not self.chain_in_mask:
            ops.linear_forward(self.za, At[4][:self.d], None, self.logits)

    def _slabs(self, splits, like):
        return self.chain_ws[:splits * like.numel()].view(splits, like.shape[0], like.shape[1])

    def _generator_backward_update(self, dist):
        ops = self.ops
        adadelta = dict(lr=self.lr, rho=ADADELTA_RHO, eps=ADADELTA_EPS, weight_decay=self.wd, grad_scale=1.0)
        if self.mode == "layered":
            g = self.dlogits
            for k in (3, 2, 1, 0):
                ops.linear_backward_params(g, self.acts_own[k], self.dW[k], self.db[k], self.splits, self.fp.total)
                if k:
                    ops.linear_backward_input(g, self.W[k], self.dacts[k])
                    g = self.dacts[k]
            if dist:
                if self.splits > 1:
                    ops.reduce_slabs(self.gslab, self.fp.total, self.splits, self.fp.grad)
                dist.all_reduce(self.fp.grad, group=self.group)
                ops.adadelta_step(self.fp.flat, self.fp.grad, self.fp.sq, self.fp.acc, **adadelta)
            elif self.splits > 1:
                ops.adadelta_step(self.fp.flat, self.gslab[0], self.fp.sq, self.fp.acc, nslabs=self.splits, slab_stride=self.fp.total,
                                  **adadelta)
            else:
                ops.adadelta_step(self.fp.flat, self.fp.grad, self.fp.sq, self.fp.acc, **adadelta)
            return
        e, d = self.e, self.d
        if self.xx_in_m4 and not self.xx_late_in_backward:
            ops.linear_backward_params_xx(self.dlogits_pad, self.z_own, self.M[4][:self.dp], self._late_xx_job())
        else:
            ops.linear_backward_params(self.dlogits_pad, self.z_own, self.M[4][:self.dp], None)
        if dist:
            dist.all_reduce(self.M[4], group=self.group)
        M, Gt, At = self.M, self.Gt, self.At
        fused_noise = dict(next_noise=self.za, noise_cols=self.L, noise_ones_col=self.L, seed=self.seed,
                           step_counter=self.step_counter) if self.noise_mode == "device" else {}
        if self.chain_flops:
            Wt = self.Wt
            for k in (4, 3, 2):
                sp = self.bwd_split[k]
                probs = [("TN", Wt[k], M[k], self._slabs(sp, M[k - 1]), sp) if sp > 1 else ("TN", Wt[k], M[k], M[k - 1])]
                if k < 4:
                    probs.append(("NT", M[k + 1], At[k], Gt[k + 1]))
                ops.gemm_grouped(probs, fold=self._fold if (self.xx_in_m4 and k == 4) else None)
                if sp > 1:
                    ops.reduce_slabs(self.chain_ws, M[k - 1].numel(), sp, M[k - 1])
            ops.gemm_grouped([("NT", M[2], At[1], Gt[2])])
            ops.adadelta_step_packed(self.fp.flat, self.pmap, self.Gt_all, self.Wt_all, self.fp.sq, self.fp.acc, **adadelta, **fused_noise)
            return
        if not self.fuse_update:
            ops.gemm_grouped([("TN", self.Wt[4], M[4], M[3]), ("TN", self.B3, M[4], M[2]), ("TN", self.B2, M[4], M[1])],
                             fold=self._fold if self.xx_in_m4 else None)
            ops.gemm_grouped([("NT", M[4], At[3], Gt[4]), ("NT", M[3], At[2], Gt[3]), ("NT", M[2], At[1], Gt[2])])
            ops.adadelta_step_packed(self.fp.flat, self.pmap, self.Gt_all, self.Wt_all, self.fp.sq, self.fp.acc, **adadelta, **fused_noise)
            return
        ops.gemm_grouped([("TN", self.Wt[4], M[4], M[3]), ("TN", self.B3, M[4], M[2]), ("TN", self.B2, M[4], M[1])],
                         copy=(self.Wt[1], self.At1s), fold=self._fold if self.xx_in_m4 else None)
        w, off = self.widths, self.fp.offsets
        layers = [(self.Wt[k], off[2 * (k - 1)], off[2 * (k - 1) + 1], w[k], w[k - 1]) for k in (4, 3, 2, 1)]
        ops.gemm_grouped([("NT", M[4], At[3], Gt[4]), ("NT", M[3], At[2], Gt[3]), ("NT", M[2], self.At1s, Gt[2])],
                         adadelta=dict(p=self.fp.flat, sq=self.fp.sq, acc=self.fp.acc, layers=layers, extra_grad=Gt[1], **adadelta),
                         noise=fused_noise or None)

    def _collect(self):
        import torch.distributed as dist
        return dist

    def _forward(self):
        ops, n, nl, lo = self.ops, self.n, self.nl, self.lo
        if self.noise_mode == "device" and (self.mode == "layered" or self.steps_done == 0):
            ops.noise_normal(self.za, self.seed, self.step_counter, 0, cols=self.L, ones_col=self.L)
        self._generator_forward()
        rowsel = dict(row_cursor=self.step_counter, row_batches=self.nb, row_stride=n)
        logits = self.logits
        if self.chain_in_mask:
            if self._chain is None:
                self._chain = ops.logits_chain(self.za, self.At[4][:self.d])
            rowsel["chain"] = self._chain
            logits = None
        if self.fused_prepare:
            xx = None
            if self.xx_ride and self.has_bw:
                if self._xx is None:
                    ntx = self.tiles.shape[0] - self.n_main
                    self._xx = ops.xx_job(self.Dh, self.Dl, self.dsq, self.tiles[self.n_main:], self.bw, self.partial[self.n_main:self.n_main + ntx])
                xx = self._xx
            ops.mask_project_forward_bf3(logits, self.data, self.perm, self.S, self.Z, self.sqn, self.Zh, self.Zl, self.ZTh, self.ZTl,
                                         center=self.center, write_x=not self.x_ahead, xx=xx, **rowsel)
            return
        if self.x_ahead:
            ops.mask_project_forward(logits, self.data, self.perm, self.S, None, None, self.Z[n:], None, self.sqn[n:],
                                     row_offset=0, center=self.center, norm_split=self.bf3, **rowsel)
        else:
            ops.mask_project_forward(logits, self.data, self.perm, self.S, None, self.Z[:n], self.Z[n:], self.sqn[:n], self.sqn[n:],
                                     row_offset=0, center=self.center, norm_split=self.bf3, **rowsel)

    def _calibrate(self):
        ops = self.ops
        if self.bf3:
            ops.row_sqnorm(self.Z, self.sq_cal, self.dp)
        ops.mmd_gram(self.Z, self.sq_cal, self.n, self.dp, None, self.tiles_cal, True, None, 0, self.partial)
        ops.mmd_reduce(self.partial, self.tiles_cal, self.stats, True)
        ops.mmd_set_bandwidth(self.stats, self.n, self.bw)
        self.has_bw = True

    def _loss_backward_update(self):
        ops, n, nl, lo, d = self.ops, self.n, self.nl, self.lo, self.d
        dist = self._collect() if self.exchange else None
        gstride = nl * self.dp
        bf3 = self.precision == "bf16x3"
        if bf3 and not self.fused_prepare:
            if self.x_ahead:
                ops.mmd_bf3_prepare(self.Z[n:], n, d, self.Zh[n:], self.Zl[n:])
            else:
                ops.mmd_bf3_prepare(self.Z, 2 * n, d, self.Zh, self.Zl, self.ZTh, self.ZTl)
        if bf3:
            ops.mmd_gram_bf3(self.Zh, self.Zl, self.sqn, n, self.bw, self.tiles[:self.n_main], self.Wh, self.Wl, n + lo, self.partial, self.S, 0,
                             self.colpart, True, tile=self.gram_tile, tail_ws=self.gram_tail_ws, rs_part=self.rs_part)
        else:
            ops.mmd_gram_colmax(self.Z, self.sqn, n, self.dp, self.bw, self.tiles[:self.n_main], self.Wg, n + lo, self.partial, self.S, 0,
                                self.colpart, True)
        if self._fin is None:
            fin_args = (self.partial, self.tiles, self.colpart, ops.colmax_chunks(n), self.colkey, n, d, self.pen if self.rank == 0 else 0.0,
                        self.stats, self.loss, self.loss_accum, self.accum_scale, self.step_counter)
            if self.xx_in_m4:
                self._fin = ops.finalize_job(*fin_args, mode=1, ntiles_main=self.n_main)
                self._fold = ops.finalize_job(*fin_args, mode=2, ntiles_main=self.n_main)
            else:
                self._fin = ops.finalize_job(*fin_args)
        fin = self._fin
        if bf3:
            if self.rm_backward:
                ops.mmd_backward_bf3_rm(self.Wh, self.Wl, self.Zh, self.Zl, 2 * n, self.Z, n + lo, nl, d, self.Z[lo:lo + nl], self.gU,
                                        self.bsplits, gstride, fin, mul_shift=self.center, tile=self.bwd_tile,
                                        xx=self._late_xx_job() if self.xx_late_in_backward else None, rs_part=self.rs_part)
            else:
                ops.mmd_backward_bf3(self.Wh, self.Wl, self.ZTh, self.ZTl, self.Z, n + lo, nl, d, self.Z[lo:lo + nl], self.gU, self.bsplits,
                                     gstride, fin, mul_shift=self.center, tile=self.bwd_tile)
        else:
            ops.mmd_backward(self.Wg, self.Z, n + lo, nl, 2 * n, self.dp, self.Z[lo:lo + nl], self.gU, self.bsplits, gstride, fin,
                             mul_shift=self.center)
        self._fork_prefetch()
        ops.mask_backward(self.gU, self.S_own, self.colkey, self.pen, lo, self.dlogits, self.bsplits, gstride)
        self._generator_backward_update(dist)
        self._join_prefetch()

    def _forward_sharded(self):
        ops, n, nl, lo, d = self.ops, self.n, self.nl, self.lo, self.d
        if self.noise_mode == "device" and self.steps_done == 0:
            ops.noise_normal(self.za, self.seed, self.step_counter, 0, cols=self.L, ones_col=self.L)
        self._generator_forward(own_rows=True)
        rowsel = dict(row_cursor=self.step_counter, row_batches=self.nb, row_stride=n)
        own, yown = slice(lo, lo + nl), slice(n + lo, n + lo + nl)
        if self.bf3:
            ops.gather_rows_split(self.data, self.perm, self.center, None, self.sqn[:n], True, self.Zh[:n], self.Zl[:n], **rowsel)
        else:
            ops.gather_rows_split(self.data, self.perm, self.center, self.Z[:n], self.sqn[:n], False, **rowsel)
        ops.mask_project_forward(self.logits[own], self.data, self.perm, self.S_own, None, self.Z[own] if self.bf3 else None, self.Z[yown],
                                 None, self.sqn[yown], row_offset=lo, center=self.center, norm_split=self.bf3, **rowsel)
        if self.bf3:
            ops.mmd_bf3_prepare(self.Z[yown], nl, d, self.Zh[yown], self.Zl[yown])
        ops.colmax_partial(self.S_own, lo, self.colpart_own)

    def _all_gather(self, dist, out, own):
        size = dist.get_world_size(self.group) if dist.is_initialized() else 1
        if size != self.world:
            out = own
        if own.is_cuda and dist.get_backend(self.group) == "gloo":
            host = out.cpu()
            dist.all_gather_into_tensor(host, own.cpu(), group=self.group)
            out.copy_(host)
            return None
        return dist.all_gather_into_tensor(out, own, group=self.group, async_op=True)

    def _exchange_front(self, dist):
        n, nl, lo = self.n, self.nl, self.lo
        yown = slice(n + lo, n + lo + nl)
        pairs = []
        if self.bf3:
            pairs += [(img[n:2 * n].view(torch.int32), img[yown].view(torch.int32)) for img in (self.Zh, self.Zl)]
        else:
            pairs.append((self.Z[n:], self.Z[yown]))
        pairs += [(self.sqn[n:], self.sqn[yown]), (self.colpart, self.colpart_own)]
        if self._coalesce is None:
            self._coalesce = self._probe_coalescing(dist)
        if self._coalesce:
            emulated = dist.get_world_size(self.group) != self.world
            with dist._coalescing_manager(group=self.group, device=self.dev, async_ops=True) as cm:
                for out, own in pairs:
                    dist.all_gather_into_tensor(own if emulated else out, own, group=self.group)
            return [cm]
        return [self._all_gather(dist, out, own) for out, own in pairs]

    def _probe_coalescing(self, dist):
        if os.environ.get("VGAN_DP_COALESCE", "0") != "1" or not self.data.is_cuda or torch.cuda.is_current_stream_capturing():
            return False
        try:
            if dist.get_backend(self.group) != "nccl" or not hasattr(dist, "_coalescing_manager"):
                return False
            size = dist.get_world_size(self.group)
            a, b = torch.zeros(size * 4, device=self.dev), torch.zeros(size * 2, dtype=torch.int64, device=self.dev)
            r = dist.get_rank(self.group)
            with dist._coalescing_manager(group=self.group, device=self.dev, async_ops=True) as cm:
                dist.all_gather_into_tensor(a, a[4 * r:4 * r + 4], group=self.group)
                dist.all_gather_into_tensor(b, b[2 * r:2 * r + 2], group=self.group)
            cm.wait()
            torch.cuda.synchronize()
            return True
        except Exception as e:
            import warnings
            warnings.warn(f"vgan_amd: coalesced all-gather is not available on this stack ({type(e).__name__}: {e}); one launch per gather")
            return False

    def _loss_backward_update_sharded(self, all_rows_here=False):
        ops, n, nl, lo, d = self.ops, self.n, self.nl, self.lo, self.d
        dist = self._collect()
        works = []
        if all_rows_here:
            if self.bf3:
                ops.mmd_bf3_prepare(self.Z, 2 * n, d, self.Zh, self.Zl)
            self.colpart.zero_()
            ops.colmax_partial(self.S, 0, self.colpart[:ops.colmax_chunks(n) * d])
        else:
            works = self._exchange_front(dist)
        na = self.n_main

        def gram(t0, t1):
            if t1 <= t0:
                return
            if self.bf3:
                ops.mmd_gram_bf3(self.Zh, self.Zl, self.sqn, n, self.bw, self.tiles[t0:t1], self.Wh, self.Wl, n + lo, self.partial[t0:t1],
                                 tile=self.gram_tile, tail_ws=self.gram_tail_ws, rs_part=self.rs_part)
            else:
                ops.mmd_gram(self.Z, self.sqn, n, self.dp, self.bw, self.tiles[t0:t1], False, self.Wg, n + lo, self.partial[t0:t1])

        gram(0, na)
        for w in works:
            if w is not None:
                w.wait()
        gram(na, self.tiles.shape[0])
        if self._fin is None:
            self._fin = ops.finalize_job(self.partial, self.tiles, self.colpart, self.col_chunks, self.colkey, n, d,
                                         self.pen if self.rank == 0 else 0.0, self.stats, self.loss, self.loss_accum, self.accum_scale,
                                         self.step_counter)
        gstride = nl * self.dp
        if self.bf3:
            ops.mmd_backward_bf3_rm(self.Wh, self.Wl, self.Zh, self.Zl, 2 * n, self.Z, n + lo, nl, d, self.Z[lo:lo + nl], self.gU,
                                    self.bsplits, gstride, self._fin, mul_shift=self.center, tile=self.bwd_tile, rs_part=self.rs_part)
        else:
            ops.mmd_backward(self.Wg, self.Z, n + lo, nl, 2 * n, self.dp, self.Z[lo:lo + nl], self.gU, self.bsplits, gstride, self._fin,
                             mul_shift=self.center)
        ops.mask_backward(self.gU, self.S_own, self.colkey, self.pen, lo, self.dlogits, self.bsplits, gstride)
        self._generator_backward_update(dist)

    def _late_xx_job(self):
        if self._xx_m4 is None:
            ntx = self.tiles.shape[0] - self.n_main
            self._xx_m4 = self.ops.xx_job(self.Zh, self.Zl, self.sqn, self.tiles[self.n_main:], self.bw,
                                          self.partial[self.n_main:self.n_main + ntx])
        return self._xx_m4

    def _step_body(self):
        if self.front_sharded:
            self._forward_sharded()
            self._loss_backward_update_sharded()
        else:
            self._forward()
            self._loss_backward_update()

    def step(self):
        if not self.has_bw:
            if self.overlap:
                self._prefetch_x_operand()
            self._forward()
            self._calibrate()
            if self.overlap or self.xx_ride:
                self._xx_tiles()
                self._xx_primed = True
            if self.front_sharded:
                self._loss_backward_update_sharded(all_rows_here=True)
            else:
                self._loss_backward_update()
        elif self.use_graph and self.steps_done > 0:
            if self.graph is None:
                self._capture()
# ... 70 lines not shown
```

Baseline: 9801 steps/s.

## Skip fp32 Z writes; rebuild projected values in backward from data, S and row index

The forward mask/project kernel can now skip writing the fp32 Z matrix (both the centred x and the projected y rows) once a bandwidth is set, and instead records the source row index per sample. The bf3 row-major backward kernel gains a REBUILD variant that reloads S, the raw data row and the centre, then recomputes the masked projection and centred x in registers. This is meant to cut global memory traffic, about 2*n*d floats written in forward and read back in backward. In exchange the backward does extra gathers and arithmetic, and the transposed ZTh/ZTl buffers are no longer produced on this path.

```diff
diff --git a/include/vgan_hip.h b/include/vgan_hip.h
--- a/include/vgan_hip.h
+++ b/include/vgan_hip.h
@@ -136,6 +136,18 @@
                                 int p, const float* mul, int ldmul, const float* mul_shift, float* out, int ldo,
                                 int splits, int64_t slab_stride, const vgan_finalize_job* finalize,
                                 const struct vgan_xx_job* xx, vgan_stream_t stream);
+typedef struct vgan_bwd_rebuild {
+    const float* data;
+    const int32_t* xrow;
+    const float* S;
+    const float* center;
+    int32_t ldd, lds;
+} vgan_bwd_rebuild;
+int vgan_mmd_backward_bf3_rm_rebuild(const uint16_t* Wh, const uint16_t* Wl, int ldw, int kn, const uint16_t* Zh,
+                                     const uint16_t* Zl, int kp, int zrows, int nr, int p,
+                                     const vgan_bwd_rebuild* rebuild, float* out, int ldo, int splits,
+                                     int64_t slab_stride, const vgan_finalize_job* finalize,
+                                     const struct vgan_xx_job* xx, vgan_stream_t stream);
 #define VGAN_GEMM_MAX_GROUP 4
 #define VGAN_GEMM_NN 0
 #define VGAN_GEMM_NT 1
@@ -191,6 +203,12 @@
                                   int ldz, float* sq, uint16_t* Zh, uint16_t* Zl, int kp, uint16_t* ZTh,
                                   uint16_t* ZTl, int kn, int n, int d, const float* center, int write_x,
                                   const vgan_xx_job* xx, const vgan_logits_chain* chain, vgan_stream_t stream);
+int vgan_mask_project_forward_bf3_ex(const float* logits, int ldl, const float* data, int ldd, const int32_t* rows,
+                                     const uint64_t* row_cursor, int row_batches, int row_stride, float* S, float* Z,
+                                     int ldz, float* sq, uint16_t* Zh, uint16_t* Zl, int kp, uint16_t* ZTh,
+                                     uint16_t* ZTl, int kn, int n, int d, const float* center, int write_x,
+                                     const vgan_xx_job* xx, const vgan_logits_chain* chain, int write_z, int32_t* xrow,
+                                     vgan_stream_t stream);
 int vgan_row_sqnorm(const float* Z, int ldz, float* sq, int rows, int p, vgan_stream_t stream);
 
 int vgan_adadelta_step(float* p, const float* g, int nslabs, int64_t slab_stride, float* sq_avg,
diff --git a/v-gan_amd/csrc/mmd_bf16.hip b/v-gan_amd/csrc/mmd_bf16.hip
--- a/v-gan_amd/csrc/mmd_bf16.hip
+++ b/v-gan_amd/csrc/mmd_bf16.hip
@@ -472,7 +472,15 @@
             make_float4(((red[0] + red[1]) + (red[2] + red[3])) + ((red[4] + red[5]) + (red[6] + red[7])), 0.f, 0.f, 0.f);
 }
 
-template <int BK, bool RM>
+struct BwdRebuild {
+    const float* data;
+    const int* xrow;
+    const float* S;
+    const float* center;
+    int ldd, lds;
+};
+
+template <int BK, bool RM, bool REBUILD>
 __global__ __launch_bounds__(kBlock, BK == 64 ? 2 : 3) void mmd_backward_bf3_kernel(const unsigned short* __restrict__ Wh, const unsigned short* __restrict__ Wl,
                                                                     int ldw, const unsigned short* __restrict__ ZTh,
                                                                     const unsigned short* __restrict__ ZTl, int kn, int ldb, int brows,
@@ -480,7 +488,7 @@
                                                                     int ptiles, const float* __restrict__ mul, int ldmul,
                                                                     const float* __restrict__ mul_shift, float* __restrict__ out, int ldo,
                                                                     int kchunk, long slab_stride, vgan_finalize_job job, int nfin,
-                                                                    XXJob xx) {
+                                                                    XXJob xx, BwdRebuild rb) {
     using G = GemmBF3<BK>;
     constexpr int kBytes = (RM ? G::kLdsBytesT : G::kLdsBytes) > G::kLdsBytes ? (RM ? G::kLdsBytesT : G::kLdsBytes) : G::kLdsBytes;
     __shared__ __attribute__((aligned(16))) char lds[kBytes];
@@ -508,12 +516,23 @@
     out += blockIdx.y * slab_stride;
     const int col = n0 + G::sub_col(), colc = min(col, p - 1);
     float z_pre[16], m_pre[16];
-    const float mshift = mul_shift != nullptr ? mul_shift[colc] : 0.f;
-#pragma unroll
-    for (int r = 0; r < 16; ++r) {
-        const int rowc = min(m0 + G::sub_row(r), nr - 1);
-        z_pre[r] = Z[(long)(wrow0 + rowc) * ldz + colc];
-        m_pre[r] = mul != nullptr ? mul[(long)rowc * ldmul + colc] + mshift : 1.f;
+    float mshift;
+    if constexpr (REBUILD) {
+        mshift = rb.center[colc];
+#pragma unroll
+        for (int r = 0; r < 16; ++r) {
+            const int rowc = min(m0 + G::sub_row(r), nr - 1);
+            z_pre[r] = rb.S[(long)rowc * rb.lds + colc];
+            m_pre[r] = rb.data[(long)rb.xrow[rowc] * rb.ldd + colc];
+        }
+    } else {
+        mshift = mul_shift != nullptr ? mul_shift[colc] : 0.f;
+#pragma unroll
+        for (int r = 0; r < 16; ++r) {
+            const int rowc = min(m0 + G::sub_row(r), nr - 1);
+            z_pre[r] = Z[(long)(wrow0 + rowc) * ldz + colc];
+            m_pre[r] = mul != nullptr ? mul[(long)rowc * ldmul + colc] + mshift : 1.f;
+        }
     }
     if (klen > 0) {
         if constexpr (RM)
@@ -523,6 +542,15 @@
             G::template run<true>(Wh + k0, Wl + k0, ldw, ZTh + k0, ZTl + k0, ldb, m0, n0, nr, gx * 64, klen, lds, rs, acc);
     }
     if (col >= p) return;
+    if constexpr (REBUILD) {
+        const float tau = 1.0f / (float)p;
+#pragma unroll
+        for (int r = 0; r < 16; ++r) {
+            const float x = m_pre[r];
+            z_pre[r] = project_centred(upper_mask(z_pre[r], tau), x, mshift);
+            m_pre[r] = uncentred_x(centred_x(x, mshift), mshift);
+        }
+    }
 #pragma unroll
     for (int r = 0; r < 16; ++r) {
         const int lrow = G::sub_row(r), row = m0 + lrow;
@@ -752,9 +780,16 @@
                                int zrows, const float* Z, int ldz, int wrow0, int nr, int p, const float* mul, int ldmul,
                                const float* mul_shift, float* out, int ldo, int splits, int64_t slab_stride, int tile,
                                const vgan_finalize_job* finalize, vgan_stream_t stream, const vgan_xx_job* xxjob = nullptr,
-                               const float* rs_part = nullptr, int ldrs = 0) {
-    VGAN_CHECK_ARG(Wh && Wl && Bh && Bl && Z && out && nr > 0 && p > 0 && kn > 0 && kn % 64 == 0 && kp >= p && kp % 64 == 0);
-    VGAN_CHECK_ARG(ldw >= kn && ldz >= p && ldo >= p && (mul == nullptr || ldmul >= p) && wrow0 >= 0);
+                               const float* rs_part = nullptr, int ldrs = 0, const vgan_bwd_rebuild* rebuild = nullptr) {
+    VGAN_CHECK_ARG(Wh && Wl && Bh && Bl && (Z || rebuild) && out && nr > 0 && p > 0 && kn > 0 && kn % 64 == 0 && kp >= p && kp % 64 == 0);
+    VGAN_CHECK_ARG(ldw >= kn && (rebuild || ldz >= p) && ldo >= p && (mul == nullptr || ldmul >= p) && wrow0 >= 0);
+    BwdRebuild rb{};
+    if (rebuild != nullptr) {
+        const vgan_bwd_rebuild& q = *rebuild;
+        VGAN_CHECK_ARG(rm && tile == 64 && q.data && q.xrow && q.S && q.center && q.ldd >= p && q.lds >= p && Z == nullptr && mul == nullptr &&
+                       mul_shift == nullptr);
+        rb = BwdRebuild{q.data, q.xrow, q.S, q.center, q.ldd, q.lds};
+    }
     VGAN_CHECK_ARG(aligned16(Wh) && aligned16(Wl) && aligned16(Bh) && aligned16(Bl) && ldw % 8 == 0);
     VGAN_CHECK_ARG(splits >= 1 && splits <= 64 && (splits == 1 || slab_stride >= (int64_t)nr * ldo));
     VGAN_CHECK_ARG((tile == 0 || tile == 64 || tile == 128 || tile == 256) && (mul_shift == nullptr || mul != nullptr) && (!rm || zrows > 0));
@@ -802,12 +837,15 @@
     }
     const int ptiles = (p + 63) / 64;
     dim3 grid(ptiles * ((nr + 63) / 64) + nfin + xx.ntiles, splits);
-    if (rm)
-        hipLaunchKernelGGL((mmd_backward_bf3_kernel<64, true>), grid, dim3(kBlock), 0, st, Wh, Wl, ldw, Bh, Bl, kn, ldb, zrows, Z, ldz, wrow0, nr,
-                           p, ptiles, mul, ldmul, mul_shift, out, ldo, kchunk, (long)slab_stride, job, nfin, xx);
+    if (rebuild != nullptr)
+        hipLaunchKernelGGL((mmd_backward_bf3_kernel<64, true, true>), grid, dim3(kBlock), 0, st, Wh, Wl, ldw, Bh, Bl, kn, ldb, zrows, Z, ldz, wrow0,
+                           nr, p, ptiles, mul, ldmul, mul_shift, out, ldo, kchunk, (long)slab_stride, job, nfin, xx, rb);
+    else if (rm)
+        hipLaunchKernelGGL((mmd_backward_bf3_kernel<64, true, false>), grid, dim3(kBlock), 0, st, Wh, Wl, ldw, Bh, Bl, kn, ldb, zrows, Z, ldz, wrow0,
+                           nr, p, ptiles, mul, ldmul, mul_shift, out, ldo, kchunk, (long)slab_stride, job, nfin, xx, rb);
     else
-        hipLaunchKernelGGL((mmd_backward_bf3_kernel<64, false>), grid, dim3(kBlock), 0, st, Wh, Wl, ldw, Bh, Bl, kn, ldb, 0, Z, ldz, wrow0, nr, p,
-                           ptiles, mul, ldmul, mul_shift, out, ldo, kchunk, (long)slab_stride, job, nfin, xx);
+        hipLaunchKernelGGL((mmd_backward_bf3_kernel<64, false, false>), grid, dim3(kBlock), 0, st, Wh, Wl, ldw, Bh, Bl, kn, ldb, 0, Z, ldz, wrow0, nr,
+                           p, ptiles, mul, ldmul, mul_shift, out, ldo, kchunk, (long)slab_stride, job, nfin, xx, rb);
     VGAN_CHECK_LAUNCH();
     return VGAN_OK;
 }
@@ -836,3 +874,12 @@
     return launch_backward_bf3(1, Wh, Wl, ldw, Zh, Zl, kn, kp, zrows, Z, ldz, wrow0, nr, p, mul, ldmul, mul_shift, out, ldo, splits,
                                slab_stride, tile, finalize, stream, nullptr, rs_part, ldrs);
 }
+
+extern "C" int vgan_mmd_backward_bf3_rm_rebuild(const uint16_t* Wh, const uint16_t* Wl, int ldw, int kn, const uint16_t* Zh, const uint16_t* Zl,
+                                                int kp, int zrows, int nr, int p, const vgan_bwd_rebuild* rebuild, float* out, int ldo,
+                                                int splits, int64_t slab_stride, const vgan_finalize_job* finalize, const vgan_xx_job* xx,
+                                                vgan_stream_t stream) {
+    VGAN_CHECK_ARG(rebuild != nullptr);
+    return launch_backward_bf3(1, Wh, Wl, ldw, Zh, Zl, kn, kp, zrows, nullptr, 0, 0, nr, p, nullptr, 0, nullptr, out, ldo, splits, slab_stride, 64,
+                               finalize, stream, xx, nullptr, 0, rebuild);
+}
diff --git a/v-gan_amd/csrc/rows.hip b/v-gan_amd/csrc/rows.hip
--- a/v-gan_amd/csrc/rows.hip
+++ b/v-gan_amd/csrc/rows.hip
@@ -16,11 +16,6 @@
     }
 };
 
-__device__ __forceinline__ float project_centred(float u, float x, float c) {
-#pragma clang fp contract(off)
-    const float y = u * x;
-    return y - c;
-}
 
 template <bool PROJECT>
 __global__ __launch_bounds__(kBlock) void mask_forward_kernel(const float* __restrict__ logits, int ldl, const float* __restrict__ data,
@@ -194,7 +189,7 @@
                                                                  unsigned short* __restrict__ Zl, int kp, unsigned short* __restrict__ ZTh,
                                                                  unsigned short* __restrict__ ZTl, int kn, int n, int d,
                                                                  const float* __restrict__ center, int write_x, int mask_blocks,
-                                                                 XXJob xx, LogitsChain ch) {
+                                                                 XXJob xx, LogitsChain ch, int write_z, int* __restrict__ xrow) {
     constexpr int R = 8;
     if constexpr (XX) {
         __shared__ __attribute__((aligned(16))) char xx_lds[GemmBF3<64>::kLdsBytes];
@@ -219,7 +214,9 @@
         if constexpr (CHAIN) chain_logits<NT>(ch, reinterpret_cast<float*>(tile), d, i, i < n, v);
         if (i < n) {
             const float4* x4 = reinterpret_cast<const float4*>(logits + (long)i * ldl);
-            const float4* xr4 = reinterpret_cast<const float4*>(data + rows(i) * ldd);
+            const long src = rows(i);
+            const float4* xr4 = reinterpret_cast<const float4*>(data + src * ldd);
+            if (xrow != nullptr && lane == 0) xrow[i] = (int)src;
             float4 xv[NT], cv[NT];
 #pragma unroll
             for (int t = 0; t < NT; ++t) {
@@ -246,13 +243,16 @@
                 const int q = lane + 64 * t;
                 if (q < nq) {
                     const float4 s4 = make_float4(v[t].x / sum, v[t].y / sum, v[t].z / sum, v[t].w / sum);
-                    const float4 u4 = make_float4(s4.x < tau ? s4.x : 1.f, s4.y < tau ? s4.y : 1.f, s4.z < tau ? s4.z : 1.f, s4.w < tau ? s4.w : 1.f);
-                    const float4 x4c = make_float4(xv[t].x - cv[t].x, xv[t].y - cv[t].y, xv[t].z - cv[t].z, xv[t].w - cv[t].w);
+                    const float4 u4 = make_float4(upper_mask(s4.x, tau), upper_mask(s4.y, tau), upper_mask(s4.z, tau), upper_mask(s4.w, tau));
+                    const float4 x4c = make_float4(centred_x(xv[t].x, cv[t].x), centred_x(xv[t].y, cv[t].y), centred_x(xv[t].z, cv[t].z),
+                                                   centred_x(xv[t].w, cv[t].w));
                     const float4 y4 = make_float4(project_centred(u4.x, xv[t].x, cv[t].x), project_centred(u4.y, xv[t].y, cv[t].y), project_centred(u4.z, xv[t].z, cv[t].z),
                                               project_centred(u4.w, xv[t].w, cv[t].w));
                     reinterpret_cast<float4*>(S + (long)i * d)[q] = s4;
-                    if (write_x) reinterpret_cast<float4*>(Z + (long)i * ldz)[q] = x4c;
-                    reinterpret_cast<float4*>(Z + (long)(n + i) * ldz)[q] = y4;
+                    if (write_z) {
+                        if (write_x) reinterpret_cast<float4*>(Z + (long)i * ldz)[q] = x4c;
+                        reinterpret_cast<float4*>(Z + (long)(n + i) * ldz)[q] = y4;
+                    }
                     const float xs[4] = {x4c.x, x4c.y, x4c.z, x4c.w}, ys[4] = {y4.x, y4.y, y4.z, y4.w};
                     unsigned short h[2][4], l[2][4];
                     float xn[4], yn[4];
@@ -549,8 +549,18 @@
                                              float* sq, uint16_t* Zh, uint16_t* Zl, int kp, uint16_t* ZTh, uint16_t* ZTl, int kn,
                                              int n, int d, const float* center, int write_x, const vgan_xx_job* xxjob,
                                              const vgan_logits_chain* chain, vgan_stream_t stream) {
-    VGAN_CHECK_ARG((logits || chain) && data && S && Z && sq && Zh && Zl && n > 0 && d > 0 && (logits == nullptr || ldl >= d) && ldd >= d &&
-                   ldz >= d);
+    VGAN_CHECK_ARG(Z != nullptr);
+    return vgan_mask_project_forward_bf3_ex(logits, ldl, data, ldd, rows, row_cursor, row_batches, row_stride, S, Z, ldz, sq, Zh, Zl, kp, ZTh,
+                                            ZTl, kn, n, d, center, write_x, xxjob, chain, 1, nullptr, stream);
+}
+
+extern "C" int vgan_mask_project_forward_bf3_ex(const float* logits, int ldl, const float* data, int ldd, const int32_t* rows,
+                                                const uint64_t* row_cursor, int row_batches, int row_stride, float* S, float* Z, int ldz,
+                                                float* sq, uint16_t* Zh, uint16_t* Zl, int kp, uint16_t* ZTh, uint16_t* ZTl, int kn,
+                                                int n, int d, const float* center, int write_x, const vgan_xx_job* xxjob,
+                                                const vgan_logits_chain* chain, int write_z, int32_t* xrow, vgan_stream_t stream) {
+    VGAN_CHECK_ARG((logits || chain) && data && S && (Z || !write_z) && sq && Zh && Zl && n > 0 && d > 0 && (logits == nullptr || ldl >= d) &&
+                   ldd >= d && (!write_z || ldz >= d));
     LogitsChain ch{};
     if (chain != nullptr) {
         VGAN_CHECK_ARG(ZTh == nullptr && chain->za && chain->At4 && chain->e0 > 0 && chain->e0 % 4 == 0 && chain->ldza >= chain->e0 &&
@@ -561,8 +571,8 @@
     VGAN_CHECK_ARG((ZTh == nullptr) == (ZTl == nullptr));
     VGAN_CHECK_ARG(row_batches >= 1 && row_stride >= 0 && kp >= d && kp % 64 == 0 && (ZTh == nullptr || (kn >= 2 * n && kn % 64 == 0)));
     VGAN_CHECK_ARG(write_x || ZTh == nullptr);
-    VGAN_CHECK_ARG(d % 4 == 0 && d <= 1024 && n % 8 == 0 && ldl % 4 == 0 && ldd % 4 == 0 && ldz % 4 == 0);
-    VGAN_CHECK_ARG(aligned16(logits) && aligned16(data) && aligned16(S) && aligned16(Z) && aligned16(Zh) && aligned16(Zl) &&
+    VGAN_CHECK_ARG(d % 4 == 0 && d <= 1024 && n % 8 == 0 && ldl % 4 == 0 && ldd % 4 == 0 && (!write_z || ldz % 4 == 0));
+    VGAN_CHECK_ARG(aligned16(logits) && aligned16(data) && aligned16(S) && (!write_z || aligned16(Z)) && aligned16(Zh) && aligned16(Zl) &&
                    (ZTh == nullptr || (aligned16(ZTh) && aligned16(ZTl))) && (center == nullptr || aligned16(center)));
     const RowSel sel{rows, reinterpret_cast<const unsigned long long*>(row_cursor), row_batches, row_stride, 0};
     const int mask_blocks = 8 * ((n / 8 + 7) / 8);
@@ -587,7 +597,7 @@
             (void)hipFuncSetAttribute(reinterpret_cast<const void*>(&mask_forward_bf3_kernel<NT, XXF, CHF>),                          \
                                       hipFuncAttributeMaxDynamicSharedMemorySize, (int)shmem);                                      \
         hipLaunchKernelGGL((mask_forward_bf3_kernel<NT, XXF, CHF>), grid, block, shmem, st, logits, ldl, data, ldd, sel, S, Z, ldz, sq, \
-                           Zh, Zl, kp, ZTh, ZTl, kn, n, d, center, write_x, mask_blocks, xx, ch);                                    \
+                           Zh, Zl, kp, ZTh, ZTl, kn, n, d, center, write_x, mask_blocks, xx, ch, write_z, xrow);                     \
     } while (0)
 #define VGAN_LAUNCH_FWD3(NT)                                                                                                        \
     do {                                                                                                                            \
diff --git a/v-gan_amd/csrc/vgan_common.hpp b/v-gan_amd/csrc/vgan_common.hpp
--- a/v-gan_amd/csrc/vgan_common.hpp
+++ b/v-gan_amd/csrc/vgan_common.hpp
@@ -119,6 +119,11 @@
     return bf16_val(hi) + bf16_val(lo);
 }
 
+__device__ __forceinline__ float centred_x(float x, float c) { return __fsub_rn(x, c); }
+__device__ __forceinline__ float project_centred(float u, float x, float c) { return __fmaf_rn(u, x, -c); }
+__device__ __forceinline__ float uncentred_x(float xc, float c) { return __fadd_rn(xc, c); }
+__device__ __forceinline__ float upper_mask(float s, float tau) { return s < tau ? s : 1.0f; }
+
 inline bool aligned16(const void* p) { return (reinterpret_cast<uintptr_t>(p) & 15) == 0; }
 
 }
diff --git a/v-gan_amd/lib.py b/v-gan_amd/lib.py
--- a/v-gan_amd/lib.py
+++ b/v-gan_amd/lib.py
@@ -29,6 +29,10 @@
 class XXJob(ctypes.Structure):
     _fields_ = [("Dh", _p), ("Dl", _p), ("dsq", _p), ("tiles", _p), ("bw", _p), ("partial", _p), ("ldd", ctypes.c_int32),
                 ("ntiles", ctypes.c_int32)]
+
+
+class BwdRebuild(ctypes.Structure):
+    _fields_ = [("data", _p), ("xrow", _p), ("S", _p), ("center", _p), ("ldd", ctypes.c_int32), ("lds", ctypes.c_int32)]
 
 
 class AdadeltaLayer(ctypes.Structure):
@@ -83,6 +87,7 @@
     "vgan_mmd_backward_bf3_tile": (_i, [_i, _i, _i, _i]),
     "vgan_mmd_backward_bf3_rm": (_i, [_p, _p, _i, _i, _p, _p, _i, _i, _p, _i, _i, _i, _i, _p, _i, _p, _p, _i, _i, _i64, _i, _p, _p, _i, _p]),
     "vgan_mmd_backward_bf3_rm_xx": (_i, [_p, _p, _i, _i, _p, _p, _i, _i, _p, _i, _i, _i, _i, _p, _i, _p, _p, _i, _i, _i64, _p, _p, _p]),
+    "vgan_mmd_backward_bf3_rm_rebuild": (_i, [_p, _p, _i, _i, _p, _p, _i, _i, _i, _i, _p, _p, _i, _i, _i64, _p, _p, _p]),
     "vgan_row_sqnorm": (_i, [_p, _i, _p, _i, _i, _p]),
     "vgan_adadelta_step": (_i, [_p, _p, _i, _i64, _p, _p, _i64, _f, _f, _f, _f, _f, _p]),
     "vgan_noise_normal": (_i, [_p, _i, _i, _i, _i, _u64, _p, _u64, _p]),
@@ -91,6 +96,8 @@
     "vgan_gemm_grouped": (_i, [_p, _i, _p]),
     "vgan_gemm_grouped_ex": (_i, [_p, _i, _p, _p]),
     "vgan_mask_project_forward_bf3": (_i, [_p, _i, _p, _i, _p, _p, _i, _i, _p, _p, _i, _p, _p, _p, _i, _p, _p, _i, _i, _i, _p, _i, _p, _p, _p]),
+    "vgan_mask_project_forward_bf3_ex": (_i, [_p, _i, _p, _i, _p, _p, _i, _i, _p, _p, _i, _p, _p, _p, _i, _p, _p, _i, _i, _i, _p, _i, _p, _p, _i, _p,
+                                              _p]),
     "vgan_mse_grad": (_i, [_p, _i, _p, _i, _i, _i, _f, _p, _p, _i, _p]),
     "vgan_sum_f64": (_i, [_p, _i, ctypes.c_double, _p, _i, _p]),
     "vgan_rbf_kernel_matrix": (_i, [_p, _i, _i, _i, _p, _f, _p, _i, _p]),
diff --git a/v-gan_amd/ops.py b/v-gan_amd/ops.py
--- a/v-gan_amd/ops.py
+++ b/v-gan_amd/ops.py
@@ -126,16 +126,33 @@
                                                       n, d, _ptr(center), int(bool(norm_split)),
                                                       ctypes.byref(chain) if chain is not None else None, self._stream()), "vgan_mask_project_forward")
 
+    bf3_rebuild = True
+
     def xx_job(self, Dh, Dl, dsq, tiles, bw, partial):
         assert tiles.is_contiguous() and partial.is_contiguous() and Dh.stride(0) == Dl.stride(0)
         return _lib.XXJob(_ptr(Dh), _ptr(Dl), _ptr(dsq), _ptr(tiles), _ptr(bw), _ptr(partial), Dh.stride(0), tiles.shape[0])
 
+    def bwd_rebuild(self, data, xrow, S, center):
+        _mat(data, "data"), _mat(S, "S")
+        assert xrow.dtype == torch.int32 and xrow.is_contiguous() and center.is_contiguous()
+        return _lib.BwdRebuild(_ptr(data), _ptr(xrow), _ptr(S), _ptr(center), data.stride(0), S.stride(0))
+
     def mask_project_forward_bf3(self, logits, data, rows, S, Z, sq, Zh, Zl, ZTh, ZTl, row_cursor=None, row_batches=1, row_stride=0,
-                                 center=None, write_x=True, xx=None, chain=None):
+                                 center=None, write_x=True, xx=None, chain=None, write_z=True, xrow=None):
         _mat(data, "data"), _mat(Z, "Z"), _mat(S, "S")
         n, d = S.shape
         if logits is not None:
             _mat(logits, "logits")
+        if not write_z or xrow is not None:
+            _lib.check(self.lib.vgan_mask_project_forward_bf3_ex(_ptr(logits), logits.stride(0) if logits is not None else 0, _ptr(data),
+                                                                 data.stride(0), _ptr(rows), _ptr(row_cursor), int(row_batches),
+                                                                 int(row_stride), _ptr(S), _ptr(Z), Z.stride(0), _ptr(sq), _ptr(Zh), _ptr(Zl),
+                                                                 Zh.stride(0), _ptr(ZTh), _ptr(ZTl), ZTh.stride(0) if ZTh is not None else 0,
+                                                                 n, d, _ptr(center), int(bool(write_x)),
+                                                                 ctypes.byref(xx) if xx is not None else None,
+                                                                 ctypes.byref(chain) if chain is not None else None, int(bool(write_z)),
+                                                                 _ptr(xrow), self._stream()), "vgan_mask_project_forward_bf3_ex")
+            return
         _lib.check(self.lib.vgan_mask_project_forward_bf3(_ptr(logits), logits.stride(0) if logits is not None else 0, _ptr(data), data.stride(0), _ptr(rows),
                                                           _ptr(row_cursor), int(row_batches), int(row_stride), _ptr(S), _ptr(Z), Z.stride(0),
                                                           _ptr(sq), _ptr(Zh), _ptr(Zl), Zh.stride(0), _ptr(ZTh), _ptr(ZTl),
@@ -334,6 +351,16 @@
                                                      ctypes.byref(finalize) if finalize is not None else None, _ptr(rs_part),
                                                      rs_part.stride(0) if rs_part is not None else 0, self._stream()),
                    "vgan_mmd_backward_bf3_rm")
+
+    def mmd_backward_bf3_rm_rebuild(self, Wh, Wl, Zh, Zl, zrows, nr, p, rebuild, out, splits=1, slab_stride=0, finalize=None, xx=None):
+        _mat(out, "out")
+        kn = (int(zrows) + 63) // 64 * 64
+        assert Wh.stride(0) >= kn and Zh.shape[0] >= zrows
+        _lib.check(self.lib.vgan_mmd_backward_bf3_rm_rebuild(_ptr(Wh), _ptr(Wl), Wh.stride(0), kn, _ptr(Zh), _ptr(Zl), Zh.stride(0), int(zrows),
+                                                             int(nr), int(p), ctypes.byref(rebuild), _ptr(out), out.stride(0), int(splits),
+                                                             int(slab_stride), ctypes.byref(finalize) if finalize is not None else None,
+                                                             ctypes.byref(xx) if xx is not None else None, self._stream()),
+                   "vgan_mmd_backward_bf3_rm_rebuild")
 
     def mmd_backward_bf3_tile(self, nr, p, splits=1, tile=0):
         return int(self.lib.vgan_mmd_backward_bf3_tile(int(nr), int(p), int(splits), int(tile)))
diff --git a/v-gan_amd/trainer.py b/v-gan_amd/trainer.py
--- a/v-gan_amd/trainer.py
+++ b/v-gan_amd/trainer.py
@@ -280,6 +280,12 @@
             late = self.tiles.shape[0] - self.n_main
             bwd_wgs = ((d + 63) // 64) * ((nl + 63) // 64) * self.bsplits + 1
             self.xx_late_in_backward = (ops.mmd_backward_bf3_tile(nl, d, self.bsplits, self.bwd_tile) == 64 and late <= 512 - bwd_wgs)
+        plain_bf3 = (getattr(ops, "bf3_rebuild", False) and self.bf3 and self.fused_prepare and self.gram_tile == 64 and
+                     self.rm_backward and world == 1 and not self.overlap and not self.front_sharded and
+                     ops.mmd_backward_bf3_tile(nl, d, self.bsplits, self.bwd_tile) == 64)
+        self.lean = plain_bf3 and os.environ.get("VGAN_Z_FP32", "0") != "1"
+        self.xrow = torch.zeros(n, dtype=torch.int32, device=self.dev) if self.lean else None
+        self._rebuild = None
         self.tiles_cal = self.tiles if (world == 1 and self.gram_tile == 64 and not (self.overlap or self.xx_ride or self.xx_in_m4 or self.front_sharded)) else ops.build_tiles(n, 0, 0, 1, device=self.dev)
         self.partial = torch.zeros(max(self.tiles.shape[0], self.tiles_cal.shape[0]), 4, **f32)
         self.stats = torch.zeros(4, dtype=torch.float64, device=self.dev)
@@ -537,8 +543,12 @@
                     ntx = self.tiles.shape[0] - self.n_main
                     self._xx = ops.xx_job(self.Dh, self.Dl, self.dsq, self.tiles[self.n_main:], self.bw, self.partial[self.n_main:self.n_main + ntx])
                 xx = self._xx
-            ops.mask_project_forward_bf3(logits, self.data, self.perm, self.S, self.Z, self.sqn, self.Zh, self.Zl, self.ZTh, self.ZTl,
-                                         center=self.center, write_x=not self.x_ahead, xx=xx, **rowsel)
+            if self.lean:
+                ops.mask_project_forward_bf3(logits, self.data, self.perm, self.S, self.Z, self.sqn, self.Zh, self.Zl, None, None,
+                                             center=self.center, xx=xx, write_z=not self.has_bw, xrow=self.xrow, **rowsel)
+            else:
+                ops.mask_project_forward_bf3(logits, self.data, self.perm, self.S, self.Z, self.sqn, self.Zh, self.Zl, self.ZTh, self.ZTl,
+                                             center=self.center, write_x=not self.x_ahead, xx=xx, **rowsel)
             return
         if self.x_ahead:
             ops.mask_project_forward(logits, self.data, self.perm, self.S, None, None, self.Z[n:], None, self.sqn[n:],
@@ -582,7 +592,12 @@
                 self._fin = ops.finalize_job(*fin_args)
         fin = self._fin
         if bf3:
-            if self.rm_backward:
+            if self.lean:
+                if self._rebuild is None:
+                    self._rebuild = ops.bwd_rebuild(self.data, self.xrow, self.S, self.center)
+                ops.mmd_backward_bf3_rm_rebuild(self.Wh, self.Wl, self.Zh, self.Zl, 2 * n, nl, d, self._rebuild, self.gU, self.bsplits, gstride,
+                                                fin, xx=self._late_xx_job() if self.xx_late_in_backward else None)
+            elif self.rm_backward:
                 ops.mmd_backward_bf3_rm(self.Wh, self.Wl, self.Zh, self.Zl, 2 * n, self.Z, n + lo, nl, d, self.Z[lo:lo + nl], self.gU,
                                         self.bsplits, gstride, fin, mul_shift=self.center, tile=self.bwd_tile,
                                         xx=self._late_xx_job() if self.xx_late_in_backward else None, rs_part=self.rs_part)
```

Measured after the change: 10160 steps/s, median of 6. +3.6%, better.
